# anonymousauthors001/SGS-GNN

Measured on AMD Instinct MI355X. Metric: sampled edges/sec + training steps/sec, Reddit hybrid 20% sparsity, higher is better.
Workload: dtype f32

## Files before the change

### include/sgs_hip.h

```cpp
#ifndef SGS_HIP_H_
#define SGS_HIP_H_

#include <stddef.h>
#include <stdint.h>

#ifdef __cplusplus
extern "C" {
#endif

#define SGS_ABI_VERSION 1

#define SGS_OK 0
#define SGS_EINVAL (-1)
#define SGS_EWORKSPACE (-2)
#define SGS_EHIP (-3)

typedef void* sgs_stream_t;

int sgs_abi_version(void);
const char* sgs_last_error(void);

int sgs_rng_set_epoch_buffer(const uint64_t* epoch_dev);
int sgs_exp_noise(uint64_t seed, uint64_t stream_id, int64_t E, float* noise, sgs_stream_t stream);
int sgs_dropout_keep(uint64_t seed, uint32_t site, int64_t rows, int64_t cols, float p, uint8_t* keep,
// ... 171 lines not shown
                            const float* W1, const float* b1, const float* w2, const float* b2, float p_drop,
                            uint64_t seed, uint32_t site, float* dv, float* hdz_part, float* dz, float* feat, void* ws,
                            size_t ws_bytes, sgs_stream_t stream);
int sgs_edge_score_bwd_dfeat_supported(int64_t H);
int sgs_edge_score_bwd_dfeat(const float* dv, int64_t n, int64_t H, const float* W1, float* dfeat, void* ws, size_t ws_bytes,
                             sgs_stream_t stream);

int sgs_edge_score_bwd_bits_supported(int64_t H);
int sgs_edge_score_fwd_mask(const float* codes, const float* U, int64_t N, int64_t H, const int64_t* edge_index, int64_t E,
                            int64_t edge_id_offset, const int32_t* canon, int64_t M, const int32_t* mate, const float* W1, const float* b1,
                            const float* w2, const float* b2, float p_drop, uint64_t seed, uint32_t site, float* p_out, uint32_t* maskbits,
                            void* ws, size_t ws_bytes, sgs_stream_t stream);
int sgs_edge_score_bwd_prep(const float* codes, int64_t N, int64_t H, const int64_t* edge_index, int64_t E, const int64_t* active_eid,
                            int64_t n_active, const float* grad_p, const float* p, const uint32_t* maskbits, float* dz, uint32_t* dvbits,
                            float* feat, sgs_stream_t stream);
int sgs_edge_score_dw2_from_parts(const float* W1, const float* T_raw, const float* U, const float* R_raw, const float* b1, const float* c_raw,
                                  int64_t N, int64_t H, float p_drop, float* dw2, sgs_stream_t stream);
int sgs_edge_score_probe_set(int stagger, int prio, uint32_t mode_mask);
int sgs_edge_score_probe_trace(unsigned long long* buf);
size_t sgs_edge_score_epd_workspace_bytes(int64_t H);
int sgs_edge_score_epd_fwd(const float* A, int64_t N, int64_t H, const int64_t* edge_index, int64_t E, int64_t edge_id_offset, const float* W1,
                           const float* b1, const float* w2, const float* b2, float p_hidden, uint64_t seed, uint32_t site, float p_ep,
                           uint64_t seed_x, uint32_t site_x, uint64_t seed_y, uint32_t site_y, float* p_out, void* ws, size_t ws_bytes,
                           sgs_stream_t stream);
int sgs_edge_score_epd_bwd_core(const float* A, int64_t N, int64_t H, const int64_t* edge_index, int64_t E, int64_t edge_id_offset,
                                const int64_t* active_eid, int64_t n_active, const float* grad_p, const float* W1, const float* b1, const float* w2,
                                const float* b2, float p_hidden, uint64_t seed, uint32_t site, float p_ep, uint64_t seed_x, uint32_t site_x,
                                uint64_t seed_y, uint32_t site_y, float* dv, float* hdz_part, float* dz, float* feat2, void* ws, size_t ws_bytes,
                                sgs_stream_t stream);
int sgs_edge_score_epd_reduce(const float* dfeat2, const float* A, int64_t N, int64_t H, const int32_t* in_ptr, const int32_t* in_src,
                              const int32_t* in_eid, const int32_t* out_ptr, const int32_t* out_dst, const int32_t* out_eid,
                              const int64_t* active_eid, int64_t edge_id_offset, float p_ep, uint64_t seed_x, uint32_t site_x, uint64_t seed_y,
                              uint32_t site_y, float* dA, sgs_stream_t stream);

int sgs_edge_score_bwd_prep_sd(const float* codes, int64_t N, int64_t H, const int64_t* edge_index, int64_t E, const int64_t* active_eid,
                               int64_t n_active, const float* grad_p, const float* p, const uint32_t* maskbits, float* dz, uint32_t* dvbits,
                               int32_t* sd, sgs_stream_t stream);
size_t sgs_edge_score_bwd_fused_opart_rows(int64_t n, int64_t N);
int sgs_edge_score_bwd_dfeat_fused(const uint32_t* dvbits, const float* dz, const int32_t* sd, const float* codes, int64_t n, int64_t N, int64_t H,
                                   const float* W1, const float* w2, float p_drop, float* G, float* opart, void* ws, size_t ws_bytes,
                                   sgs_stream_t stream);
int sgs_edge_score_bwd_reduce_fused(const float* G, const float* opart, const uint32_t* dvbits, const float* dz, const float* w2, float p_drop,
                                    int64_t N, int64_t H, int64_t nnz, const int32_t* in_ptr, const int32_t* in_eid, const int32_t* out_ptr,
                                    float* out_codes, float* out_U, float* out_U_raw, sgs_stream_t stream);
int sgs_edge_score_bwd_prep_sd_pack(const float* codes, int64_t N, int64_t H, const int64_t* edge_index, int64_t E, const int64_t* active_eid,
                                    int64_t n_active, const float* grad_p, const float* p, const uint32_t* maskbits, float* dz, uint32_t* dvbits,
                                    int32_t* sd, const float* W1, const float* w2, float p_drop, void* ws, size_t ws_bytes, sgs_stream_t stream);
int sgs_edge_score_bwd_dfeat_fused_packed(const uint32_t* dvbits, const float* dz, const int32_t* sd, const float* codes, int64_t n, int64_t N,
                                          int64_t H, float* G, float* opart, const void* ws, size_t ws_bytes, sgs_stream_t stream);
int sgs_edge_score_bwd_core_bits(const float* codes, const float* U, int64_t N, int64_t H, const int64_t* edge_index, int64_t E,
                                 int64_t edge_id_offset, const int64_t* active_eid, int64_t n_active, const float* grad_p, const float* W1,
                                 const float* b1, const float* w2, const float* b2, float p_drop, uint64_t seed, uint32_t site,
                                 uint32_t* dvbits, float* hdz_part, float* dz, float* feat, void* ws, size_t ws_bytes, sgs_stream_t stream);
int sgs_edge_score_bwd_dfeat_bits(const uint32_t* dvbits, const float* dz, int64_t n, int64_t H, const float* W1, const float* w2, float p_drop,
                                  float* dfeat, void* ws, size_t ws_bytes, sgs_stream_t stream);
int sgs_endpoint_reduce_pair_bits(const float* dfeat, const uint32_t* dvbits, const float* dz, const float* w2, float p_drop, const float* codes,
                                  int64_t N, int64_t H, int64_t nnz, const int32_t* in_ptr, const int32_t* in_src, const int32_t* in_eid,
                                  const int32_t* out_ptr, const int32_t* out_dst, const int32_t* out_eid, float* out_codes, float* out_U,
                                  float* out_U_raw, sgs_stream_t stream);
int sgs_gemm_tn_mask_supported(int64_t K, int64_t M, int64_t N);
int sgs_gemm_tn_mask_gather(const uint32_t* Abits, const float* dz, const float* rowscale, float scale, const float* codes, int64_t codes_rows,
                            const int32_t* sd, int64_t K, int64_t M, int64_t N, float* C, int64_t ldc, float* colsum_A, float* dz_sum, float* C_raw,
                            float* colsum_raw, void* ws, size_t ws_bytes, sgs_stream_t stream);
void sgs_gemm_tn_set_gather_variant(int shared, int slabs);
int sgs_gemm_tn_mask(const uint32_t* Abits, const float* dz, const float* rowscale, float scale, const float* B, int64_t K, int64_t M, int64_t N,
                     float* C, int64_t ldc, float* colsum_A, float* dz_sum, float* C_raw, float* colsum_raw, void* ws, size_t ws_bytes,
                     sgs_stream_t stream);

int sgs_edge_score_bf16_supported(int64_t H);
int sgs_edge_score_fwd_bf16(const float* codes, const float* U, int64_t N, int64_t H, const int64_t* edge_index, int64_t E,
                            int64_t edge_id_offset, const float* W1, const float* b1, const float* w2, const float* b2, float p_drop,
                            uint64_t seed, uint32_t site, float* p_out, void* ws, size_t ws_bytes, sgs_stream_t stream);
int sgs_edge_score_fwd_paired_bf16(const float* codes, const float* U, int64_t N, int64_t H, const int64_t* edge_index, int64_t E,
                                   int64_t edge_id_offset, const int32_t* canon, int64_t M, const int32_t* mate, const float* W1, const float* b1,
                                   const float* w2, const float* b2, float p_drop, uint64_t seed, uint32_t site, float* p_out, void* ws,
                                   size_t ws_bytes, sgs_stream_t stream);
int sgs_edge_score_fwd_mask_bf16(const float* codes, const float* U, int64_t N, int64_t H, const int64_t* edge_index, int64_t E,
                                 int64_t edge_id_offset, const int32_t* canon, int64_t M, const int32_t* mate, const float* W1, const float* b1,
                                 const float* w2, const float* b2, float p_drop, uint64_t seed, uint32_t site, float* p_out, uint32_t* maskbits,
                                 void* ws, size_t ws_bytes, sgs_stream_t stream);
int sgs_edge_score_bwd_dfeat_bits_bf16(const uint32_t* dvbits, const float* dz, int64_t n, int64_t H, const float* W1, const float* w2,
                                       float p_drop, float* dfeat, void* ws, size_t ws_bytes, sgs_stream_t stream);
int sgs_edge_score_bwd_prep_sd_pack_bf16(const float* codes, int64_t N, int64_t H, const int64_t* edge_index, int64_t E, const int64_t* active_eid,
                                         int64_t n_active, const float* grad_p, const float* p, const uint32_t* maskbits, float* dz, uint32_t* dvbits,
                                         int32_t* sd, const float* W1, const float* w2, float p_drop, void* ws, size_t ws_bytes, sgs_stream_t stream);
int sgs_edge_score_bwd_dfeat_fused_bf16(const uint32_t* dvbits, const float* dz, const int32_t* sd, const float* codes, int64_t n, int64_t N,
                                        int64_t H, const float* W1, const float* w2, float p_drop, float* G, float* opart, void* ws, size_t ws_bytes,
                                        sgs_stream_t stream);
int sgs_edge_score_bwd_dfeat_fused_packed_bf16(const uint32_t* dvbits, const float* dz, const int32_t* sd, const float* codes, int64_t n, int64_t N,
                                               int64_t H, float* G, float* opart, const void* ws, size_t ws_bytes, sgs_stream_t stream);
int sgs_gemm_tn_mask_bf16(const uint32_t* Abits, const float* dz, const float* rowscale, float scale, const float* B, int64_t K, int64_t M, int64_t N,
                          float* C, int64_t ldc, float* colsum_A, float* dz_sum, float* C_raw, float* colsum_raw, void* ws, size_t ws_bytes,
                          sgs_stream_t stream);
int sgs_gemm_tn_mask_gather_bf16(const uint32_t* Abits, const float* dz, const float* rowscale, float scale, const float* codes, int64_t codes_rows,
                                 const int32_t* sd, int64_t K, int64_t M, int64_t N, float* C, int64_t ldc, float* colsum_A, float* dz_sum, float* C_raw,
                                 float* colsum_raw, void* ws, size_t ws_bytes, sgs_stream_t stream);

int sgs_endpoint_reduce(const float* M_out, const float* M_in, const float* T, int64_t N, int64_t H, int64_t nnz,
                        const int32_t* in_ptr, const int32_t* in_src, const int32_t* in_eid, const int32_t* out_ptr,
                        const int32_t* out_dst, const int32_t* out_eid, float sign_out, float sign_in, float* out,
                        sgs_stream_t stream);
int sgs_endpoint_reduce_pair(const float* dfeat, const float* dv, const float* codes, int64_t N, int64_t H, int64_t nnz,
                             const int32_t* in_ptr, const int32_t* in_src, const int32_t* in_eid, const int32_t* out_ptr,
                             const int32_t* out_dst, const int32_t* out_eid, float* out_codes, float* out_U, sgs_stream_t stream);

int sgs_masked_correct(const float* logits, int64_t N, int64_t C, const int64_t* y, const uint8_t* train_mask,
                       int32_t* correct, sgs_stream_t stream);
int sgs_masked_correct_pair(const float* logits_a, const float* logits_b, int64_t N, int64_t C, const int64_t* y,
                            const uint8_t* train_mask, int32_t* correct4, sgs_stream_t stream);

int sgs_confusion_counts(const float* logits, int64_t N, int64_t C, const int64_t* y, const uint8_t* m0, const uint8_t* m1, const uint8_t* m2,
                         int64_t* conf, sgs_stream_t stream);
int sgs_confusion_variant(int64_t N, int64_t C);
int sgs_confusion_variant_set(int code);

size_t sgs_gate_counts_workspace_bytes(int64_t N);
int sgs_gate_counts(const float* logits_a, const float* logits_b, int64_t N, int64_t C, const int64_t* y, const uint8_t* train_mask,
                    int32_t* out5, const uint64_t* seq_dev, int32_t* dst_host_mapped, void* ws, size_t ws_bytes, sgs_stream_t stream);

int sgs_loss_tick(float* loss_sum, const float* loss, uint64_t* epoch, sgs_stream_t stream);
int sgs_publish_to_host(const int32_t* src_dev, int64_t n, const uint64_t* seq_dev, int32_t* dst_host_mapped, sgs_stream_t stream);

int sgs_masked_ce_fwd(const float* logits, int64_t N, int64_t C, const int64_t* y, const uint8_t* train_mask,
                      float* loss, float* row_lse, float* rowloss, int32_t* n_rows, sgs_stream_t stream);
int sgs_masked_ce_bwd(const float* logits, int64_t N, int64_t C, const int64_t* y, const uint8_t* train_mask,
                      const float* row_lse, const int32_t* n_rows, const float* grad_loss, float* dlogits,
                      sgs_stream_t stream);

size_t sgs_edge_reg_workspace_bytes(int64_t q);
int sgs_edge_reg_fwd(const float* w, const int64_t* sampled_edge_index, int64_t q, const float* logits, int64_t N,
                     int64_t C, const int64_t* y, const uint8_t* train_mask, float coef1, float coef2, float* out,
                     float* cos_out, void* ws, size_t ws_bytes, sgs_stream_t stream);
int sgs_edge_reg_bwd(const float* w, const int64_t* sampled_edge_index, int64_t q, int64_t q_global, const float* logits,
                     int64_t N, int64_t C, const int64_t* y, const uint8_t* train_mask, const float* out, float coef1,
                     float coef2, const float* grad_loss, float* dw, float* Gs, float* Gd, sgs_stream_t stream);

int sgs_hybrid_loss_fwd(const float* logits, int64_t N, int64_t C, const int64_t* y, const uint8_t* train_mask, const float* w,
                        const int64_t* sampled_edge_index, int64_t q, float coef1, float coef2, float* out, float* row_lse, float* rowloss,
                        int32_t* n_rows, void* ws, size_t ws_bytes, sgs_stream_t stream);
int sgs_masked_ce_bwd_acc(const float* logits, int64_t N, int64_t C, const int64_t* y, const uint8_t* train_mask, const float* row_lse,
                          const int32_t* n_rows, const float* grad_loss, float* dlogits, sgs_stream_t stream);

int sgs_masked_ce_w_fwd(const float* logits, int64_t N, int64_t C, const int64_t* y, const uint8_t* train_mask, const float* weight,
                        float label_smoothing, float* loss, float* row_lse, float* rowloss, float* den, sgs_stream_t stream);
int sgs_masked_ce_w_bwd(const float* logits, int64_t N, int64_t C, const int64_t* y, const uint8_t* train_mask, const float* weight,
                        float label_smoothing, const float* row_lse, const float* den, const float* grad_loss, float* dlogits,
                        sgs_stream_t stream);
int sgs_masked_ce_w_bwd_acc(const float* logits, int64_t N, int64_t C, const int64_t* y, const uint8_t* train_mask, const float* weight,
                            float label_smoothing, const float* row_lse, const float* den, const float* grad_loss, float* dlogits,
                            sgs_stream_t stream);
int sgs_hybrid_loss_w_fwd(const float* logits, int64_t N, int64_t C, const int64_t* y, const uint8_t* train_mask, const float* w,
                          const int64_t* sampled_edge_index, int64_t q, float coef1, float coef2, const float* weight, float label_smoothing,
                          float* out, float* row_lse, float* rowloss, float* den, void* ws, size_t ws_bytes, sgs_stream_t stream);

int sgs_edge_reg_partial(const float* w, const int64_t* sampled_edge_index, int64_t q, const float* logits, int64_t N,
                         int64_t C, const int64_t* y, const uint8_t* train_mask, float* raw, void* ws, size_t ws_bytes,
                         sgs_stream_t stream);

int sgs_gat_scores_fwd(const float* xl, int64_t N, int64_t D, const float* att_src, const float* att_dst, float* a_src, float* a_dst,
                       sgs_stream_t stream);
size_t sgs_gat_scores_bwd_workspace_bytes(int64_t N, int64_t D);
int sgs_gat_scores_bwd(const float* xl, int64_t N, int64_t D, const float* att_src, const float* att_dst, const float* g_src, const float* g_dst,
                       int accumulate, float* dxl, float* datt_src, float* datt_dst, void* ws, size_t ws_bytes, sgs_stream_t stream);
int sgs_gat_alpha_fwd(const float* a_src, const float* a_dst, int64_t N, int64_t n_edges, const int32_t* in_ptr,
                      const int32_t* in_src, const int32_t* in_eid, float negative_slope, float p_drop, uint64_t seed,
                      uint32_t site, float* soft_in, float* soft_loop, float* alpha_in, float* alpha_loop,
                      sgs_stream_t stream);
int sgs_gat_alpha_bwd(const float* a_src, const float* a_dst, int64_t N, int64_t n_edges, const int32_t* in_ptr,
                      const int32_t* in_src, const int32_t* in_eid, float negative_slope, float p_drop, uint64_t seed,
                      uint32_t site, const float* soft_in, const float* soft_loop, const float* galpha,
                      const float* gloop, float* g_edge, float* g_selfloop, float* d_a_dst, sgs_stream_t stream);
int sgs_gather_by_eid(const float* by_eid, const int32_t* eid, int64_t n, float* out_order, sgs_stream_t stream);
int sgs_scatter_by_eid(const float* in_order, const int32_t* eid, int64_t n, float* by_eid, sgs_stream_t stream);

#define SGS_HEADS_CONCAT 0
#define SGS_HEADS_MEAN 1
#define SGS_HEADS_BROADCAST 2
int sgs_gat_heads_supported(int64_t K, int64_t C);
#define SGS_GAT_OP_SCORES_FWD 0
#define SGS_GAT_OP_SCORES_BWD 1
#define SGS_GAT_OP_SPMM_CONCAT 2
#define SGS_GAT_OP_SPMM_MEAN 3
#define SGS_GAT_OP_SPMM_BROADCAST 4
#define SGS_GAT_OP_SDDMM 5
#define SGS_GAT_OP_SDDMM_BROADCAST 6
#define SGS_GAT_OP_ROW 7
int sgs_gat_heads_variant(int op, int64_t N, int64_t K, int64_t C, int aligned16);
int sgs_gat_scores_heads_fwd(const float* xl, int64_t N, int64_t K, int64_t C, const float* att_src, const float* att_dst, float* a_src,
                             float* a_dst, sgs_stream_t stream);
size_t sgs_gat_scores_heads_bwd_workspace_bytes(int64_t N, int64_t K, int64_t C);
int sgs_gat_scores_heads_bwd(const float* xl, int64_t N, int64_t K, int64_t C, const float* att_src, const float* att_dst, const float* g_src,
                             const float* g_dst, int accumulate, float* dxl, float* datt_src, float* datt_dst, void* ws, size_t ws_bytes,
                             sgs_stream_t stream);
int sgs_gat_alpha_heads_fwd(const float* a_src, const float* a_dst, int64_t N, int64_t K, int64_t n_edges, const int32_t* in_ptr,
                            const int32_t* in_src, const int32_t* in_eid, float negative_slope, float p_drop, uint64_t seed, uint32_t site,
                            float* soft, float* soft_loop, float* alpha, float* alpha_loop, sgs_stream_t stream);
int sgs_gat_alpha_heads_bwd(const float* a_src, const float* a_dst, int64_t N, int64_t K, int64_t n_edges, const int32_t* in_ptr,
                            const int32_t* in_src, const int32_t* in_eid, float negative_slope, float p_drop, uint64_t seed, uint32_t site,
                            const float* soft, const float* soft_loop, const float* galpha, const float* gloop, float* g_edge, float* g_selfloop,
                            float* d_a_dst, sgs_stream_t stream);
int sgs_gat_alpha_heads_edge_fwd(const float* a_src, const float* a_dst, const float* edge_w, const float* edge_coef, int64_t N, int64_t K,
                                 int64_t n_edges, const int32_t* in_ptr, const int32_t* in_src, const int32_t* in_eid, float negative_slope,
                                 float p_drop, uint64_t seed, uint32_t site, float* soft, float* soft_loop, float* alpha, float* alpha_loop,
                                 float* loop_w, float* loop_inv_cnt, sgs_stream_t stream);
size_t sgs_gat_alpha_heads_edge_bwd_workspace_bytes(int64_t N, int64_t K);
int sgs_gat_alpha_heads_edge_bwd(const float* a_src, const float* a_dst, const float* edge_w, const float* edge_coef, const float* loop_w,
                                 const float* loop_inv_cnt, int64_t N, int64_t K, int64_t n_edges, const int32_t* in_ptr, const int32_t* in_src,
                                 const int32_t* in_eid, float negative_slope, float p_drop, uint64_t seed, uint32_t site, const float* soft,
                                 const float* soft_loop, const float* galpha, const float* gloop, const float* dw_add, float* g_edge,
                                 float* g_selfloop, float* d_a_dst, float* d_edge_w, float* d_edge_coef, void* ws, size_t ws_bytes,
                                 sgs_stream_t stream);
int sgs_edge_sum_by_row_heads(const float* g_edge, const float* g_self, int64_t N, int64_t K, int64_t nnz, const int32_t* ptr, const int32_t* eid,
                              float* out, sgs_stream_t stream);
int sgs_spmm_csr_heads(const float* X, int64_t N, int64_t K, int64_t C, int64_t nnz, const int32_t* ptr, const int32_t* col, const int32_t* eid,
                       const float* val, const float* diag, int mode, const float* bias, int act, float p_drop, uint64_t seed, uint32_t site,
                       float* Y, sgs_stream_t stream);
int sgs_sddmm_csr_heads(const float* A, const float* B, int64_t N, int64_t K, int64_t C, int64_t nnz, const int32_t* ptr, const int32_t* col,
                        const int32_t* eid, int broadcast, float* g, float* gdiag, sgs_stream_t stream);

#define SGS_GATV2_OP_ALPHA_FWD 0
#define SGS_GATV2_OP_ALPHA_BWD 1
#define SGS_GATV2_OP_DXL 2
int sgs_gatv2_variant(int op, int64_t N, int64_t K, int64_t C, int aligned16);
int sgs_gatv2_alpha_heads_fwd(const float* xl, const float* xr, const float* att, const float* edge_w, const float* lin_edge, int64_t N,
                              int64_t K, int64_t C, int64_t n_edges, const int32_t* in_ptr, const int32_t* in_src, const int32_t* in_eid,
                              float negative_slope, float p_drop, uint64_t seed, uint32_t site, float* soft, float* soft_loop, float* alpha,
                              float* alpha_loop, float* loop_w, float* loop_inv_cnt, sgs_stream_t stream);
int sgs_gatv2_alpha_heads_fwd_multi(const float* xl, const float* xr, int64_t x_stride, const float* att, const float* edge_w,
                                    const float* lin_edge, int64_t N, int64_t K, int64_t C, int64_t D, int64_t nnz, const int32_t* in_ptr,
                                    const int32_t* in_src, const int32_t* in_eid, float negative_slope, float* alpha, float* alpha_loop,
                                    sgs_stream_t stream);
size_t sgs_gatv2_alpha_heads_bwd_workspace_bytes(int64_t N, int64_t K, int64_t C);
int sgs_gatv2_alpha_heads_bwd(const float* xl, const float* xr, const float* att, const float* edge_w, const float* lin_edge, const float* loop_w,
                              const float* loop_inv_cnt, int64_t N, int64_t K, int64_t C, int64_t n_edges, const int32_t* in_ptr,
                              const int32_t* in_src, const int32_t* in_eid, float negative_slope, float p_drop, uint64_t seed, uint32_t site,
                              const float* soft, const float* soft_loop, const float* galpha, const float* gloop, const float* dw_add,
                              float* g_logit, float* g_loop, float* d_xr, float* d_att, float* d_lin_edge, float* d_edge_w, void* ws,
                              size_t ws_bytes, sgs_stream_t stream);
int sgs_gatv2_dxl_heads(const float* xl, const float* xr, const float* att, const float* edge_w, const float* lin_edge, const float* loop_w,
                        const float* g_logit, const float* g_loop, int64_t N, int64_t K, int64_t C, int64_t nnz, const int32_t* out_ptr,
                        const int32_t* out_dst, const int32_t* out_eid, float negative_slope, int accumulate, float* d_xl,
                        sgs_stream_t stream);

int sgs_gine_variant(int64_t N, int64_t D, int64_t nnz, int align_bytes);
int sgs_gine_aggregate_fwd(const float* x, const float* edge_w, const float* a, const float* b, float diag, int64_t N, int64_t D,
                           int64_t n_edges, const int32_t* in_ptr, const int32_t* in_src, const int32_t* in_eid, float* z,
                           sgs_stream_t stream);
int sgs_gine_aggregate_fwd_multi(const float* x, int64_t x_stride, const float* edge_w, const float* a, const float* b, float diag,
                                 int64_t N, int64_t Dc, int64_t nnz, int64_t D, const int32_t* in_ptr, const int32_t* in_src,
                                 const int32_t* in_eid, float* z, sgs_stream_t stream);
size_t sgs_gine_aggregate_bwd_workspace_bytes(int64_t N, int64_t D);
int sgs_gine_aggregate_bwd(const float* x, const float* dz, const float* edge_w, const float* a, const float* b, float diag, int64_t N,
                           int64_t D, int64_t n_edges, const int32_t* out_ptr, const int32_t* out_dst, const int32_t* out_eid,
                           const float* dw_add, float* d_x, float* d_edge_w, float* d_a, float* d_b, void* ws, size_t ws_bytes,
                           sgs_stream_t stream);

int sgs_cheb_supported(int64_t K);
int sgs_cheb_norm_fwd(const float* w, int64_t n_edges, int64_t N, const int32_t* in_ptr, const int32_t* in_src, const int32_t* in_eid,
                      const int32_t* out_ptr, const int32_t* out_dst, const int32_t* out_eid, float* dis, float* l_in, float* l_out,
                      sgs_stream_t stream);
size_t sgs_cheb_norm_bwd_workspace_bytes(int64_t N);
int sgs_cheb_norm_bwd(const float* w, const float* g, const float* g2, int64_t n_edges, int64_t N, const float* dis, const int32_t* in_ptr,
                      const int32_t* in_src, const int32_t* in_eid, const int32_t* out_ptr, const int32_t* out_dst, const int32_t* out_eid,
                      const int64_t* edge_index, float* dw, void* ws, size_t ws_bytes, sgs_stream_t stream);
int sgs_cheb_spmm_variant(int64_t N, int64_t D, int64_t nnz, int64_t ldx, int aligned16);
int sgs_cheb_spmm(int64_t K, const float* X, int64_t ldx, int64_t N, int64_t D, int64_t nnz, const int32_t* ptr, const int32_t* col,
                  const float* val, float alpha, const float* add, int64_t ldadd, const float* sub, int64_t ldsub, const float* bias, int act,
                  float p_drop, uint64_t seed, uint32_t site, float* Y, int64_t ldy, float* Y2, int64_t ldy2, float scale2,
                  sgs_stream_t stream);

size_t sgs_gemm_tn_workspace_bytes(int64_t K, int64_t M, int64_t N);
int sgs_gemm_tn(const float* A, const float* B, int64_t K, int64_t M, int64_t N, float* C, void* ws, size_t ws_bytes,
                sgs_stream_t stream);
void sgs_gemm_tn_set_tall_variant(int variant);
int sgs_gemm_tn_can_colsum(int64_t K, int64_t M, int64_t N);
int sgs_gemm_tn_colsum(const float* A, const float* B, int64_t K, int64_t M, int64_t N, float* C, float* colsum_A, void* ws,
                       size_t ws_bytes, sgs_stream_t stream);
int sgs_gemm_tn_ld(const float* A, const float* B, int64_t K, int64_t M, int64_t N, float* C, int64_t ldc, float* colsum_A, void* ws,
                   size_t ws_bytes, sgs_stream_t stream);
typedef struct SgsGemmTnProblem {
    const float* A;
    const float* B;
    int64_t K, M, N;
    float* C;
    int64_t ldc;
    void* ws;
    size_t ws_bytes;
} SgsGemmTnProblem;
int sgs_gemm_tn_group_supported(int64_t K, int64_t M, int64_t N);
int sgs_gemm_tn_group(const SgsGemmTnProblem* problems, int count, sgs_stream_t stream);

int sgs_er_weight(const int64_t* edge_index, int64_t E, int64_t N, const int32_t* out_ptr, const int32_t* out_dst, int walk_lengths,
                  int walks, uint64_t seed, float* weight, sgs_stream_t stream);

int sgs_adam_max_tensors(void);
int sgs_adam_step(const int64_t* desc_host, int64_t n_tensors, float lr, float beta1, float beta2, float eps, float weight_decay,
                  int maximize, uint32_t* ticket, sgs_stream_t stream);
int sgs_adam_multi_max_tensors(void);
int sgs_adam_step_multi(const int64_t* desc_host, const float* hyper_host, int64_t n_tensors, uint32_t* ticket, float* loss_sum, const float* loss,
                        uint64_t* epoch, sgs_stream_t stream);

size_t sgs_sample_topq_multi_workspace_bytes(int64_t E, int64_t D);
int sgs_sample_topq_multi(int mode, const float* p, const float* prior, double degree_bias_coef, const float* noise, uint64_t seed,
                          uint64_t stream_id0, int64_t D, int64_t E, int64_t q, const int64_t* edge_index, uint8_t* mask, int64_t* sampled_eid,
                          int64_t* sampled_edge_index, float* stats, float* st_weights, void* ws, size_t ws_bytes, sgs_stream_t stream);
size_t sgs_sample_topq_multi_cover_workspace_bytes(int64_t E, int64_t N, int64_t D);
// ... 41 lines not shown
```

### sgs-gnn_amd/csrc/edge_score.hip

```cpp
#include <type_traits>

#include "sgs_common.h"

namespace sgs {
namespace {

constexpr int kT = 256;
constexpr int kBM = 64;
constexpr int kBK = 16;
using f32x16 = __attribute__((ext_vector_type(16))) float;

__global__ void __launch_bounds__(kT) transpose_w1a(const float* __restrict__ W1, int H, float* __restrict__ WaT) {
    __shared__ float t[32][33];
    const int bx = blockIdx.x * 32, by = blockIdx.y * 32;
    const int tx = threadIdx.x & 31, ty = threadIdx.x >> 5;
    for (int r = ty; r < 32; r += 8) {
        const int h = by + r, k = bx + tx;
        t[r][tx] = (h < H && k < H) ? W1[static_cast<int64_t>(h) * 2 * H + k] : 0.f;
    }
    __syncthreads();
    for (int r = ty; r < 32; r += 8) {
        const int k = bx + r, h = by + tx;
        if (k < H && h < H) WaT[static_cast<int64_t>(k) * H + h] = t[tx][r];
    }
}

__global__ void __launch_bounds__(kT) transpose_w1_full(const float* __restrict__ W1, int H, float* __restrict__ WT) {
    __shared__ float t[32][33];
    const int bx = blockIdx.x * 32, by = blockIdx.y * 32;
    const int tx = threadIdx.x & 31, ty = threadIdx.x >> 5;
    for (int r = ty; r < 32; r += 8) {
        const int h = by + r, k = bx + tx;
        t[r][tx] = (h < H && k < 2 * H) ? W1[static_cast<int64_t>(h) * 2 * H + k] : 0.f;
    }
    __syncthreads();
    for (int r = ty; r < 32; r += 8) {
        const int k = bx + r, h = by + tx;
        if (k < 2 * H && h < H) WT[static_cast<int64_t>(k) * H + h] = t[tx][r];
    }
}

struct ScoreArgs {
    const float* codes;
    const float* U;
    const int64_t* src;
    const int64_t* dst;
    const int64_t* active;
    int64_t n;
    const int32_t* canon;
    const int32_t* mate;
    const int64_t* dyn_n;
    int64_t row_offset;
    int H;
    const float* WaT;
    const float* b1;
    const float* w2;
    const float* b2;
    float drop_scale;
    uint32_t drop_thresh;
    uint64_t seed;
    const uint64_t* epoch;
    uint32_t site;
    int use_drop;
    float* p_out;
    const float* gp;
    float* dv;
    float* hdz;
    float* dz;
    float* feat;
    uint32_t* dvbits;
    const uint32_t* inbits;
    const float* indz;
    int epd;
    uint64_t seed_x, seed_y;
    uint32_t site_x, site_y;
    float ep_scale;
    uint32_t ep_thresh;
    const int32_t* sd;
    float* opart;
    int stagger, prio;
    unsigned long long* trace;
};

template <int NT, bool BWD, bool EXACT, bool EPD = false>
__global__ void __launch_bounds__(kT, 3) edge_score_kernel(ScoreArgs a) {
    constexpr int HP = 32 * NT;
    constexpr int NTW = NT / 2;
    extern __shared__ __attribute__((aligned(16))) char smem[];
    float* Wt_s0 = reinterpret_cast<float*>(smem);
    float* Ft_s0 = Wt_s0 + 2 * kBK * HP;
    int* s_idx = reinterpret_cast<int*>(Ft_s0 + 2 * kBK * kBM);
    int* d_idx = s_idx + kBM;
    float* zpart = reinterpret_cast<float*>(d_idx + kBM);
    const int tid = threadIdx.x, lane = tid & 63, wave = tid >> 6;
    const int eg = wave & 1, hh = wave >> 1;
    const int H = EXACT ? HP : a.H;
    const int64_t row0 = static_cast<int64_t>(blockIdx.x) * kBM;
    if (a.dyn_n) {
        const int64_t live_n = *a.dyn_n;
        if (live_n < a.n) a.n = live_n;
        if (row0 >= a.n) return;
    }

    if (tid < kBM) {
        const int64_t r = row0 + tid;
        int s = 0, d = 0;
        if (r < a.n) {
            const int64_t e = a.active ? a.active[r] : r;
            s = static_cast<int>(a.src[e]);
            d = static_cast<int>(a.dst[e]);
        }
        s_idx[tid] = s;
        d_idx[tid] = d;
    }

    f32x16 acc[NTW];
#pragma unroll
    for (int t = 0; t < NTW; ++t)
#pragma unroll
        for (int r = 0; r < 16; ++r) acc[t][r] = 0.f;

    const int kh = lane >> 5, l31 = lane & 31;
    __syncthreads();

    constexpr int kWV = (kBK * (HP / 4) + kT - 1) / kT;
    float4 wreg[kWV], xreg, yreg;
    const int fe = tid & (kBM - 1), fc = tid >> 6;
    const int my_s = s_idx[fe], my_d = d_idx[fe];
    const int KT = EPD ? 2 * H : H;
    uint32_t rkx = 0u, rky = 0u;
    if (EPD) {
        const int64_t r_ = row0 + fe;
        const int64_t e_ = r_ < a.n ? (a.active ? a.active[r_] : r_) : 0;
        rkx = dropout_row_key(fold_epoch(a.seed_x, a.epoch), a.site_x, static_cast<uint64_t>(a.row_offset + e_));
        rky = dropout_row_key(fold_epoch(a.seed_y, a.epoch), a.site_y, static_cast<uint64_t>(a.row_offset + e_));
    }
    auto ep_mask = [&](float4& v, uint32_t rk, int kk) {
        const uint32_t b0 = dropout_pair_bits(rk, static_cast<uint32_t>(kk >> 1)), b1 = dropout_pair_bits(rk, static_cast<uint32_t>((kk >> 1) + 1));
        v.x = (b0 & 0xFFFFu) >= a.ep_thresh ? v.x * a.ep_scale : 0.f;
        v.y = (b0 >> 16) >= a.ep_thresh ? v.y * a.ep_scale : 0.f;
        v.z = (b1 & 0xFFFFu) >= a.ep_thresh ? v.z * a.ep_scale : 0.f;
        v.w = (b1 >> 16) >= a.ep_thresh ? v.w * a.ep_scale : 0.f;
    };
    auto fetch = [&](int k0) {
#pragma unroll
        for (int j = 0; j < kWV; ++j) {
            const int i = j * kT + tid;
            const int k = i / (HP / 4), h4 = (i % (HP / 4)) * 4;
            wreg[j] = make_float4(0.f, 0.f, 0.f, 0.f);
            if (EXACT || (i < kBK * (HP / 4) && k0 + k < KT && h4 < H))
                wreg[j] = *reinterpret_cast<const float4*>(a.WaT + static_cast<int64_t>(k0 + k) * H + h4);
        }
        const int kf = k0 + 4 * fc;
        const int kk = (EPD && kf >= H) ? kf - H : kf;
        xreg = make_float4(0.f, 0.f, 0.f, 0.f);
// ... 1367 lines not shown
#pragma unroll
    for (int i = 0; i < 4 * NT; ++i) {
        if (8 * i < Hrt) {
            const int t = i >> 2, g4 = i & 3;
            const int hb = 8 * i + 4 * kh;
            const float4 ww = *reinterpret_cast<const float4*>(&bw[1][hb]);
            const float w4[4] = {ww.x, ww.y, ww.z, ww.w};
            float dv4[4], hs[4];
#pragma unroll
            for (int j = 0; j < 4; ++j) {
                const float hd = acc[t][4 * g4 + j];
                dv4[j] = dzv * w4[j] * (hd > 0.f ? dscale : 0.f);
                hs[j] = dzv * hd;
                mbits[t] |= (hd > 0.f ? 1u : 0u) << (8 * g4 + 4 * kh + j);
            }
            if (live && a.dv) *reinterpret_cast<float4*>(a.dv + r * H + hb) = make_float4(dv4[0], dv4[1], dv4[2], dv4[3]);
#pragma unroll
            for (int j = 0; j < 4; ++j) hs[j] = half_wave_sum_hi(hs[j]);
            if (l31 == 31) *reinterpret_cast<float4*>(hsum + wave * H + hb) = make_float4(hs[0], hs[1], hs[2], hs[3]);
        }
    }
    if (a.dvbits) {
#pragma unroll
        for (int t = 0; t < NT; ++t) mbits[t] |= __shfl_xor(mbits[t], 32, 64);
        if (live && kh == 0) {
            uint4* bo = reinterpret_cast<uint4*>(a.dvbits + r * NT);
#pragma unroll
            for (int t = 0; t < NT; t += 4) bo[t >> 2] = make_uint4(mbits[t], mbits[t + 1], mbits[t + 2], mbits[t + 3]);
        }
    }
    __syncthreads();
    for (int idx = tid; idx < (NW / 2) * H; idx += TH) {
        const int m = idx / H, h = idx - m * H;
        const int64_t prow = static_cast<int64_t>(blockIdx.x) * (NW / 2) + m;
        if (prow * 64 < a.n) a.hdz[prow * H + h] = hsum[(2 * m) * H + h] + hsum[(2 * m + 1) * H + h];
    }
}

template <int NT, int THREADS>
__global__ void __launch_bounds__(THREADS, THREADS / 256) edge_score_wres_kernel(ScoreArgs a, const float* __restrict__ Wp,
                                                                                  const float* __restrict__ Ceo,
                                                                                  unsigned int* __restrict__ tile_ctr,
                                                                                  float* __restrict__ zpart) {
    constexpr int H = 32 * NT;
    constexpr int NTW = NT / 2;
    constexpr int NJ4 = H / 8;
    extern __shared__ __attribute__((aligned(16))) char smem[];
    float4* Ws = reinterpret_cast<float4*>(smem);
    const int tid = threadIdx.x, lane = tid & 63;
    const int hh = blockIdx.x & 1;
    const int kh = lane >> 5, l31 = lane & 31;
    {
        const float4* src = reinterpret_cast<const float4*>(Wp) + static_cast<int64_t>(hh) * NTW * NJ4 * 64;
        for (int i = tid; i < NTW * NJ4 * 64; i += THREADS) Ws[i] = src[i];
    }
    __syncthreads();
    const int64_t n_tiles = (a.n + 31) >> 5;
    const int Hrt = a.H;
    for (;;) {
        unsigned int t32 = 0;
        if (lane == 0) t32 = atomicAdd(&tile_ctr[hh], 1u);
        t32 = __builtin_amdgcn_readfirstlane(t32);
        if (static_cast<int64_t>(t32) >= n_tiles) break;
        const int64_t r = static_cast<int64_t>(t32) * 32 + l31;
        const bool live = r < a.n;
        int s = 0, d = 0;
        int64_t eg_id = 0;
        if (live) {
            eg_id = a.active ? a.active[r] : r;
            s = static_cast<int>(a.src[eg_id]);
            d = static_cast<int>(a.dst[eg_id]);
        }
        const float4* xp = reinterpret_cast<const float4*>(Ceo + static_cast<int64_t>(s) * H + kh * (H / 2));
        const float4* yp = reinterpret_cast<const float4*>(Ceo + static_cast<int64_t>(d) * H + kh * (H / 2));
        f32x16 acc[NTW];
#pragma unroll
        for (int t = 0; t < NTW; ++t)
#pragma unroll
            for (int q = 0; q < 16; ++q) acc[t][q] = 0.f;
        float4 A0[NTW], A1[NTW], x0, y0, x1, y1;
        auto load = [&](int j4, float4 (&A)[NTW], float4& x, float4& y) {
#pragma unroll
            for (int t = 0; t < NTW; ++t) A[t] = Ws[(t * NJ4 + j4) * 64 + lane];
            x = xp[j4];
            y = yp[j4];
        };
        auto mma = [&](const float4 (&A)[NTW], const float4& x, const float4& y) {
            const float b[4] = {x.x * y.x, x.y * y.y, x.z * y.z, x.w * y.w};
#pragma unroll
            for (int jj = 0; jj < 4; ++jj) {
#pragma unroll
                for (int t = 0; t < NTW; ++t) {
                    const float av = jj == 0 ? A[t].x : jj == 1 ? A[t].y : jj == 2 ? A[t].z : A[t].w;
                    acc[t] = __builtin_amdgcn_mfma_f32_32x32x2f32(av, b[jj], acc[t], 0, 0, 0);
                }
            }
        };
        load(0, A0, x0, y0);
#pragma unroll 1
        for (int j4 = 0; j4 < NJ4; j4 += 2) {
            load(j4 + 1, A1, x1, y1);
            mma(A0, x0, y0);
            if (j4 + 2 < NJ4) load(j4 + 2, A0, x0, y0);
            mma(A1, x1, y1);
        }
        const uint32_t rkey = dropout_row_key(fold_epoch(a.seed, a.epoch), a.site, static_cast<uint64_t>(a.row_offset + eg_id));
        const float* Us = a.U + static_cast<int64_t>(s) * H;
        const float* Ud = a.U + static_cast<int64_t>(d) * H;
        float z = 0.f;
#pragma unroll
        for (int t = 0; t < NTW; ++t) {
#pragma unroll
            for (int g = 0; g < 4; ++g) {
                const int hb = hh * (H / 2) + 32 * t + 8 * g + 4 * kh;
                if (hb < Hrt) {
                    const float4 us = *reinterpret_cast<const float4*>(Us + hb);
                    const float4 ud = *reinterpret_cast<const float4*>(Ud + hb);
                    const float4 bb = *reinterpret_cast<const float4*>(a.b1 + hb);
                    const float4 ww = *reinterpret_cast<const float4*>(a.w2 + hb);
                    const float u4[4] = {us.x - ud.x, us.y - ud.y, us.z - ud.z, us.w - ud.w};
                    const float b4[4] = {bb.x, bb.y, bb.z, bb.w};
                    const float w4[4] = {ww.x, ww.y, ww.z, ww.w};
                    uint32_t bits[2] = {0u, 0u};
                    if (a.use_drop) {
                        bits[0] = dropout_pair_bits(rkey, static_cast<uint32_t>(hb >> 1));
                        bits[1] = dropout_pair_bits(rkey, static_cast<uint32_t>((hb >> 1) + 1));
                    }
#pragma unroll
                    for (int j = 0; j < 4; ++j) {
                        const float v = (acc[t][4 * g + j] + u4[j]) + b4[j];
                        float m = v > 0.f ? 1.f : 0.f;
                        if (a.use_drop) {
                            const uint32_t draw = (j & 1) ? (bits[j >> 1] >> 16) : (bits[j >> 1] & 0xFFFFu);
                            m = draw >= a.drop_thresh ? m * a.drop_scale : 0.f;
                        }
                        z = fmaf(w4[j], v * m, z);
                    }
                }
            }
        }
        z += __shfl_xor(z, 32, 64);
        if (live && kh == 0) zpart[static_cast<int64_t>(hh) * a.n + r] = z;
    }
}

__global__ void __launch_bounds__(kT) edge_score_finish(const float* __restrict__ zpart, int64_t n, const float* __restrict__ b2,
                                                       float* __restrict__ p_out) {
    const int64_t r = static_cast<int64_t>(blockIdx.x) * kT + threadIdx.x;
    if (r >= n) return;
    const float z = (zpart[r] + zpart[n + r]) + b2[0];
    p_out[r] = 1.0f / (1.0f + expf(-z));
}

template <int VEC, bool HAS_T>
__global__ void __launch_bounds__(kT) endpoint_reduce(const float* __restrict__ Mo, const float* __restrict__ Mi,
                                                     const float* __restrict__ T, int64_t N, int64_t H,
                                                     const int* __restrict__ in_ptr, const int* __restrict__ in_src,
                                                     const int* __restrict__ in_eid, const int* __restrict__ out_ptr,
                                                     const int* __restrict__ out_dst, const int* __restrict__ out_eid,
                                                     float sgn_out, float sgn_in, float* __restrict__ out) {
    const int lane = threadIdx.x & 63;
    const int64_t v = (static_cast<int64_t>(blockIdx.x) * kT + threadIdx.x) >> 6;
    if (v >= N) return;
    for (int64_t c0 = static_cast<int64_t>(lane) * VEC; c0 < H; c0 += 64 * VEC) {
        float acc[VEC];
#pragma unroll
        for (int j = 0; j < VEC; ++j) acc[j] = 0.f;
        for (int dir = 0; dir < 2; ++dir) {
            const int* ptr = dir == 0 ? out_ptr : in_ptr;
            const int* col = dir == 0 ? out_dst : in_src;
            const int* eid = dir == 0 ? out_eid : in_eid;
            const float sg = dir == 0 ? sgn_out : sgn_in;
            const float* M = dir == 0 ? Mo : Mi;
            const int b = ptr[v], e = ptr[v + 1];
            for (int k = b; k < e; ++k) {
                float m[VEC], t[VEC];
                if (VEC == 4) {
                    *reinterpret_cast<float4*>(m) = *reinterpret_cast<const float4*>(M + static_cast<int64_t>(eid[k]) * H + c0);
                    if (HAS_T) *reinterpret_cast<float4*>(t) = *reinterpret_cast<const float4*>(T + static_cast<int64_t>(col[k]) * H + c0);
                } else {
                    m[0] = M[static_cast<int64_t>(eid[k]) * H + c0];
                    if (HAS_T) t[0] = T[static_cast<int64_t>(col[k]) * H + c0];
                }
#pragma unroll
                for (int j = 0; j < VEC; ++j) acc[j] = fmaf(sg * m[j], HAS_T ? t[j] : 1.0f, acc[j]);
            }
        }
        if (VEC == 4) *reinterpret_cast<float4*>(out + v * H + c0) = *reinterpret_cast<float4*>(acc);
        else out[v * H + c0] = acc[0];
    }
}

template <int VEC, bool HAS_T, int NW>
__global__ void __launch_bounds__(64 * NW) endpoint_reduce_rowblock(const float* __restrict__ Mo, const float* __restrict__ Mi,
                                                              const float* __restrict__ T, int64_t N, int64_t H,
                                                              const int* __restrict__ in_ptr, const int* __restrict__ in_src,
                                                              const int* __restrict__ in_eid, const int* __restrict__ out_ptr,
                                                              const int* __restrict__ out_dst, const int* __restrict__ out_eid,
                                                              float sgn_out, float sgn_in, float* __restrict__ out) {
    using V = typename std::conditional<VEC == 4, float4, float>::type;
    __shared__ float part[NW][64 * VEC];
    const int lane = threadIdx.x & 63, wave = threadIdx.x >> 6;
    const int64_t v = blockIdx.x;
    const int ob = out_ptr[v], no = out_ptr[v + 1] - ob;
    const int ib = in_ptr[v], ni = in_ptr[v + 1] - ib;
    const int total = no + ni;
    for (int64_t cbase = 0; cbase < H; cbase += 64 * VEC) {
        const int64_t c0 = cbase + static_cast<int64_t>(lane) * VEC;
        float acc[VEC];
#pragma unroll
        for (int j = 0; j < VEC; ++j) acc[j] = 0.f;
        if (c0 < H) {
            for (int k0 = wave; k0 < total; k0 += 4 * NW) {
                float m[4][VEC], t[4][VEC], sg[4];
                int er[4], cr[4];
                const float* Mp[4];
#pragma unroll
                for (int u = 0; u < 4; ++u) {
                    const int k = k0 + NW * u;
                    const int kc = k < total ? k : total - 1;
                    const bool isout = kc < no;
                    const int idx = isout ? ob + kc : ib + (kc - no);
                    er[u] = (isout ? out_eid : in_eid)[idx];
                    if (HAS_T) cr[u] = (isout ? out_dst : in_src)[idx];
                    Mp[u] = isout ? Mo : Mi;
                    sg[u] = k < total ? (isout ? sgn_out : sgn_in) : 0.f;
                }
#pragma unroll
                for (int u = 0; u < 4; ++u) {
                    *reinterpret_cast<V*>(m[u]) = *reinterpret_cast<const V*>(Mp[u] + static_cast<int64_t>(er[u]) * H + c0);
                    if (HAS_T) *reinterpret_cast<V*>(t[u]) = *reinterpret_cast<const V*>(T + static_cast<int64_t>(cr[u]) * H + c0);
                    else {
#pragma unroll
                        for (int j = 0; j < VEC; ++j) t[u][j] = 1.f;
                    }
                }
#pragma unroll
                for (int u = 0; u < 4; ++u)
#pragma unroll
                    for (int j = 0; j < VEC; ++j) acc[j] = fmaf(sg[u] * m[u][j], t[u][j], acc[j]);
            }
        }
#pragma unroll
        for (int j = 0; j < VEC; ++j) part[wave][lane * VEC + j] = acc[j];
        __syncthreads();
        const int tt = threadIdx.x;
        if (tt < 64 * VEC && cbase + tt < H) {
            float sum = 0.f;
#pragma unroll
            for (int g = 0; g < NW; g += 4) sum += (part[g][tt] + part[g + 1][tt]) + (part[g + 2][tt] + part[g + 3][tt]);
            out[v * H + cbase + tt] = sum;
        }
        __syncthreads();
    }
}

__global__ void __launch_bounds__(kT) scorer_bwd_prep(const float* __restrict__ codes, int64_t H, const int64_t* __restrict__ src,
                                                     const int64_t* __restrict__ dst, const int64_t* __restrict__ active, int64_t n,
                                                     const float* __restrict__ gp, const float* __restrict__ p,
                                                     const uint32_t* __restrict__ maskbits, float* __restrict__ dz,
                                                     uint32_t* __restrict__ bits, float* __restrict__ feat, int32_t* __restrict__ sd) {
    constexpr int R = 4;
    const int lane = threadIdx.x & 63;
    const int64_t r0 = ((static_cast<int64_t>(blockIdx.x) * kT + threadIdx.x) >> 6) * R;
    if (r0 >= n) return;
    const int wpr = static_cast<int>(H >> 5);
    int64_t e[R], s[R], d[R];
#pragma unroll
    for (int u = 0; u < R; ++u) {
        const int64_t r = r0 + u < n ? r0 + u : n - 1;
        e[u] = active ? active[r] : r;
    }
#pragma unroll
    for (int u = 0; u < R; ++u) { s[u] = src[e[u]]; d[u] = dst[e[u]]; }
#pragma unroll
    for (int u = 0; u < R; ++u) {
        if (r0 + u >= n) break;
        if (lane < wpr) bits[(r0 + u) * wpr + lane] = maskbits[e[u] * wpr + lane];
        if (lane == 63) { const float pe = p[e[u]]; dz[r0 + u] = gp[r0 + u] * pe * (1.0f - pe); }
        if (sd && lane == 62) { sd[2 * (r0 + u)] = static_cast<int32_t>(s[u]); sd[2 * (r0 + u) + 1] = static_cast<int32_t>(d[u]); }
    }
    if (!feat) return;
    for (int64_t c0 = static_cast<int64_t>(lane) * 4; c0 < H; c0 += 256) {
        float4 a[R], b[R];
#pragma unroll
        for (int u = 0; u < R; ++u) {
            a[u] = *reinterpret_cast<const float4*>(codes + s[u] * H + c0);
            b[u] = *reinterpret_cast<const float4*>(codes + d[u] * H + c0);
        }
#pragma unroll
        for (int u = 0; u < R; ++u)
            if (r0 + u < n)
                *reinterpret_cast<float4*>(feat + (r0 + u) * H + c0) = make_float4(a[u].x * b[u].x, a[u].y * b[u].y, a[u].z * b[u].z, a[u].w * b[u].w);
    }
}

template <int P = 3>
__global__ void __launch_bounds__(kT) scorer_bwd_prep_sd_pack(const int64_t* __restrict__ src, const int64_t* __restrict__ dst,
                                                             const int64_t* __restrict__ active, int64_t n, int wpr,
                                                             const float* __restrict__ gp, const float* __restrict__ p,
                                                             const uint32_t* __restrict__ maskbits, float* __restrict__ dz,
                                                             uint32_t* __restrict__ bits, int2* __restrict__ sd, int64_t n_prep_blocks,
                                                             const float* __restrict__ W1, int H, uint4* __restrict__ Wp16,
                                                             const float* __restrict__ w2, float scale) {
    if (static_cast<int64_t>(blockIdx.x) >= n_prep_blocks) {
        pack_w1a_bf16x3_one<true, P>((static_cast<int64_t>(blockIdx.x) - n_prep_blocks) * kT + threadIdx.x, W1, H, Wp16, w2, scale);
        return;
    }
    const int64_t r = static_cast<int64_t>(blockIdx.x) * kT + threadIdx.x;
    if (r >= n) return;
    const int64_t e = active ? active[r] : r;
    const int64_t s = src[e], d = dst[e];
    const float pe = p[e], g = gp[r];
    if ((wpr & 3) == 0) {
        const uint4* mi = reinterpret_cast<const uint4*>(maskbits + e * wpr);
        uint4* mo = reinterpret_cast<uint4*>(bits + r * wpr);
        for (int k = 0; k < (wpr >> 2); ++k) mo[k] = mi[k];
    } else {
        for (int k = 0; k < wpr; ++k) bits[r * wpr + k] = maskbits[e * wpr + k];
    }
    dz[r] = g * pe * (1.0f - pe);
    sd[r] = make_int2(static_cast<int32_t>(s), static_cast<int32_t>(d));
}

__global__ void __launch_bounds__(kT) scorer_dw2_from_parts(const float* __restrict__ W1, const float* __restrict__ Traw, const float* __restrict__ U,
                                                           const float* __restrict__ Rraw, const float* __restrict__ b1,
                                                           const float* __restrict__ craw, int64_t N, int H, float scale,
                                                           float* __restrict__ dw2) {
    __shared__ float red[kT / 64];
    const int h = blockIdx.x;
    float a = 0.f, b = 0.f;
    for (int k = threadIdx.x; k < H; k += kT) a = fmaf(W1[static_cast<int64_t>(h) * 2 * H + k], Traw[static_cast<int64_t>(h) * H + k], a);
    for (int64_t v = threadIdx.x; v < N; v += kT) b = fmaf(U[v * H + h], Rraw[v * H + h], b);
    const float ra = block_sum(a, red);
    const float rb = block_sum(b, red);
    if (threadIdx.x == 0) dw2[h] = scale * ((ra + rb) + b1[h] * craw[h]);
}

constexpr int kEpU = 4;
template <int NW, bool BITS = false>
__global__ void __launch_bounds__(64 * NW) endpoint_reduce_pair_rowblock(const float* __restrict__ dfeat, const float* __restrict__ dv,
                                                                        const float* __restrict__ codes, int64_t N, int64_t H,
                                                                        const int* __restrict__ in_ptr, const int* __restrict__ in_src,
                                                                        const int* __restrict__ in_eid, const int* __restrict__ out_ptr,
                                                                        const int* __restrict__ out_dst, const int* __restrict__ out_eid,
                                                                        float* __restrict__ out_codes, float* __restrict__ out_U,
                                                                        const uint32_t* __restrict__ bits = nullptr,
                                                                        const float* __restrict__ dz = nullptr,
                                                                        const float* __restrict__ w2 = nullptr, float scale = 1.f,
                                                                        float* __restrict__ out_Uraw = nullptr) {
    __shared__ float part[2][NW][256];
    const int lane = threadIdx.x & 63, wave = threadIdx.x >> 6;
    const int64_t v = blockIdx.x;
    const int ob = out_ptr[v], no = out_ptr[v + 1] - ob;
    const int ib = in_ptr[v], ni = in_ptr[v + 1] - ib;
    const int total = no + ni;
    for (int64_t cbase = 0; cbase < H; cbase += 256) {
        const int64_t c0 = cbase + static_cast<int64_t>(lane) * 4;
        float a1[4] = {0.f, 0.f, 0.f, 0.f}, a2[4] = {0.f, 0.f, 0.f, 0.f};
        if (c0 < H) {
            for (int k0 = wave; k0 < total; k0 += kEpU * NW) {
                int er[kEpU], cr[kEpU];
                float sg[kEpU], ok[kEpU];
#pragma unroll
                for (int u = 0; u < kEpU; ++u) {
                    const int k = k0 + NW * u;
                    const int kc = k < total ? k : total - 1;
                    const bool isout = kc < no;
                    const int idx = isout ? ob + kc : ib + (kc - no);
                    er[u] = (isout ? out_eid : in_eid)[idx];
                    cr[u] = (isout ? out_dst : in_src)[idx];
                    ok[u] = k < total ? 1.f : 0.f;
                    sg[u] = k < total ? (isout ? 1.f : -1.f) : 0.f;
                }
                float m1[kEpU][4], m2[kEpU][4], t[kEpU][4];
                uint32_t wd[kEpU];
                float dzr[kEpU];
#pragma unroll
                for (int u = 0; u < kEpU; ++u) {
                    *reinterpret_cast<float4*>(m1[u]) = *reinterpret_cast<const float4*>(dfeat + static_cast<int64_t>(er[u]) * H + c0);
                    *reinterpret_cast<float4*>(t[u]) = *reinterpret_cast<const float4*>(codes + static_cast<int64_t>(cr[u]) * H + c0);
                    if constexpr (BITS) {
                        wd[u] = bits[static_cast<int64_t>(er[u]) * (H >> 5) + (c0 >> 5)];
                        dzr[u] = dz[er[u]];
                    } else {
                        *reinterpret_cast<float4*>(m2[u]) = *reinterpret_cast<const float4*>(dv + static_cast<int64_t>(er[u]) * H + c0);
                    }
                }
#pragma unroll
                for (int u = 0; u < kEpU; ++u) {
                    if constexpr (BITS) {
                        const uint32_t w = wd[u] >> (c0 & 31);
#pragma unroll
                        for (int j = 0; j < 4; ++j) m2[u][j] = (w >> j) & 1u ? dzr[u] : 0.f;
                    }
#pragma unroll
                    for (int j = 0; j < 4; ++j) {
                        a1[j] = fmaf(ok[u] * m1[u][j], t[u][j], a1[j]);
                        a2[j] = fmaf(sg[u], m2[u][j], a2[j]);
                    }
                }
            }
        }
#pragma unroll
        for (int j = 0; j < 4; ++j) { part[0][wave][lane * 4 + j] = a1[j]; part[1][wave][lane * 4 + j] = a2[j]; }
        __syncthreads();
        for (int tt = threadIdx.x; tt < 512; tt += 64 * NW) {
            const int which = tt >> 8, c = tt & 255;
// ... 528 lines not shown
    SGS_REQUIRE(n_active >= 0 && (active_eid || n_active == E), SGS_EINVAL,
                "sgs_edge_score_bwd_core: n_active must equal E when active_eid is NULL");
    if (n_active == 0) return SGS_OK;
    SGS_REQUIRE(codes && U && edge_index && grad_p && W1 && b1 && w2 && b2 && (dv || dvbits) && hdz_part && dz && feat, SGS_EINVAL,
                "sgs_edge_score_bwd_core: null pointer");
    SGS_REQUIRE(ws && ws_bytes >= sgs_edge_score_workspace_bytes(N, H, 0), SGS_EWORKSPACE, "sgs_edge_score_bwd_core: workspace too small");
    Carver cv(ws);
    float* WaT = cv.take<float>(static_cast<size_t>(H) * H);
    float* Ceo = cv.take<float>(static_cast<size_t>(N) * H);
    if (H > 256) {
        SGS_REQUIRE(dv && !dvbits && N > 0, SGS_EINVAL, "sgs_edge_score_bwd_core: H=%lld needs the dense dv form", (long long)H);
        hipLaunchKernelGGL(transpose_w1a, dim3(cdiv(H, 32), cdiv(H, 32)), dim3(kT), 0, stream, W1, static_cast<int>(H), WaT);
        ScoreArgs a{};
        a.codes = codes; a.U = U; a.src = edge_index; a.dst = edge_index + E; a.active = active_eid; a.n = n_active;
        a.row_offset = edge_id_offset;
        a.H = static_cast<int>(H); a.WaT = WaT; a.b1 = b1; a.w2 = w2; a.b2 = b2;
        a.drop_scale = 1.0f / (1.0f - p_drop); a.drop_thresh = dropout_thresh(p_drop); a.seed = seed; a.epoch = epoch_ptr(); a.site = site;
        a.use_drop = p_drop > 0.f; a.gp = grad_p; a.dv = dv; a.hdz = hdz_part; a.dz = dz; a.feat = feat;
        return launch_score_wide<true, false>(a, stream);
    }
    const int bwd_variant = dvbits ? 4 : (g_bwd_variant >= 0 ? g_bwd_variant : ((H % 128 == 0 && cdiv(n_active, 128) >= 512) ? 4 : 0));
    if (bwd_variant == 4 && H % 128 == 0 && N > 0) {
        cv.take<float>(0);
        cv.take<unsigned int>(64);
        uint4* Wp16 = cv.take<uint4>(static_cast<size_t>(H) * H * 6 / 16);
        hipLaunchKernelGGL(pack_w1a_bf16x3<false>, dim3(static_cast<unsigned>(cdiv((H / 16) * (H / 32) * 64, kT))), dim3(kT), 0, stream, W1,
                           static_cast<int>(H), Wp16);
        ScoreArgs b{};
        b.codes = codes; b.U = U; b.src = edge_index; b.dst = edge_index + E; b.active = active_eid; b.n = n_active;
        b.row_offset = edge_id_offset;
        b.H = static_cast<int>(H); b.WaT = nullptr; b.b1 = b1; b.w2 = w2; b.b2 = b2;
        b.drop_scale = 1.0f / (1.0f - p_drop); b.drop_thresh = dropout_thresh(p_drop); b.seed = seed; b.epoch = epoch_ptr(); b.site = site;
        b.use_drop = p_drop > 0.f; b.gp = grad_p; b.dv = dv; b.dvbits = dvbits; b.hdz = hdz_part; b.dz = dz; b.feat = feat;
        const dim3 grid(static_cast<unsigned>(cdiv(n_active, 128))), blk(256);
        bf16x6_launch_knobs(b, 1, H);
        if (H == 256) hipLaunchKernelGGL((edge_score_bf16x6_kernel<8, 4, 1>), grid, blk, 0, stream, b, Wp16);
        else          hipLaunchKernelGGL((edge_score_bf16x6_kernel<4, 4, 1>), grid, blk, 0, stream, b, Wp16);
        SGS_LAUNCH_OK();
        return SGS_OK;
    }
    const bool stream64 = H % 64 == 0 && bwd_variant == 3;
    if (stream64) {
        const int n_w = static_cast<int>(cdiv(H * H, kT));
        hipLaunchKernelGGL(pack_stream_operands, dim3(static_cast<unsigned>(n_w + cdiv(N * H, kT))), dim3(kT), 0, stream, W1,
                           static_cast<int>(H), WaT, n_w, codes, N, Ceo);
    } else {
        hipLaunchKernelGGL(transpose_w1a, dim3(cdiv(H, 32), cdiv(H, 32)), dim3(kT), 0, stream, W1, static_cast<int>(H), WaT);
    }
    ScoreArgs a{};
    a.codes = codes; a.U = U; a.src = edge_index; a.dst = edge_index + E; a.active = active_eid; a.n = n_active;
    a.row_offset = edge_id_offset;
    a.H = static_cast<int>(H); a.WaT = WaT; a.b1 = b1; a.w2 = w2; a.b2 = b2;
    a.drop_scale = 1.0f / (1.0f - p_drop); a.drop_thresh = dropout_thresh(p_drop); a.seed = seed; a.epoch = epoch_ptr(); a.site = site;
    a.use_drop = p_drop > 0.f; a.gp = grad_p; a.dv = dv; a.hdz = hdz_part; a.dz = dz; a.feat = feat;
    if (stream64) {
        const dim3 grid(static_cast<unsigned>(cdiv(n_active, kBM2))), blk(kT);
        if (H == 256)      hipLaunchKernelGGL((edge_score_stream64_kernel<8, true>), grid, blk, 0, stream, a, WaT, Ceo);
        else if (H == 128) hipLaunchKernelGGL((edge_score_stream64_kernel<4, true>), grid, blk, 0, stream, a, WaT, Ceo);
        else               hipLaunchKernelGGL((edge_score_stream64_kernel<2, true>), grid, blk, 0, stream, a, WaT, Ceo);
        SGS_LAUNCH_OK();
        return SGS_OK;
    }
    return launch_score<true>(a, stream);
}

int sgs_edge_score_bwd_dfeat_supported(int64_t H) { return (H == 128 || H == 256) ? 1 : 0; }

int sgs_edge_score_bwd_dfeat(const float* dv, int64_t n, int64_t H, const float* W1, float* dfeat, void* ws, size_t ws_bytes,
                             sgs_stream_t stream_) {
    hipStream_t stream = static_cast<hipStream_t>(stream_);
    SGS_REQUIRE(n >= 0 && H > 0, SGS_EINVAL, "sgs_edge_score_bwd_dfeat: bad sizes");
    SGS_REQUIRE(sgs_edge_score_bwd_dfeat_supported(H), SGS_EINVAL, "sgs_edge_score_bwd_dfeat: H=%lld unsupported (128 or 256)", (long long)H);
    if (n == 0) return SGS_OK;
    SGS_REQUIRE(dv && W1 && dfeat, SGS_EINVAL, "sgs_edge_score_bwd_dfeat: null pointer");
    SGS_REQUIRE(ws && ws_bytes >= sgs_edge_score_workspace_bytes(0, H, 0), SGS_EWORKSPACE, "sgs_edge_score_bwd_dfeat: workspace too small");
    Carver cv(ws);
    cv.take<float>(static_cast<size_t>(H) * H);
    cv.take<float>(0);
    cv.take<float>(0);
    cv.take<unsigned int>(64);
    uint4* Wp16 = cv.take<uint4>(static_cast<size_t>(H) * H * 6 / 16);
    hipLaunchKernelGGL(pack_w1a_bf16x3<true>, dim3(static_cast<unsigned>(cdiv((H / 16) * (H / 32) * 64, kT))), dim3(kT), 0, stream, W1,
                       static_cast<int>(H), Wp16);
    ScoreArgs a{};
    a.codes = dv; a.n = n; a.H = static_cast<int>(H); a.feat = dfeat;
    const dim3 grid(static_cast<unsigned>(cdiv(n, 128))), blk(256);
    bf16x6_launch_knobs(a, 2, H);
    if (H == 256) hipLaunchKernelGGL((edge_score_bf16x6_kernel<8, 4, 2>), grid, blk, 0, stream, a, Wp16);
    else          hipLaunchKernelGGL((edge_score_bf16x6_kernel<4, 4, 2>), grid, blk, 0, stream, a, Wp16);
    SGS_LAUNCH_OK();
    return SGS_OK;
}

int sgs_edge_score_bwd_dfeat_bits(const uint32_t* dvbits, const float* dz, int64_t n, int64_t H, const float* W1, const float* w2, float p_drop,
                                  float* dfeat, void* ws, size_t ws_bytes, sgs_stream_t stream_) {
    hipStream_t stream = static_cast<hipStream_t>(stream_);
    SGS_REQUIRE(n >= 0 && H > 0 && p_drop >= 0.f && p_drop < 1.f, SGS_EINVAL, "sgs_edge_score_bwd_dfeat_bits: bad arguments");
    SGS_REQUIRE(sgs_edge_score_bwd_bits_supported(H), SGS_EINVAL, "sgs_edge_score_bwd_dfeat_bits: H=%lld unsupported (128 or 256)", (long long)H);
    if (n == 0) return SGS_OK;
    SGS_REQUIRE(dvbits && dz && W1 && w2 && dfeat, SGS_EINVAL, "sgs_edge_score_bwd_dfeat_bits: null pointer");
    SGS_REQUIRE(ws && ws_bytes >= sgs_edge_score_workspace_bytes(0, H, 0), SGS_EWORKSPACE, "sgs_edge_score_bwd_dfeat_bits: workspace too small");
    Carver cv(ws);
    cv.take<float>(static_cast<size_t>(H) * H);
    cv.take<float>(0);
    cv.take<float>(0);
    cv.take<unsigned int>(64);
    uint4* Wp16 = cv.take<uint4>(static_cast<size_t>(H) * H * 6 / 16);
    hipLaunchKernelGGL(pack_w1a_bf16x3<true>, dim3(static_cast<unsigned>(cdiv((H / 16) * (H / 32) * 64, kT))), dim3(kT), 0, stream, W1,
                       static_cast<int>(H), Wp16, w2, 1.0f / (1.0f - p_drop));
    ScoreArgs a{};
    a.inbits = dvbits; a.indz = dz; a.n = n; a.H = static_cast<int>(H); a.feat = dfeat;
    const dim3 grid(static_cast<unsigned>(cdiv(n, 128))), blk(256);
    bf16x6_launch_knobs(a, 4, H);
    if (H == 256) hipLaunchKernelGGL((edge_score_bf16x6_kernel<8, 4, 4>), grid, blk, 0, stream, a, Wp16);
    else          hipLaunchKernelGGL((edge_score_bf16x6_kernel<4, 4, 4>), grid, blk, 0, stream, a, Wp16);
    SGS_LAUNCH_OK();
    return SGS_OK;
}

static uint4* fused_wp16(void* ws, int64_t H);

int sgs_edge_score_bwd_dfeat_bits_bf16(const uint32_t* dvbits, const float* dz, int64_t n, int64_t H, const float* W1, const float* w2,
                                       float p_drop, float* dfeat, void* ws, size_t ws_bytes, sgs_stream_t stream_) {
    hipStream_t stream = static_cast<hipStream_t>(stream_);
    SGS_REQUIRE(n >= 0 && H > 0 && p_drop >= 0.f && p_drop < 1.f, SGS_EINVAL, "sgs_edge_score_bwd_dfeat_bits_bf16: bad arguments");
    SGS_REQUIRE(sgs_edge_score_bf16_supported(H), SGS_EINVAL, "sgs_edge_score_bwd_dfeat_bits_bf16: H=%lld unsupported (128 or 256)", (long long)H);
    if (n == 0) return SGS_OK;
    SGS_REQUIRE(dvbits && dz && W1 && w2 && dfeat, SGS_EINVAL, "sgs_edge_score_bwd_dfeat_bits_bf16: null pointer");
    SGS_REQUIRE(ws && ws_bytes >= sgs_edge_score_workspace_bytes(0, H, 0), SGS_EWORKSPACE, "sgs_edge_score_bwd_dfeat_bits_bf16: workspace too small");
    uint4* Wp16 = fused_wp16(ws, H);
    hipLaunchKernelGGL((pack_w1a_bf16x3<true, 1>), dim3(static_cast<unsigned>(cdiv(pack_w1a_threads(H), kT))), dim3(kT), 0, stream, W1,
                       static_cast<int>(H), Wp16, w2, 1.0f / (1.0f - p_drop));
    ScoreArgs a{};
    a.inbits = dvbits; a.indz = dz; a.n = n; a.H = static_cast<int>(H); a.feat = dfeat;
    const dim3 grid(static_cast<unsigned>(cdiv(n, 128))), blk(256);
    bf16x6_launch_knobs(a, 4, H, 1);
    if (H == 256) hipLaunchKernelGGL((edge_score_bf16x6_kernel<8, 4, 4, 1>), grid, blk, 0, stream, a, Wp16);
    else          hipLaunchKernelGGL((edge_score_bf16x6_kernel<4, 4, 4, 1>), grid, blk, 0, stream, a, Wp16);
    SGS_LAUNCH_OK();
    return SGS_OK;
}

int sgs_endpoint_reduce(const float* M_out, const float* M_in, const float* T, int64_t N, int64_t H, int64_t nnz,
                        const int32_t* in_ptr, const int32_t* in_src,
                        const int32_t* in_eid, const int32_t* out_ptr, const int32_t* out_dst, const int32_t* out_eid,
                        float sign_out, float sign_in, float* out, sgs_stream_t stream_) {
    hipStream_t stream = static_cast<hipStream_t>(stream_);
    SGS_REQUIRE(N >= 0 && H >= 0, SGS_EINVAL, "sgs_endpoint_reduce: bad sizes");
    if (N == 0 || H == 0) return SGS_OK;
    SGS_REQUIRE(M_out && M_in && in_ptr && out_ptr && out, SGS_EINVAL, "sgs_endpoint_reduce: null pointer");
    const bool v4 = H % 4 == 0 && (reinterpret_cast<uintptr_t>(M_out) & 15) == 0 && (reinterpret_cast<uintptr_t>(M_in) & 15) == 0 &&
                    (reinterpret_cast<uintptr_t>(out) & 15) == 0 &&
                    (!T || (reinterpret_cast<uintptr_t>(T) & 15) == 0);
    const dim3 blk(kT);
    if (nnz >= 8 * N) {
        const dim3 grid(static_cast<unsigned>(N));
        const bool wide = nnz >= 64 * N;
#define SGS_EPR(VEC_, HT_)                                                                                                   \
        do {                                                                                                                    \
            if (wide) hipLaunchKernelGGL((endpoint_reduce_rowblock<VEC_, HT_, 16>), grid, dim3(1024), 0, stream, M_out, M_in, T, N, H, in_ptr, \
                                         in_src, in_eid, out_ptr, out_dst, out_eid, sign_out, sign_in, out);                  \
            else      hipLaunchKernelGGL((endpoint_reduce_rowblock<VEC_, HT_, 4>), grid, blk, 0, stream, M_out, M_in, T, N, H, in_ptr,        \
                                         in_src, in_eid, out_ptr, out_dst, out_eid, sign_out, sign_in, out);                  \
        } while (0)
        if (v4) { if (T) SGS_EPR(4, true); else SGS_EPR(4, false); }
        else    { if (T) SGS_EPR(1, true); else SGS_EPR(1, false); }
#undef SGS_EPR
        SGS_LAUNCH_OK();
        return SGS_OK;
    }
    const dim3 grid(static_cast<unsigned>(cdiv(N * 64, kT)));
    if (v4) {
        if (T) hipLaunchKernelGGL((endpoint_reduce<4, true>), grid, blk, 0, stream, M_out, M_in, T, N, H, in_ptr, in_src, in_eid, out_ptr, out_dst, out_eid, sign_out, sign_in, out);
        else   hipLaunchKernelGGL((endpoint_reduce<4, false>), grid, blk, 0, stream, M_out, M_in, T, N, H, in_ptr, in_src, in_eid, out_ptr, out_dst, out_eid, sign_out, sign_in, out);
    } else {
        if (T) hipLaunchKernelGGL((endpoint_reduce<1, true>), grid, blk, 0, stream, M_out, M_in, T, N, H, in_ptr, in_src, in_eid, out_ptr, out_dst, out_eid, sign_out, sign_in, out);
        else   hipLaunchKernelGGL((endpoint_reduce<1, false>), grid, blk, 0, stream, M_out, M_in, T, N, H, in_ptr, in_src, in_eid, out_ptr, out_dst, out_eid, sign_out, sign_in, out);
    }
    SGS_LAUNCH_OK();
    return SGS_OK;
}

int sgs_endpoint_reduce_pair(const float* dfeat, const float* dv, const float* codes, int64_t N, int64_t H, int64_t nnz, const int32_t* in_ptr,
                             const int32_t* in_src, const int32_t* in_eid, const int32_t* out_ptr, const int32_t* out_dst,
                             const int32_t* out_eid, float* out_codes, float* out_U, sgs_stream_t stream_) {
    hipStream_t stream = static_cast<hipStream_t>(stream_);
    SGS_REQUIRE(N >= 0 && H >= 0 && H % 4 == 0 && N < (int64_t(1) << 31), SGS_EINVAL, "sgs_endpoint_reduce_pair: needs H %% 4 == 0");
    if (N == 0 || H == 0) return SGS_OK;
    SGS_REQUIRE(dfeat && dv && codes && in_ptr && out_ptr && out_codes && out_U, SGS_EINVAL, "sgs_endpoint_reduce_pair: null pointer");
    const dim3 grid(static_cast<unsigned>(N));
    if (nnz >= 64 * N)
        hipLaunchKernelGGL((endpoint_reduce_pair_rowblock<16>), grid, dim3(1024), 0, stream, dfeat, dv, codes, N, H, in_ptr, in_src, in_eid, out_ptr,
                           out_dst, out_eid, out_codes, out_U);
    else
        hipLaunchKernelGGL((endpoint_reduce_pair_rowblock<4>), grid, dim3(256), 0, stream, dfeat, dv, codes, N, H, in_ptr, in_src, in_eid, out_ptr,
                           out_dst, out_eid, out_codes, out_U);
    SGS_LAUNCH_OK();
    return SGS_OK;
}

static int bwd_prep_impl(const float* codes, int64_t N, int64_t H, const int64_t* edge_index, int64_t E, const int64_t* active_eid,
                         int64_t n_active, const float* grad_p, const float* p, const uint32_t* maskbits, float* dz, uint32_t* dvbits,
                         float* feat, int32_t* sd, hipStream_t stream) {
    SGS_REQUIRE(N > 0 && H > 0 && H % 32 == 0 && E >= 0 && n_active >= 0 && (active_eid || n_active == E), SGS_EINVAL,
                "sgs_edge_score_bwd_prep: bad arguments (H %% 32 == 0; n_active == E when active_eid is NULL)");
    if (n_active == 0) return SGS_OK;
    SGS_REQUIRE(codes && edge_index && grad_p && p && maskbits && dz && dvbits && (feat || sd), SGS_EINVAL, "sgs_edge_score_bwd_prep: null pointer");
    hipLaunchKernelGGL(scorer_bwd_prep, dim3(static_cast<unsigned>(cdiv(cdiv(n_active, 4) * 64, kT))), dim3(kT), 0, stream, codes, H, edge_index,
                       edge_index + E, active_eid, n_active, grad_p, p, maskbits, dz, dvbits, feat, sd);
    SGS_LAUNCH_OK();
    return SGS_OK;
}

int sgs_edge_score_bwd_prep(const float* codes, int64_t N, int64_t H, const int64_t* edge_index, int64_t E, const int64_t* active_eid,
                            int64_t n_active, const float* grad_p, const float* p, const uint32_t* maskbits, float* dz, uint32_t* dvbits,
                            float* feat, sgs_stream_t stream_) {
    SGS_REQUIRE(feat || n_active == 0, SGS_EINVAL, "sgs_edge_score_bwd_prep: null pointer");
    return bwd_prep_impl(codes, N, H, edge_index, E, active_eid, n_active, grad_p, p, maskbits, dz, dvbits, feat, nullptr,
                         static_cast<hipStream_t>(stream_));
}

static uint4* fused_wp16(void* ws, int64_t H) {
    Carver cv(ws);
    cv.take<float>(static_cast<size_t>(H) * H);
    cv.take<float>(0);
    cv.take<float>(0);
    cv.take<unsigned int>(64);
    return cv.take<uint4>(static_cast<size_t>(H) * H * 6 / 16);
}

static int bwd_prep_sd_impl(const float* codes, int64_t N, int64_t H, const int64_t* edge_index, int64_t E, const int64_t* active_eid,
                            int64_t n_active, const float* grad_p, const float* p, const uint32_t* maskbits, float* dz, uint32_t* dvbits,
                            int32_t* sd, const float* W1, const float* w2, float p_drop, uint4* Wp16, hipStream_t stream, int P = 3) {
    SGS_REQUIRE(N > 0 && H > 0 && H % 32 == 0 && E >= 0 && n_active >= 0 && (active_eid || n_active == E), SGS_EINVAL,
                "sgs_edge_score_bwd_prep_sd: bad arguments (H %% 32 == 0; n_active == E when active_eid is NULL)");
    if (n_active == 0) return SGS_OK;
    SGS_REQUIRE(codes && edge_index && grad_p && p && maskbits && dz && dvbits && sd, SGS_EINVAL, "sgs_edge_score_bwd_prep_sd: null pointer");
    const int64_t nb = cdiv(n_active, kT), npack = Wp16 ? cdiv(pack_w1a_threads(H), kT) : 0;
    if (P == 1)
        hipLaunchKernelGGL(scorer_bwd_prep_sd_pack<1>, dim3(static_cast<unsigned>(nb + npack)), dim3(kT), 0, stream, edge_index, edge_index + E,
                           active_eid, n_active, static_cast<int>(H >> 5), grad_p, p, maskbits, dz, dvbits, reinterpret_cast<int2*>(sd), nb, W1,
                           static_cast<int>(H), Wp16, w2, 1.0f / (1.0f - p_drop));
    else
        hipLaunchKernelGGL(scorer_bwd_prep_sd_pack<3>, dim3(static_cast<unsigned>(nb + npack)), dim3(kT), 0, stream, edge_index, edge_index + E,
                           active_eid, n_active, static_cast<int>(H >> 5), grad_p, p, maskbits, dz, dvbits, reinterpret_cast<int2*>(sd), nb, W1,
                           static_cast<int>(H), Wp16, w2, 1.0f / (1.0f - p_drop));
    SGS_LAUNCH_OK();
    return SGS_OK;
}

int sgs_edge_score_bwd_prep_sd(const float* codes, int64_t N, int64_t H, const int64_t* edge_index, int64_t E, const int64_t* active_eid,
                               int64_t n_active, const float* grad_p, const float* p, const uint32_t* maskbits, float* dz, uint32_t* dvbits,
                               int32_t* sd, sgs_stream_t stream_) {
    return bwd_prep_sd_impl(codes, N, H, edge_index, E, active_eid, n_active, grad_p, p, maskbits, dz, dvbits, sd, nullptr, nullptr, 0.f,
                            nullptr, static_cast<hipStream_t>(stream_));
}

int sgs_edge_score_bwd_prep_sd_pack(const float* codes, int64_t N, int64_t H, const int64_t* edge_index, int64_t E, const int64_t* active_eid,
                                    int64_t n_active, const float* grad_p, const float* p, const uint32_t* maskbits, float* dz, uint32_t* dvbits,
                                    int32_t* sd, const float* W1, const float* w2, float p_drop, void* ws, size_t ws_bytes, sgs_stream_t stream_) {
    SGS_REQUIRE(p_drop >= 0.f && p_drop < 1.f, SGS_EINVAL, "sgs_edge_score_bwd_prep_sd_pack: bad arguments");
    SGS_REQUIRE(sgs_edge_score_bwd_bits_supported(H), SGS_EINVAL, "sgs_edge_score_bwd_prep_sd_pack: H=%lld unsupported (128 or 256)", (long long)H);
    if (n_active == 0) return SGS_OK;
    SGS_REQUIRE(W1 && w2, SGS_EINVAL, "sgs_edge_score_bwd_prep_sd_pack: null pointer");
    SGS_REQUIRE(ws && ws_bytes >= sgs_edge_score_workspace_bytes(0, H, 0), SGS_EWORKSPACE, "sgs_edge_score_bwd_prep_sd_pack: workspace too small");
    return bwd_prep_sd_impl(codes, N, H, edge_index, E, active_eid, n_active, grad_p, p, maskbits, dz, dvbits, sd, W1, w2, p_drop,
                            fused_wp16(ws, H), static_cast<hipStream_t>(stream_));
}

int sgs_edge_score_bwd_prep_sd_pack_bf16(const float* codes, int64_t N, int64_t H, const int64_t* edge_index, int64_t E, const int64_t* active_eid,
                                         int64_t n_active, const float* grad_p, const float* p, const uint32_t* maskbits, float* dz, uint32_t* dvbits,
                                         int32_t* sd, const float* W1, const float* w2, float p_drop, void* ws, size_t ws_bytes, sgs_stream_t stream_) {
    SGS_REQUIRE(p_drop >= 0.f && p_drop < 1.f, SGS_EINVAL, "sgs_edge_score_bwd_prep_sd_pack_bf16: bad arguments");
    SGS_REQUIRE(sgs_edge_score_bf16_supported(H), SGS_EINVAL, "sgs_edge_score_bwd_prep_sd_pack_bf16: H=%lld unsupported (128 or 256)", (long long)H);
    if (n_active == 0) return SGS_OK;
    SGS_REQUIRE(W1 && w2, SGS_EINVAL, "sgs_edge_score_bwd_prep_sd_pack_bf16: null pointer");
    SGS_REQUIRE(ws && ws_bytes >= sgs_edge_score_workspace_bytes(0, H, 0), SGS_EWORKSPACE, "sgs_edge_score_bwd_prep_sd_pack_bf16: workspace too small");
    return bwd_prep_sd_impl(codes, N, H, edge_index, E, active_eid, n_active, grad_p, p, maskbits, dz, dvbits, sd, W1, w2, p_drop,
                            fused_wp16(ws, H), static_cast<hipStream_t>(stream_), 1);
}

size_t sgs_edge_score_bwd_fused_opart_rows(int64_t n, int64_t N) { return static_cast<size_t>(cdiv(n < 0 ? 0 : n, 32) + (N < 0 ? 0 : N)); }

static int bwd_dfeat_fused_launch(const uint32_t* dvbits, const float* dz, const int32_t* sd, const float* codes, int64_t n, int64_t H,
                                  const uint4* Wp16, float* G, float* opart, hipStream_t stream, int P = 3) {
    ScoreArgs a{};
    a.inbits = dvbits; a.indz = dz; a.n = n; a.H = static_cast<int>(H); a.feat = G; a.codes = codes; a.sd = sd; a.opart = opart;
    const dim3 grid(static_cast<unsigned>(cdiv(n, 128))), blk(256);
    bf16x6_launch_knobs(a, 5, H, P);
    if (P == 1) {
        if (H == 256) hipLaunchKernelGGL((edge_score_bf16x6_kernel<8, 4, 5, 1>), grid, blk, 0, stream, a, Wp16);
        else          hipLaunchKernelGGL((edge_score_bf16x6_kernel<4, 4, 5, 1>), grid, blk, 0, stream, a, Wp16);
        SGS_LAUNCH_OK();
        return SGS_OK;
    }
    if (H == 256) hipLaunchKernelGGL((edge_score_bf16x6_kernel<8, 4, 5>), grid, blk, 0, stream, a, Wp16);
    else          hipLaunchKernelGGL((edge_score_bf16x6_kernel<4, 4, 5>), grid, blk, 0, stream, a, Wp16);
    SGS_LAUNCH_OK();
    return SGS_OK;
}

int sgs_edge_score_bwd_dfeat_fused(const uint32_t* dvbits, const float* dz, const int32_t* sd, const float* codes, int64_t n, int64_t N, int64_t H,
                                   const float* W1, const float* w2, float p_drop, float* G, float* opart, void* ws, size_t ws_bytes,
                                   sgs_stream_t stream_) {
    hipStream_t stream = static_cast<hipStream_t>(stream_);
    SGS_REQUIRE(n >= 0 && N > 0 && H > 0 && p_drop >= 0.f && p_drop < 1.f, SGS_EINVAL, "sgs_edge_score_bwd_dfeat_fused: bad arguments");
    SGS_REQUIRE(sgs_edge_score_bwd_bits_supported(H), SGS_EINVAL, "sgs_edge_score_bwd_dfeat_fused: H=%lld unsupported (128 or 256)", (long long)H);
    if (n == 0) return SGS_OK;
    SGS_REQUIRE(dvbits && dz && sd && codes && W1 && w2 && G && opart, SGS_EINVAL, "sgs_edge_score_bwd_dfeat_fused: null pointer");
    SGS_REQUIRE(ws && ws_bytes >= sgs_edge_score_workspace_bytes(0, H, 0), SGS_EWORKSPACE, "sgs_edge_score_bwd_dfeat_fused: workspace too small");
    uint4* Wp16 = fused_wp16(ws, H);
    hipLaunchKernelGGL(pack_w1a_bf16x3<true>, dim3(static_cast<unsigned>(cdiv(pack_w1a_threads(H), kT))), dim3(kT), 0, stream, W1,
                       static_cast<int>(H), Wp16, w2, 1.0f / (1.0f - p_drop));
    return bwd_dfeat_fused_launch(dvbits, dz, sd, codes, n, H, Wp16, G, opart, stream);
}

int sgs_edge_score_bwd_dfeat_fused_packed(const uint32_t* dvbits, const float* dz, const int32_t* sd, const float* codes, int64_t n, int64_t N,
                                          int64_t H, float* G, float* opart, const void* ws, size_t ws_bytes, sgs_stream_t stream_) {
    SGS_REQUIRE(n >= 0 && N > 0 && H > 0, SGS_EINVAL, "sgs_edge_score_bwd_dfeat_fused_packed: bad arguments");
    SGS_REQUIRE(sgs_edge_score_bwd_bits_supported(H), SGS_EINVAL, "sgs_edge_score_bwd_dfeat_fused_packed: H=%lld unsupported (128 or 256)",
                (long long)H);
    if (n == 0) return SGS_OK;
    SGS_REQUIRE(dvbits && dz && sd && codes && G && opart, SGS_EINVAL, "sgs_edge_score_bwd_dfeat_fused_packed: null pointer");
    SGS_REQUIRE(ws && ws_bytes >= sgs_edge_score_workspace_bytes(0, H, 0), SGS_EWORKSPACE, "sgs_edge_score_bwd_dfeat_fused_packed: workspace too small");
    return bwd_dfeat_fused_launch(dvbits, dz, sd, codes, n, H, fused_wp16(const_cast<void*>(ws), H), G, opart, static_cast<hipStream_t>(stream_));
}

int sgs_edge_score_bwd_dfeat_fused_bf16(const uint32_t* dvbits, const float* dz, const int32_t* sd, const float* codes, int64_t n, int64_t N,
                                        int64_t H, const float* W1, const float* w2, float p_drop, float* G, float* opart, void* ws, size_t ws_bytes,
                                        sgs_stream_t stream_) {
    hipStream_t stream = static_cast<hipStream_t>(stream_);
// ... 158 lines not shown
```

### sgs-gnn_amd/csrc/losses.hip

```cpp
#include <algorithm>
#include <atomic>

#include "sgs_common.h"

namespace sgs {
namespace {

constexpr int kT = 256;

__device__ __forceinline__ void lane_argmax(const float* __restrict__ row, int64_t C, int lane, float& best, int& bi) {
    if (lane >= C) return;
    best = row[lane];
    bi = lane;
    for (int64_t c = lane + 64; c < C; c += 64) {
        const float v = row[c];
        if (v > best) { best = v; bi = static_cast<int>(c); }
    }
}

__global__ void __launch_bounds__(kT) masked_correct(const float* __restrict__ logits, int64_t N, int64_t C,
                                                    const int64_t* __restrict__ y, const uint8_t* __restrict__ mask,
                                                    int* __restrict__ correct) {
    const int lane = threadIdx.x & 63;
    const int64_t i = (static_cast<int64_t>(blockIdx.x) * kT + threadIdx.x) >> 6;
    if (i >= N || !mask[i]) return;
    float best = -INFINITY;
    int bi = 0x7fffffff;
    lane_argmax(logits + i * C, C, lane, best, bi);
#pragma unroll
    for (int o = 32; o > 0; o >>= 1) {
        const float ov = __shfl_xor(best, o, 64);
        const int oi = __shfl_xor(bi, o, 64);
        if (oi != 0x7fffffff && (bi == 0x7fffffff || ov > best || (ov == best && oi < bi))) { best = ov; bi = oi; }
    }
    if (lane == 0) {
        atomicAdd(&correct[1], 1);
        if (static_cast<int64_t>(bi) == y[i]) atomicAdd(&correct[0], 1);
    }
}

__global__ void __launch_bounds__(1024) masked_correct_pair(const float* __restrict__ logits_a, const float* __restrict__ logits_b, int64_t N,
                                                           int64_t C, const int64_t* __restrict__ y, const uint8_t* __restrict__ mask,
                                                           int* __restrict__ correct) {
    __shared__ int red[2 * 16];
    const int lane = threadIdx.x & 63, wid = threadIdx.x >> 6;
    const int64_t i = static_cast<int64_t>(blockIdx.x) * 16 + wid;
    const float* __restrict__ logits = blockIdx.y ? logits_b : logits_a;
    int ok = 0, row = 0;
    if (i < N && mask[i]) {
        float best = -INFINITY;
        int bi = 0x7fffffff;
        lane_argmax(logits + i * C, C, lane, best, bi);
#pragma unroll
        for (int o = 32; o > 0; o >>= 1) {
            const float ov = __shfl_xor(best, o, 64);
            const int oi = __shfl_xor(bi, o, 64);
            if (oi != 0x7fffffff && (bi == 0x7fffffff || ov > best || (ov == best && oi < bi))) { best = ov; bi = oi; }
        }
        row = 1;
        ok = (static_cast<int64_t>(bi) == y[i]) ? 1 : 0;
    }
    if (lane == 0) { red[2 * wid] = ok; red[2 * wid + 1] = row; }
    __syncthreads();
    if (threadIdx.x == 0) {
        int a_ = 0, b_ = 0;
        for (int w = 0; w < 16; ++w) { a_ += red[2 * w]; b_ += red[2 * w + 1]; }
        int* out = correct + (blockIdx.y ? 2 : 0);
        if (b_) atomicAdd(&out[1], b_);
        if (a_) atomicAdd(&out[0], a_);
    }
}

__global__ void __launch_bounds__(1024) gate_counts_partial(const float* __restrict__ logits_a, const float* __restrict__ logits_b, int64_t N,
                                                           int64_t C, const int64_t* __restrict__ y, const uint8_t* __restrict__ mask,
                                                           int2* __restrict__ part) {
    __shared__ int red[2 * 16];
    const int lane = threadIdx.x & 63, wid = threadIdx.x >> 6;
    const int64_t i = static_cast<int64_t>(blockIdx.x) * 16 + wid;
    const float* __restrict__ logits = blockIdx.y ? logits_b : logits_a;
    int ok = 0, row = 0;
    if (i < N && mask[i]) {
        float best = -INFINITY;
        int bi = 0x7fffffff;
        lane_argmax(logits + i * C, C, lane, best, bi);
#pragma unroll
        for (int o = 32; o > 0; o >>= 1) {
            const float ov = __shfl_xor(best, o, 64);
            const int oi = __shfl_xor(bi, o, 64);
            if (oi != 0x7fffffff && (bi == 0x7fffffff || ov > best || (ov == best && oi < bi))) { best = ov; bi = oi; }
        }
        row = 1;
        ok = (static_cast<int64_t>(bi) == y[i]) ? 1 : 0;
    }
    if (lane == 0) { red[2 * wid] = ok; red[2 * wid + 1] = row; }
    __syncthreads();
    if (threadIdx.x == 0) {
        int a_ = 0, b_ = 0;
        for (int w = 0; w < 16; ++w) { a_ += red[2 * w]; b_ += red[2 * w + 1]; }
        part[static_cast<int64_t>(blockIdx.y) * gridDim.x + blockIdx.x] = make_int2(a_, b_);
    }
}
__global__ void __launch_bounds__(64) gate_counts_finish(const int2* __restrict__ part, int nblk, int* __restrict__ out,
                                                        const uint64_t* __restrict__ seq, int32_t* __restrict__ dst) {
    int a0 = 0, r0 = 0, a1 = 0, r1 = 0;
    for (int b = threadIdx.x; b < nblk; b += 64) {
        const int2 pa = part[b], pb = part[nblk + b];
        a0 += pa.x; r0 += pa.y; a1 += pb.x; r1 += pb.y;
    }
    a0 = wave_sum_int_all(a0); r0 = wave_sum_int_all(r0); a1 = wave_sum_int_all(a1); r1 = wave_sum_int_all(r1);
    if (threadIdx.x == 0) {
        out[0] = a0; out[1] = r0; out[2] = a1; out[3] = r1; out[4] = 0;
        if (dst) {
            __hip_atomic_store(dst + 0, a0, __ATOMIC_RELAXED, __HIP_MEMORY_SCOPE_SYSTEM);
            __hip_atomic_store(dst + 1, r0, __ATOMIC_RELAXED, __HIP_MEMORY_SCOPE_SYSTEM);
            __hip_atomic_store(dst + 2, a1, __ATOMIC_RELAXED, __HIP_MEMORY_SCOPE_SYSTEM);
            __hip_atomic_store(dst + 3, r1, __ATOMIC_RELAXED, __HIP_MEMORY_SCOPE_SYSTEM);
            __atomic_thread_fence(__ATOMIC_RELEASE);
            __hip_atomic_store(dst + 4, static_cast<int32_t>(seq ? seq[0] : 1), __ATOMIC_RELEASE, __HIP_MEMORY_SCOPE_SYSTEM);
        }
    }
}

__global__ void loss_tick(float* __restrict__ sum, const float* __restrict__ loss, uint64_t* __restrict__ epoch) {
    if (threadIdx.x == 0) {
        if (sum && loss) sum[0] += loss[0];
        if (epoch) epoch[0] += 1;
    }
}

__global__ void publish_words(const int32_t* __restrict__ src, int n, const uint64_t* __restrict__ seq, int32_t* dst) {
    if (threadIdx.x < n) __hip_atomic_store(dst + threadIdx.x, src[threadIdx.x], __ATOMIC_RELAXED, __HIP_MEMORY_SCOPE_SYSTEM);
    __syncthreads();
    if (threadIdx.x == 0) {
        __atomic_thread_fence(__ATOMIC_RELEASE);
        __hip_atomic_store(dst + n, static_cast<int32_t>(seq ? seq[0] : 1), __ATOMIC_RELEASE, __HIP_MEMORY_SCOPE_SYSTEM);
    }
}

__global__ void __launch_bounds__(kT) ce_rows(const float* __restrict__ logits, int64_t N, int64_t C, const int64_t* __restrict__ y,
                                             const uint8_t* __restrict__ mask, float* __restrict__ row_lse,
                                             float* __restrict__ rowloss) {
    const int lane = threadIdx.x & 63;
    const int64_t i = (static_cast<int64_t>(blockIdx.x) * kT + threadIdx.x) >> 6;
    if (i >= N) return;
    if (!mask[i]) {
        if (lane == 0) { rowloss[i] = 0.f; row_lse[i] = 0.f; }
        return;
    }
    float mx = -INFINITY;
    for (int64_t c = lane; c < C; c += 64) mx = fmaxf(mx, logits[i * C + c]);
    mx = wave_max_all(mx);
    float s = 0.f;
    for (int64_t c = lane; c < C; c += 64) s += expf(logits[i * C + c] - mx);
    s = wave_sum_all(s);
    const float lse = mx + logf(s);
    if (lane == 0) {
        row_lse[i] = lse;
        rowloss[i] = lse - logits[i * C + y[i]];
    }
}

__global__ void __launch_bounds__(1024) ce_final(const float* __restrict__ rowloss, const uint8_t* __restrict__ mask, int64_t N,
                                                float* __restrict__ loss, int* __restrict__ n_rows) {
    __shared__ float red[16];
    __shared__ int redi[16];
    float acc = 0.f;
    int cnt = 0;
    for (int64_t i = threadIdx.x; i < N; i += 1024) { acc += rowloss[i]; cnt += mask[i] ? 1 : 0; }
    const float r = block_sum(acc, red);
    cnt = wave_sum_int_all(cnt);
    if ((threadIdx.x & 63) == 0) redi[threadIdx.x >> 6] = cnt;
    __syncthreads();
    if (threadIdx.x == 0) {
        int n = 0;
        for (int w = 0; w < 16; ++w) n += redi[w];
        n_rows[0] = n;
        loss[0] = r / static_cast<float>(n);
    }
}

__global__ void __launch_bounds__(kT) ce_bwd(const float* __restrict__ logits, int64_t N, int64_t C, const int64_t* __restrict__ y,
                                            const uint8_t* __restrict__ mask, const float* __restrict__ row_lse,
                                            const int* __restrict__ n_rows, const float* __restrict__ grad_loss,
                                            float* __restrict__ dlogits) {
    const int64_t idx = static_cast<int64_t>(blockIdx.x) * kT + threadIdx.x;
    if (idx >= N * C) return;
    const int64_t i = idx / C, c = idx - i * C;
    float g = 0.f;
    if (mask[i]) {
        const float sm = expf(logits[idx] - row_lse[i]);
        g = (sm - (y[i] == c ? 1.f : 0.f)) * (grad_loss[0] / static_cast<float>(n_rows[0]));
    }
    dlogits[idx] = g;
}

struct EdgeTerms {
    float dot, nx, ny;
};
__device__ __forceinline__ EdgeTerms edge_dot(const float* __restrict__ x, const float* __restrict__ y, int64_t C) {
    EdgeTerms t{0.f, 0.f, 0.f};
    for (int64_t c = 0; c < C; ++c) {
        const float a = x[c], b = y[c];
        t.dot = fmaf(a, b, t.dot); t.nx = fmaf(a, a, t.nx); t.ny = fmaf(b, b, t.ny);
    }
    return t;
}
__device__ __forceinline__ float cos_from(const EdgeTerms& t) { return t.dot / sqrtf(fmaxf(t.nx * t.ny, 1e-16f)); }

constexpr int kRegRounds = 4;
constexpr int kRegEdges = kRegRounds * (kT / 16);
__global__ void __launch_bounds__(kT) reg_fwd_partial(const float* __restrict__ w, const int64_t* __restrict__ sei, int64_t q,
                                                     const float* __restrict__ logits, int64_t C, const int64_t* __restrict__ y,
                                                     const uint8_t* __restrict__ tm, float* __restrict__ cos_out,
                                                     float* __restrict__ part) {
    __shared__ float red[kT / 64];
    const int sub = threadIdx.x & 15, grp = threadIdx.x >> 4;
    float bce = 0.f, sq = 0.f, nv = 0.f, nl = 0.f;
#pragma unroll
    for (int r = 0; r < kRegRounds; ++r) {
        const int64_t j = static_cast<int64_t>(blockIdx.x) * kRegEdges + r * (kT / 16) + grp;
        const bool live = j < q;
        const int64_t jj = live ? j : 0;
        const int64_t s = sei[jj], d = sei[q + jj];
        const float* x = logits + s * C;
        const float* yv = logits + d * C;
        float dot = 0.f, nx = 0.f, ny = 0.f;
        for (int64_t c = sub; c < C; c += 16) {
            const float a = x[c], b = yv[c];
            dot = fmaf(a, b, dot); nx = fmaf(a, a, nx); ny = fmaf(b, b, ny);
        }
        dot = row16_sum_all_dpp(dot); nx = row16_sum_all_dpp(nx); ny = row16_sum_all_dpp(ny);
        if (live && sub == 0) {
            const float wj = w[j];
            const float cs = cos_from(EdgeTerms{dot, nx, ny});
            if (cos_out) cos_out[j] = cs;
            const float df = wj - cs;
            sq += df * df;
            if (tm[s] && tm[d]) {
                nv += 1.f;
                const bool same = y[s] == y[d];
                nl += same ? 1.f : 0.f;
                bce += same ? -fmaxf(logf(wj), -100.f) : -fmaxf(logf(1.f - wj), -100.f);
            }
        }
    }
    const float r0 = block_sum(bce, red);
    const float r1 = block_sum(sq, red);
    const float r2 = block_sum(nv, red);
    const float r3 = block_sum(nl, red);
    if (threadIdx.x == 0) {
        part[4 * blockIdx.x + 0] = r0; part[4 * blockIdx.x + 1] = r1;
        part[4 * blockIdx.x + 2] = r2; part[4 * blockIdx.x + 3] = r3;
    }
}

__global__ void __launch_bounds__(kT) reg_fwd_final(const float* __restrict__ part, int64_t nblk, int64_t q, float coef1, float coef2,
                                                   float* __restrict__ out) {
    __shared__ float red[kT / 64];
    float a0 = 0.f, a1 = 0.f, a2 = 0.f, a3 = 0.f;
    for (int64_t b = threadIdx.x; b < nblk; b += kT) {
        a0 += part[4 * b]; a1 += part[4 * b + 1]; a2 += part[4 * b + 2]; a3 += part[4 * b + 3];
    }
    const float r0 = block_sum(a0, red), r1 = block_sum(a1, red), r2 = block_sum(a2, red), r3 = block_sum(a3, red);
    if (threadIdx.x == 0) {
        const float reg1 = (r3 > 1.f) ? r0 / r2 : 0.f;
        const float reg2 = r1 / static_cast<float>(q);
        out[0] = reg1; out[1] = reg2; out[2] = r2; out[3] = r3;
        out[4] = coef1 * reg1 + coef2 * reg2;
    }
}

__global__ void __launch_bounds__(kT) hybrid_loss_final(const float* __restrict__ part, int64_t nblk, int64_t q, float coef1, float coef2,
                                                       const float* __restrict__ rowloss, const uint8_t* __restrict__ mask, int64_t N,
                                                       float* __restrict__ out, int* __restrict__ n_rows) {
    __shared__ float red[kT / 64];
    float a0 = 0.f, a1 = 0.f, a2 = 0.f, a3 = 0.f, ce = 0.f, cnt = 0.f;
    for (int64_t b = threadIdx.x; b < nblk; b += kT) {
        a0 += part[4 * b]; a1 += part[4 * b + 1]; a2 += part[4 * b + 2]; a3 += part[4 * b + 3];
    }
    for (int64_t i = threadIdx.x; i < N; i += kT) { ce += rowloss[i]; cnt += mask[i] ? 1.f : 0.f; }
    const float r0 = block_sum(a0, red), r1 = block_sum(a1, red), r2 = block_sum(a2, red), r3 = block_sum(a3, red);
    const float rc = block_sum(ce, red), rn = block_sum(cnt, red);
    if (threadIdx.x == 0) {
        const float reg1 = (r3 > 1.f) ? r0 / r2 : 0.f;
        const float reg2 = r1 / static_cast<float>(q);
        out[0] = reg1; out[1] = reg2; out[2] = r2; out[3] = r3;
        out[4] = coef1 * reg1 + coef2 * reg2;
        out[5] = rc / rn;
        out[6] = out[5] + out[4];
        n_rows[0] = static_cast<int>(rn);
    }
}

__global__ void __launch_bounds__(kT) ce_bwd_acc(const float* __restrict__ logits, int64_t N, int64_t C, const int64_t* __restrict__ y,
                                                const uint8_t* __restrict__ mask, const float* __restrict__ row_lse,
                                                const int* __restrict__ n_rows, const float* __restrict__ grad_loss,
                                                float* __restrict__ dlogits) {
    const int64_t idx = static_cast<int64_t>(blockIdx.x) * kT + threadIdx.x;
    if (idx >= N * C) return;
    const int64_t i = idx / C, c = idx - i * C;
    if (!mask[i]) return;
    const float sm = expf(logits[idx] - row_lse[i]);
    dlogits[idx] += (sm - (y[i] == c ? 1.f : 0.f)) * (grad_loss[0] / static_cast<float>(n_rows[0]));
}

__device__ __forceinline__ float class_weight(const float* __restrict__ weight, int64_t yi, int64_t C) {
    if (yi < 0 || yi >= C) return 0.f;
    return weight ? weight[yi] : 1.f;
}

__global__ void __launch_bounds__(kT) ce_rows_w(const float* __restrict__ logits, int64_t N, int64_t C, const int64_t* __restrict__ y,
                                               const uint8_t* __restrict__ mask, const float* __restrict__ weight, float eps,
                                               float* __restrict__ row_lse, float* __restrict__ rowloss) {
    const int lane = threadIdx.x & 63;
    const int64_t i = (static_cast<int64_t>(blockIdx.x) * kT + threadIdx.x) >> 6;
    if (i >= N) return;
    if (!mask[i]) {
        if (lane == 0) { rowloss[i] = 0.f; row_lse[i] = 0.f; }
        return;
    }
    float mx = -INFINITY;
    for (int64_t c = lane; c < C; c += 64) mx = fmaxf(mx, logits[i * C + c]);
    mx = wave_max_all(mx);
    float s = 0.f;
    for (int64_t c = lane; c < C; c += 64) s += expf(logits[i * C + c] - mx);
    s = wave_sum_all(s);
    const float lse = mx + logf(s);
    float sm = 0.f;
    if (eps != 0.f) {
        for (int64_t c = lane; c < C; c += 64) sm += (weight ? weight[c] : 1.f) * (lse - logits[i * C + c]);
        sm = wave_sum_all(sm);
    }
    if (lane == 0) {
        const int64_t yi = y[i];
        const float wy = class_weight(weight, yi, C);
        const float hard = (yi >= 0 && yi < C) ? wy * (lse - logits[i * C + yi]) : 0.f;
        row_lse[i] = lse;
        rowloss[i] = (eps != 0.f) ? (1.f - eps) * hard + (eps / static_cast<float>(C)) * sm : hard;
    }
}

__global__ void __launch_bounds__(1024) ce_final_w(const float* __restrict__ rowloss, const uint8_t* __restrict__ mask,
                                                  const int64_t* __restrict__ y, const float* __restrict__ weight, int64_t N, int64_t C,
                                                  float* __restrict__ loss, float* __restrict__ den) {
    __shared__ float red[16];
    float acc = 0.f, dn = 0.f;
    for (int64_t i = threadIdx.x; i < N; i += 1024) {
        acc += rowloss[i];
        if (mask[i]) dn += class_weight(weight, y[i], C);
    }
    const float r = block_sum(acc, red);
    const float d = block_sum(dn, red);
    if (threadIdx.x == 0) {
        den[0] = d;
        loss[0] = (d == 0.f) ? NAN : r / d;
    }
}

__device__ __forceinline__ float block_weight_sum(const float* __restrict__ weight, int64_t C, float* red) {
    float v = 0.f;
    for (int64_t c = threadIdx.x; c < C; c += kT) v += weight[c];
    v = wave_sum_all(v);
    if ((threadIdx.x & 63) == 0) red[threadIdx.x >> 6] = v;
    __syncthreads();
    float r = 0.f;
#pragma unroll
    for (int k = 0; k < kT / 64; ++k) r += red[k];
    return r;
}

__device__ __forceinline__ float ce_w_grad(float x, float lse, bool is_label, float wy, float wc, float W, float eps, float invC, float sc) {
    const float sm = expf(x - lse);
    const float hard = wy * (sm - (is_label ? 1.f : 0.f));
    if (eps == 0.f) return hard * sc;
    return ((1.f - eps) * hard + (eps * invC) * (W * sm - wc)) * sc;
}

template <bool kAcc>
__global__ void __launch_bounds__(kT) ce_bwd_w(const float* __restrict__ logits, int64_t N, int64_t C, const int64_t* __restrict__ y,
                                              const uint8_t* __restrict__ mask, const float* __restrict__ weight, float eps,
                                              const float* __restrict__ row_lse, const float* __restrict__ den,
                                              const float* __restrict__ grad_loss, float* __restrict__ dlogits) {
    __shared__ float red[kT / 64];
    float W = static_cast<float>(C);
    if (eps != 0.f && weight) W = block_weight_sum(weight, C, red);
    const int64_t idx = static_cast<int64_t>(blockIdx.x) * kT + threadIdx.x;
    if (idx >= N * C) return;
    const int64_t i = idx / C, c = idx - i * C;
    if (!mask[i]) {
        if (!kAcc) dlogits[idx] = 0.f;
        return;
    }
    const float d = den[0];
    const float sc = (d == 0.f) ? NAN : grad_loss[0] / d;
    const int64_t yi = y[i];
    const float g = ce_w_grad(logits[idx], row_lse[i], yi == c, class_weight(weight, yi, C), weight ? weight[c] : 1.f, W, eps,
                              1.f / static_cast<float>(C), sc);
    if (kAcc) dlogits[idx] += g;
    else dlogits[idx] = g;
}

__global__ void __launch_bounds__(kT) hybrid_loss_final_w(const float* __restrict__ part, int64_t nblk, int64_t q, float coef1, float coef2,
                                                         const float* __restrict__ rowloss, const uint8_t* __restrict__ mask,
                                                         const int64_t* __restrict__ y, const float* __restrict__ weight, int64_t N, int64_t C,
                                                         float* __restrict__ out, float* __restrict__ den) {
    __shared__ float red[kT / 64];
    float a0 = 0.f, a1 = 0.f, a2 = 0.f, a3 = 0.f, ce = 0.f, dn = 0.f;
    for (int64_t b = threadIdx.x; b < nblk; b += kT) {
        a0 += part[4 * b]; a1 += part[4 * b + 1]; a2 += part[4 * b + 2]; a3 += part[4 * b + 3];
    }
    for (int64_t i = threadIdx.x; i < N; i += kT) {
        ce += rowloss[i];
        if (mask[i]) dn += class_weight(weight, y[i], C);
    }
    const float r0 = block_sum(a0, red), r1 = block_sum(a1, red), r2 = block_sum(a2, red), r3 = block_sum(a3, red);
    const float rc = block_sum(ce, red), rd = block_sum(dn, red);
    if (threadIdx.x == 0) {
        const float reg1 = (r3 > 1.f) ? r0 / r2 : 0.f;
        const float reg2 = r1 / static_cast<float>(q);
        out[0] = reg1; out[1] = reg2; out[2] = r2; out[3] = r3;
        out[4] = coef1 * reg1 + coef2 * reg2;
        out[5] = (rd == 0.f) ? NAN : rc / rd;
        out[6] = out[5] + out[4];
        den[0] = rd;
    }
}

__global__ void __launch_bounds__(kT) reg_raw_final(const float* __restrict__ part, int64_t nblk, float* __restrict__ raw) {
    __shared__ float red[kT / 64];
    float a0 = 0.f, a1 = 0.f, a2 = 0.f, a3 = 0.f;
    for (int64_t b = threadIdx.x; b < nblk; b += kT) {
        a0 += part[4 * b]; a1 += part[4 * b + 1]; a2 += part[4 * b + 2]; a3 += part[4 * b + 3];
    }
    const float r0 = block_sum(a0, red), r1 = block_sum(a1, red), r2 = block_sum(a2, red), r3 = block_sum(a3, red);
    if (threadIdx.x == 0) { raw[0] = r0; raw[1] = r1; raw[2] = r2; raw[3] = r3; }
}

__global__ void __launch_bounds__(kT) reg_bwd_edges(const float* __restrict__ w, const int64_t* __restrict__ sei, int64_t q,
                                                   const float* __restrict__ logits, int64_t C, const int64_t* __restrict__ y,
                                                   const uint8_t* __restrict__ tm, const float* __restrict__ out, float coef1,
                                                   float coef2, float q_norm, const float* __restrict__ grad_loss,
                                                   float* __restrict__ dw, float* __restrict__ Gs, float* __restrict__ Gd) {
    const int sub = threadIdx.x & 15;
    const int64_t j = static_cast<int64_t>(blockIdx.x) * (kT / 16) + (threadIdx.x >> 4);
    const bool live = j < q;
    const int64_t jj = live ? j : 0;
    const float gl = grad_loss[0];
    const int64_t s = sei[jj], d = sei[q + jj];
    const float* x = logits + s * C;
    const float* yv = logits + d * C;
    float dot = 0.f, nx = 0.f, ny = 0.f;
    for (int64_t c = sub; c < C; c += 16) {
        const float a = x[c], b = yv[c];
        dot = fmaf(a, b, dot); nx = fmaf(a, a, nx); ny = fmaf(b, b, ny);
    }
    dot = row16_sum_all_dpp(dot); nx = row16_sum_all_dpp(nx); ny = row16_sum_all_dpp(ny);
    if (!live) return;
    const float den2 = fmaxf(nx * ny, 1e-16f);
    const float inv = 1.0f / sqrtf(den2);
    const float cs = dot * inv;
    const float wj = w[j];
    const float r = 2.0f * (wj - cs) / q_norm * coef2 * gl;
    if (sub == 0) {
        float g = r;
        if (coef1 != 0.f && out[3] > 1.f && tm[s] && tm[d]) {
            const float tgt = (y[s] == y[d]) ? 1.f : 0.f;
            g += coef1 * gl * (wj - tgt) / fmaxf((1.f - wj) * wj, 1e-12f) / out[2];
        }
        dw[j] = g;
    }
    const bool clamped = nx * ny < 1e-16f;
    const float cx = clamped ? 0.f : cs / nx, cy = clamped ? 0.f : cs / ny;
    for (int64_t c = sub; c < C; c += 16) {
        const float a = x[c], b = yv[c];
        Gs[j * C + c] = -r * (b * inv - cx * a);
        Gd[j * C + c] = -r * (a * inv - cy * b);
    }
}


__global__ void __launch_bounds__(kT) ensemble_mean_correct(const float* __restrict__ logits, int64_t xs, int Dc, int64_t N, int64_t C,
                                                           float* __restrict__ acc, int first, int last, int D_total, float inv,
                                                           const int64_t* __restrict__ y, const uint8_t* __restrict__ m0,
                                                           const uint8_t* __restrict__ m1, const uint8_t* __restrict__ m2,
                                                           unsigned long long* __restrict__ counts) {
    const int lane = threadIdx.x & 63;
    const int64_t i = (static_cast<int64_t>(blockIdx.x) * kT + threadIdx.x) >> 6;
    if (i >= N) return;
    float best = -INFINITY;
    int bi = 0x7fffffff;
    for (int64_t c = lane; c < C; c += 64) {
        float v = first ? logits[i * C + c] : acc[i * C + c];
        for (int d = first ? 1 : 0; d < Dc; ++d) v = __fadd_rn(v, logits[static_cast<int64_t>(d) * xs + i * C + c]);
        if (last && D_total > 1) v = __fmul_rn(v, inv);
        acc[i * C + c] = v;
        if (v > best || (v == best && static_cast<int>(c) < bi) || bi == 0x7fffffff) { best = v; bi = static_cast<int>(c); }
    }
    if (!last) return;
#pragma unroll
    for (int o = 32; o > 0; o >>= 1) {
        const float ov = __shfl_xor(best, o, 64);
        const int oi = __shfl_xor(bi, o, 64);
        if (oi != 0x7fffffff && (bi == 0x7fffffff || ov > best || (ov == best && oi < bi))) { best = ov; bi = oi; }
    }
    if (lane == 0) {
        const bool ok = static_cast<int64_t>(bi) == y[i];
        const uint8_t* ms[3] = {m0, m1, m2};
#pragma unroll
        for (int s = 0; s < 3; ++s)
            if (ms[s][i]) {
                atomicAdd(&counts[2 * s + 1], 1ull);
                if (ok) atomicAdd(&counts[2 * s], 1ull);
            }
    }
}

__device__ __forceinline__ int wave_row_argmax(const float* __restrict__ row, int64_t C, int lane) {
    float best = -INFINITY;
    int bi = 0x7fffffff;
    lane_argmax(row, C, lane, best, bi);
#pragma unroll
    for (int o = 32; o > 0; o >>= 1) {
        const float ov = __shfl_xor(best, o, 64);
        const int oi = __shfl_xor(bi, o, 64);
        if (oi != 0x7fffffff && (bi == 0x7fffffff || ov > best || (ov == best && oi < bi))) { best = ov; bi = oi; }
    }
    return bi;
}

__global__ void __launch_bounds__(kT) confusion_direct(const float* __restrict__ logits, int64_t N, int64_t C, const int64_t* __restrict__ y,
                                                      const uint8_t* __restrict__ m0, const uint8_t* __restrict__ m1,
                                                      const uint8_t* __restrict__ m2, unsigned long long* __restrict__ conf) {
    const int lane = threadIdx.x & 63;
    const int64_t i = (static_cast<int64_t>(blockIdx.x) * kT + threadIdx.x) >> 6;
    if (i >= N) return;
    const bool in0 = m0[i] != 0, in1 = m1[i] != 0, in2 = m2[i] != 0;
    if (!(in0 || in1 || in2)) return;
    const int bi = wave_row_argmax(logits + i * C, C, lane);
    if (lane != 0) return;
    const int64_t t = y[i];
    if (t < 0 || t >= C) return;
    const int64_t cell = t * C + bi;
    if (in0) atomicAdd(&conf[cell], 1ull);
    if (in1) atomicAdd(&conf[C * C + cell], 1ull);
    if (in2) atomicAdd(&conf[2 * C * C + cell], 1ull);
}

constexpr int kConfT = 1024;
__global__ void __launch_bounds__(kConfT) confusion_private(const float* __restrict__ logits, int64_t N, int64_t C, const int64_t* __restrict__ y,
                                                           const uint8_t* __restrict__ m0, const uint8_t* __restrict__ m1,
                                                           const uint8_t* __restrict__ m2, unsigned long long* __restrict__ conf) {
    extern __shared__ int hist[];
    const int cells = 3 * static_cast<int>(C * C);
    for (int k = threadIdx.x; k < cells; k += kConfT) hist[k] = 0;
    __syncthreads();
    const int lane = threadIdx.x & 63, wid = threadIdx.x >> 6;
    const int cc = static_cast<int>(C * C);
    for (int64_t i = static_cast<int64_t>(blockIdx.x) * (kConfT / 64) + wid; i < N; i += static_cast<int64_t>(gridDim.x) * (kConfT / 64)) {
        const bool in0 = m0[i] != 0, in1 = m1[i] != 0, in2 = m2[i] != 0;
        if (!(in0 || in1 || in2)) continue;
        const int bi = wave_row_argmax(logits + i * C, C, lane);
        if (lane != 0) continue;
        const int64_t t = y[i];
        if (t < 0 || t >= C) continue;
        const int cell = static_cast<int>(t * C) + bi;
        if (in0) atomicAdd(&hist[cell], 1);
        if (in1) atomicAdd(&hist[cc + cell], 1);
        if (in2) atomicAdd(&hist[2 * cc + cell], 1);
    }
    __syncthreads();
    for (int k = threadIdx.x; k < cells; k += kConfT) {
        const int v = hist[k];
        if (v) atomicAdd(&conf[k], static_cast<unsigned long long>(v));
    }
}

constexpr int64_t kConfPrivMaxC = 73;
constexpr int64_t kConfAutoMaxC = 12;
constexpr int64_t kConfAutoMinRows = 4096;
std::atomic<int> g_conf_variant{0};

}
}

using namespace sgs;

extern "C" {

int sgs_masked_correct(const float* logits, int64_t N, int64_t C, const int64_t* y, const uint8_t* train_mask,
                       int32_t* correct, sgs_stream_t stream_) {
    hipStream_t stream = static_cast<hipStream_t>(stream_);
    SGS_REQUIRE(N >= 0 && C > 0 && correct, SGS_EINVAL, "sgs_masked_correct: bad arguments");
    if (int rc = zero_async(correct, 8, stream)) return rc;
    if (N == 0) return SGS_OK;
    SGS_REQUIRE(logits && y && train_mask, SGS_EINVAL, "sgs_masked_correct: null pointer");
    hipLaunchKernelGGL(masked_correct, dim3(cdiv(N * 64, kT)), dim3(kT), 0, stream, logits, N, C, y, train_mask, correct);
    SGS_LAUNCH_OK();
    return SGS_OK;
}

int sgs_masked_correct_pair(const float* logits_a, const float* logits_b, int64_t N, int64_t C, const int64_t* y,
                            const uint8_t* train_mask, int32_t* correct4, sgs_stream_t stream_) {
    hipStream_t stream = static_cast<hipStream_t>(stream_);
    SGS_REQUIRE(N >= 0 && C > 0 && correct4, SGS_EINVAL, "sgs_masked_correct_pair: bad arguments");
    if (N == 0) return SGS_OK;
    SGS_REQUIRE(logits_a && logits_b && y && train_mask, SGS_EINVAL, "sgs_masked_correct_pair: null pointer");
    hipLaunchKernelGGL(masked_correct_pair, dim3(static_cast<unsigned>(cdiv(N, 16)), 2), dim3(1024), 0, stream, logits_a, logits_b, N, C, y, train_mask,
                       correct4);
    SGS_LAUNCH_OK();
    return SGS_OK;
}

size_t sgs_gate_counts_workspace_bytes(int64_t N) { return carve_bytes(static_cast<size_t>(2 * (cdiv(N < 0 ? 0 : N, 16) + 1)), 8) + 256; }

int sgs_gate_counts(const float* logits_a, const float* logits_b, int64_t N, int64_t C, const int64_t* y, const uint8_t* train_mask,
                    int32_t* out5, const uint64_t* seq_dev, int32_t* dst_host_mapped, void* ws, size_t ws_bytes, sgs_stream_t stream_) {
    hipStream_t stream = static_cast<hipStream_t>(stream_);
    SGS_REQUIRE(N >= 0 && N < (int64_t(1) << 30) && C > 0 && out5, SGS_EINVAL, "sgs_gate_counts: bad arguments");
    SGS_REQUIRE(N == 0 || (logits_a && logits_b && y && train_mask), SGS_EINVAL, "sgs_gate_counts: null pointer");
    SGS_REQUIRE(ws && ws_bytes >= sgs_gate_counts_workspace_bytes(N), SGS_EWORKSPACE, "sgs_gate_counts: workspace too small");
    Carver cv(ws);
    const int nblk = static_cast<int>(cdiv(N, 16));
    int2* part = reinterpret_cast<int2*>(cv.take<int64_t>(static_cast<size_t>(2 * (nblk + 1))));
    if (nblk > 0)
        hipLaunchKernelGGL(gate_counts_partial, dim3(static_cast<unsigned>(nblk), 2), dim3(1024), 0, stream, logits_a, logits_b, N, C, y, train_mask,
                           part);
    hipLaunchKernelGGL(gate_counts_finish, dim3(1), dim3(64), 0, stream, static_cast<const int2*>(part), nblk, out5, seq_dev, dst_host_mapped);
    SGS_LAUNCH_OK();
    return SGS_OK;
}

// ... 30 lines not shown
    SGS_REQUIRE(N > 0 && C > 0 && logits && y && train_mask && row_lse && n_rows && grad_loss && dlogits, SGS_EINVAL,
                "sgs_masked_ce_bwd: bad arguments");
    hipLaunchKernelGGL(ce_bwd, dim3(cdiv(N * C, kT)), dim3(kT), 0, stream, logits, N, C, y, train_mask, row_lse, n_rows, grad_loss,
                       dlogits);
    SGS_LAUNCH_OK();
    return SGS_OK;
}

size_t sgs_edge_reg_workspace_bytes(int64_t q) { return carve_bytes(4 * (cdiv(q < 0 ? 0 : q, kRegEdges) + 1), 4) + 256; }

int sgs_edge_reg_fwd(const float* w, const int64_t* sampled_edge_index, int64_t q, const float* logits, int64_t N, int64_t C,
                     const int64_t* y, const uint8_t* train_mask, float coef1, float coef2, float* out, float* cos_out,
                     void* ws, size_t ws_bytes, sgs_stream_t stream_) {
    hipStream_t stream = static_cast<hipStream_t>(stream_);
    SGS_REQUIRE(q > 0 && N > 0 && C > 0 && w && sampled_edge_index && logits && y && train_mask && out, SGS_EINVAL,
                "sgs_edge_reg_fwd: bad arguments");
    SGS_REQUIRE(ws && ws_bytes >= sgs_edge_reg_workspace_bytes(q), SGS_EWORKSPACE, "sgs_edge_reg_fwd: workspace too small");
    Carver cv(ws);
    const int64_t nblk = cdiv(q, kRegEdges);
    float* part = cv.take<float>(4 * (nblk + 1));
    hipLaunchKernelGGL(reg_fwd_partial, dim3(nblk), dim3(kT), 0, stream, w, sampled_edge_index, q, logits, C, y, train_mask, cos_out,
                       part);
    hipLaunchKernelGGL(reg_fwd_final, dim3(1), dim3(kT), 0, stream, part, nblk, q, coef1, coef2, out);
    SGS_LAUNCH_OK();
    return SGS_OK;
}

int sgs_hybrid_loss_fwd(const float* logits, int64_t N, int64_t C, const int64_t* y, const uint8_t* train_mask, const float* w,
                        const int64_t* sampled_edge_index, int64_t q, float coef1, float coef2, float* out, float* row_lse, float* rowloss,
                        int32_t* n_rows, void* ws, size_t ws_bytes, sgs_stream_t stream_) {
    hipStream_t stream = static_cast<hipStream_t>(stream_);
    SGS_REQUIRE(q > 0 && N > 0 && N < (int64_t(1) << 24) && C > 0 && logits && y && train_mask && w && sampled_edge_index && out && row_lse &&
                    rowloss && n_rows,
                SGS_EINVAL, "sgs_hybrid_loss_fwd: bad arguments");
    SGS_REQUIRE(ws && ws_bytes >= sgs_edge_reg_workspace_bytes(q), SGS_EWORKSPACE, "sgs_hybrid_loss_fwd: workspace too small");
    Carver cv(ws);
    const int64_t nblk = cdiv(q, kRegEdges);
    float* part = cv.take<float>(4 * (nblk + 1));
    hipLaunchKernelGGL(ce_rows, dim3(cdiv(N * 64, kT)), dim3(kT), 0, stream, logits, N, C, y, train_mask, row_lse, rowloss);
    hipLaunchKernelGGL(reg_fwd_partial, dim3(nblk), dim3(kT), 0, stream, w, sampled_edge_index, q, logits, C, y, train_mask,
                       static_cast<float*>(nullptr), part);
    hipLaunchKernelGGL(hybrid_loss_final, dim3(1), dim3(kT), 0, stream, part, nblk, q, coef1, coef2, rowloss, train_mask, N, out, n_rows);
    SGS_LAUNCH_OK();
    return SGS_OK;
}

int sgs_masked_ce_bwd_acc(const float* logits, int64_t N, int64_t C, const int64_t* y, const uint8_t* train_mask, const float* row_lse,
                          const int32_t* n_rows, const float* grad_loss, float* dlogits, sgs_stream_t stream_) {
    hipStream_t stream = static_cast<hipStream_t>(stream_);
    SGS_REQUIRE(N > 0 && C > 0 && logits && y && train_mask && row_lse && n_rows && grad_loss && dlogits, SGS_EINVAL,
                "sgs_masked_ce_bwd_acc: bad arguments");
    hipLaunchKernelGGL(ce_bwd_acc, dim3(cdiv(N * C, kT)), dim3(kT), 0, stream, logits, N, C, y, train_mask, row_lse, n_rows, grad_loss,
                       dlogits);
    SGS_LAUNCH_OK();
    return SGS_OK;
}

int sgs_masked_ce_w_fwd(const float* logits, int64_t N, int64_t C, const int64_t* y, const uint8_t* train_mask, const float* weight,
                        float label_smoothing, float* loss, float* row_lse, float* rowloss, float* den, sgs_stream_t stream_) {
    hipStream_t stream = static_cast<hipStream_t>(stream_);
    SGS_REQUIRE(N > 0 && N < (int64_t(1) << 24) && C > 0 && logits && y && train_mask && loss && row_lse && rowloss, SGS_EINVAL,
                "sgs_masked_ce_w_fwd: bad arguments");
    SGS_REQUIRE(label_smoothing >= 0.f && label_smoothing <= 1.f, SGS_EINVAL, "sgs_masked_ce_w_fwd: label_smoothing outside [0, 1]");
    SGS_REQUIRE(den, SGS_EINVAL, "sgs_masked_ce_w_fwd: den is NULL");
    hipLaunchKernelGGL(ce_rows_w, dim3(cdiv(N * 64, kT)), dim3(kT), 0, stream, logits, N, C, y, train_mask, weight, label_smoothing, row_lse,
                       rowloss);
    hipLaunchKernelGGL(ce_final_w, dim3(1), dim3(1024), 0, stream, rowloss, train_mask, y, weight, N, C, loss, den);
    SGS_LAUNCH_OK();
    return SGS_OK;
}

int sgs_masked_ce_w_bwd(const float* logits, int64_t N, int64_t C, const int64_t* y, const uint8_t* train_mask, const float* weight,
                        float label_smoothing, const float* row_lse, const float* den, const float* grad_loss, float* dlogits,
                        sgs_stream_t stream_) {
    hipStream_t stream = static_cast<hipStream_t>(stream_);
    SGS_REQUIRE(N > 0 && C > 0 && logits && y && train_mask && row_lse && grad_loss && dlogits, SGS_EINVAL, "sgs_masked_ce_w_bwd: bad arguments");
    SGS_REQUIRE(label_smoothing >= 0.f && label_smoothing <= 1.f, SGS_EINVAL, "sgs_masked_ce_w_bwd: label_smoothing outside [0, 1]");
    SGS_REQUIRE(den, SGS_EINVAL, "sgs_masked_ce_w_bwd: den is NULL");
    hipLaunchKernelGGL(ce_bwd_w<false>, dim3(cdiv(N * C, kT)), dim3(kT), 0, stream, logits, N, C, y, train_mask, weight, label_smoothing,
                       row_lse, den, grad_loss, dlogits);
    SGS_LAUNCH_OK();
    return SGS_OK;
}

int sgs_masked_ce_w_bwd_acc(const float* logits, int64_t N, int64_t C, const int64_t* y, const uint8_t* train_mask, const float* weight,
                            float label_smoothing, const float* row_lse, const float* den, const float* grad_loss, float* dlogits,
                            sgs_stream_t stream_) {
    hipStream_t stream = static_cast<hipStream_t>(stream_);
    SGS_REQUIRE(N > 0 && C > 0 && logits && y && train_mask && row_lse && grad_loss && dlogits, SGS_EINVAL,
                "sgs_masked_ce_w_bwd_acc: bad arguments");
    SGS_REQUIRE(label_smoothing >= 0.f && label_smoothing <= 1.f, SGS_EINVAL, "sgs_masked_ce_w_bwd_acc: label_smoothing outside [0, 1]");
    SGS_REQUIRE(den, SGS_EINVAL, "sgs_masked_ce_w_bwd_acc: den is NULL");
    hipLaunchKernelGGL(ce_bwd_w<true>, dim3(cdiv(N * C, kT)), dim3(kT), 0, stream, logits, N, C, y, train_mask, weight, label_smoothing,
                       row_lse, den, grad_loss, dlogits);
    SGS_LAUNCH_OK();
    return SGS_OK;
}

int sgs_hybrid_loss_w_fwd(const float* logits, int64_t N, int64_t C, const int64_t* y, const uint8_t* train_mask, const float* w,
                          const int64_t* sampled_edge_index, int64_t q, float coef1, float coef2, const float* weight, float label_smoothing,
                          float* out, float* row_lse, float* rowloss, float* den, void* ws, size_t ws_bytes, sgs_stream_t stream_) {
    hipStream_t stream = static_cast<hipStream_t>(stream_);
    SGS_REQUIRE(q > 0 && N > 0 && N < (int64_t(1) << 24) && C > 0 && logits && y && train_mask && w && sampled_edge_index && out && row_lse &&
                    rowloss,
                SGS_EINVAL, "sgs_hybrid_loss_w_fwd: bad arguments");
    SGS_REQUIRE(label_smoothing >= 0.f && label_smoothing <= 1.f, SGS_EINVAL, "sgs_hybrid_loss_w_fwd: label_smoothing outside [0, 1]");
    SGS_REQUIRE(den, SGS_EINVAL, "sgs_hybrid_loss_w_fwd: den is NULL");
    SGS_REQUIRE(ws && ws_bytes >= sgs_edge_reg_workspace_bytes(q), SGS_EWORKSPACE, "sgs_hybrid_loss_w_fwd: workspace too small");
    Carver cv(ws);
    const int64_t nblk = cdiv(q, kRegEdges);
    float* part = cv.take<float>(4 * (nblk + 1));
    hipLaunchKernelGGL(ce_rows_w, dim3(cdiv(N * 64, kT)), dim3(kT), 0, stream, logits, N, C, y, train_mask, weight, label_smoothing, row_lse,
                       rowloss);
    hipLaunchKernelGGL(reg_fwd_partial, dim3(nblk), dim3(kT), 0, stream, w, sampled_edge_index, q, logits, C, y, train_mask,
                       static_cast<float*>(nullptr), part);
    hipLaunchKernelGGL(hybrid_loss_final_w, dim3(1), dim3(kT), 0, stream, part, nblk, q, coef1, coef2, rowloss, train_mask, y, weight, N, C, out,
                       den);
    SGS_LAUNCH_OK();
    return SGS_OK;
}

int sgs_edge_reg_partial(const float* w, const int64_t* sampled_edge_index, int64_t q, const float* logits, int64_t N, int64_t C,
                         const int64_t* y, const uint8_t* train_mask, float* raw, void* ws, size_t ws_bytes, sgs_stream_t stream_) {
    hipStream_t stream = static_cast<hipStream_t>(stream_);
    SGS_REQUIRE(q >= 0 && N > 0 && C > 0 && raw, SGS_EINVAL, "sgs_edge_reg_partial: bad arguments");
    SGS_REQUIRE(ws && ws_bytes >= sgs_edge_reg_workspace_bytes(q), SGS_EWORKSPACE, "sgs_edge_reg_partial: workspace too small");
    Carver cv(ws);
    const int64_t nblk = cdiv(q, kRegEdges);
    float* part = cv.take<float>(4 * (nblk + 1));
    if (q > 0) {
        SGS_REQUIRE(w && sampled_edge_index && logits && y && train_mask, SGS_EINVAL, "sgs_edge_reg_partial: null pointer");
        hipLaunchKernelGGL(reg_fwd_partial, dim3(nblk), dim3(kT), 0, stream, w, sampled_edge_index, q, logits, C, y, train_mask,
                           static_cast<float*>(nullptr), part);
    }
    hipLaunchKernelGGL(reg_raw_final, dim3(1), dim3(kT), 0, stream, part, nblk, raw);
    SGS_LAUNCH_OK();
    return SGS_OK;
}

int sgs_edge_reg_bwd(const float* w, const int64_t* sampled_edge_index, int64_t q, int64_t q_global, const float* logits, int64_t N,
                     int64_t C, const int64_t* y, const uint8_t* train_mask, const float* out, float coef1, float coef2,
                     const float* grad_loss, float* dw, float* Gs, float* Gd, sgs_stream_t stream_) {
    hipStream_t stream = static_cast<hipStream_t>(stream_);
    SGS_REQUIRE(q >= 0 && q_global >= q && N > 0 && C > 0, SGS_EINVAL, "sgs_edge_reg_bwd: bad arguments");
    if (q == 0) return SGS_OK;
    SGS_REQUIRE(w && sampled_edge_index && logits && y && train_mask && out && grad_loss && dw && Gs && Gd, SGS_EINVAL,
                "sgs_edge_reg_bwd: null pointer");
    hipLaunchKernelGGL(reg_bwd_edges, dim3(cdiv(q, kT / 16)), dim3(kT), 0, stream, w, sampled_edge_index, q, logits, C, y, train_mask, out,
                       coef1, coef2, static_cast<float>(q_global), grad_loss, dw, Gs, Gd);
    SGS_LAUNCH_OK();
    return SGS_OK;
}

int sgs_ensemble_mean_correct(const float* logits, int64_t x_stride, int64_t Dc, int64_t N, int64_t C, float* acc, int first, int last,
                              int64_t D_total, const int64_t* y, const uint8_t* mask0, const uint8_t* mask1, const uint8_t* mask2, int64_t* counts,
                              sgs_stream_t stream_) {
    hipStream_t stream = static_cast<hipStream_t>(stream_);
    SGS_REQUIRE(Dc >= 1 && N >= 0 && C > 0 && D_total >= Dc && x_stride >= 0 && (Dc == 1 || x_stride == 0 || x_stride >= N * C), SGS_EINVAL,
                "sgs_ensemble_mean_correct: bad sizes");
    if (N == 0) return SGS_OK;
    SGS_REQUIRE(logits && acc && (!last || (y && mask0 && mask1 && mask2 && counts)), SGS_EINVAL, "sgs_ensemble_mean_correct: null pointer");
    const float inv = 1.0f / static_cast<float>(D_total);
    hipLaunchKernelGGL(ensemble_mean_correct, dim3(cdiv(N * 64, kT)), dim3(kT), 0, stream, logits, x_stride, static_cast<int>(Dc), N, C, acc,
                       first, last, static_cast<int>(D_total), inv, y, mask0, mask1, mask2, reinterpret_cast<unsigned long long*>(counts));
    SGS_LAUNCH_OK();
    return SGS_OK;
}

int sgs_confusion_variant_set(int code) {
    SGS_REQUIRE(code >= 0 && code <= 2, SGS_EINVAL, "sgs_confusion_variant_set: code %d, need 0 (automatic), 1 (direct) or 2 (privatised)", code);
    g_conf_variant.store(code);
    return SGS_OK;
}

int sgs_confusion_variant(int64_t N, int64_t C) {
    if (N < 0 || C < 1) return -1;
    if (N == 0) return 0;
    const bool priv_ok = C <= kConfPrivMaxC && N < (int64_t(1) << 31);
    switch (g_conf_variant.load()) {
        case 1: return 1;
        case 2: return priv_ok ? 2 : -1;
        default: return priv_ok && C <= kConfAutoMaxC && N >= kConfAutoMinRows ? 2 : 1;
    }
}

int sgs_confusion_counts(const float* logits, int64_t N, int64_t C, const int64_t* y, const uint8_t* m0, const uint8_t* m1, const uint8_t* m2,
                         int64_t* conf, sgs_stream_t stream_) {
    hipStream_t stream = static_cast<hipStream_t>(stream_);
    SGS_REQUIRE(N >= 0 && N < (int64_t(1) << 32) && C >= 1 && C < (int64_t(1) << 24) && conf, SGS_EINVAL, "sgs_confusion_counts: bad arguments");
    if (N == 0) return SGS_OK;
    SGS_REQUIRE(logits && y && m0 && m1 && m2, SGS_EINVAL, "sgs_confusion_counts: null pointer");
    const int var = sgs_confusion_variant(N, C);
    SGS_REQUIRE(var > 0, SGS_EINVAL, "sgs_confusion_counts: the privatised form (forced by sgs_confusion_variant_set(2)) needs C <= 73 and N < 2^31");
    unsigned long long* out = reinterpret_cast<unsigned long long*>(conf);
    if (var == 1) {
        hipLaunchKernelGGL(confusion_direct, dim3(cdiv(N * 64, kT)), dim3(kT), 0, stream, logits, N, C, y, m0, m1, m2, out);
    } else {
        static const int cus = [] {
            int dev = 0, n = 0;
            if (hipGetDevice(&dev) != hipSuccess || hipDeviceGetAttribute(&n, hipDeviceAttributeMultiprocessorCount, dev) != hipSuccess || n < 1) n = 256;
            return n;
        }();
        const int64_t grid = std::min<int64_t>(cdiv(N, kConfT / 64), cus);
        hipLaunchKernelGGL(confusion_private, dim3(static_cast<unsigned>(grid)), dim3(kConfT), static_cast<size_t>(12 * C * C), stream, logits, N, C, y,
                           m0, m1, m2, out);
    }
    SGS_LAUNCH_OK();
    return SGS_OK;
}

}
```

### sgs-gnn_amd/ops.py

```python
from __future__ import annotations

import ctypes
import os

import numpy as np
import torch

from . import _lib

SAMPLE_LEARNED, SAMPLE_PRIOR = 0, 1
ACT_NONE, ACT_RELU, ACT_RELU_DROPOUT = 0, 1, 2

_workspaces = {}
_retired_workspaces = []
_pin_workspaces = False


def _need_gpu(*tensors):
    for t in tensors:
        if t is not None and not t.is_cuda:
            raise RuntimeError("sgs_gnn_amd: the SGS hot path runs only on a HIP device (got a CPU tensor); "
                               "there is no CPU fallback")


# ... 1115 lines not shown
    _lib.check(L.sgs_loss_tick(_ptr(loss_sum, torch.float32), _ptr(loss.detach().reshape(1), torch.float32), epoch.data_ptr(), _stream()),
               "sgs_loss_tick")


def publish_to_host(src, n, seq, dst_pinned) -> None:
    L = _lib.lib()
    _need_gpu(src, seq)
    if dst_pinned.is_cuda or not dst_pinned.is_pinned() or dst_pinned.dtype != torch.int32 or dst_pinned.numel() < n + 1:
        raise RuntimeError("publish_to_host: destination must be a pinned host int32 tensor with n + 1 entries")
    _lib.check(L.sgs_publish_to_host(_ptr(src, torch.int32), n, None if seq is None else seq.data_ptr(), dst_pinned.data_ptr(), _stream()),
               "sgs_publish_to_host")


class _MaskedCE(torch.autograd.Function):
    @staticmethod
    def forward(ctx, logits, y, mask_u8):
        L = _lib.lib()
        N, C = logits.shape
        dev = logits.device
        loss = torch.empty(1, dtype=torch.float32, device=dev)
        row_lse = torch.empty(N, dtype=torch.float32, device=dev)
        rowloss = torch.empty(N, dtype=torch.float32, device=dev)
        n_rows = torch.empty(1, dtype=torch.int32, device=dev)
        _lib.check(L.sgs_masked_ce_fwd(_ptr(logits), N, C, _ptr(y), _ptr(mask_u8), _ptr(loss), _ptr(row_lse), _ptr(rowloss),
                                       _ptr(n_rows), _stream()), "sgs_masked_ce_fwd")
        ctx.save_for_backward(logits, y, mask_u8, row_lse, n_rows)
        return loss.reshape(())

    @staticmethod
    def backward(ctx, g):
        L = _lib.lib()
        logits, y, mask_u8, row_lse, n_rows = ctx.saved_tensors
        N, C = logits.shape
        g = g.reshape(1).contiguous().float()
        d = torch.empty_like(logits)
        _lib.check(L.sgs_masked_ce_bwd(_ptr(logits), N, C, _ptr(y), _ptr(mask_u8), _ptr(row_lse), _ptr(n_rows), _ptr(g), _ptr(d),
                                       _stream()), "sgs_masked_ce_bwd")
        return d, None, None


def check_ce_spec(logits, weight, label_smoothing):
    eps = float(label_smoothing)
    if not 0.0 <= eps <= 1.0:
        raise ValueError(f"sgs_gnn_amd: label_smoothing must lie in [0, 1], got {label_smoothing!r}")
    if weight is None:
        return None, eps
    if not torch.is_tensor(weight):
        raise ValueError(f"sgs_gnn_amd: class weight must be a tensor, got {type(weight).__name__}")
    C = logits.shape[-1]
    if weight.dtype != torch.float32:
        raise ValueError(f"sgs_gnn_amd: class weight must be float32, got dtype {weight.dtype}")
    if weight.dim() != 1 or weight.numel() != C:
        raise ValueError(f"sgs_gnn_amd: class weight must have length C = {C}, got shape {tuple(weight.shape)}")
    if weight.device != logits.device:
        raise ValueError(f"sgs_gnn_amd: class weight is on device {weight.device}, the logits on {logits.device}")
    if not weight.is_contiguous():
        raise ValueError("sgs_gnn_amd: class weight must be contiguous")
    return weight.detach(), eps


class _MaskedCEW(torch.autograd.Function):

    @staticmethod
    def forward(ctx, logits, y, mask_u8, weight, eps):
        L = _lib.lib()
        N, C = logits.shape
        dev = logits.device
        loss = torch.empty(1, dtype=torch.float32, device=dev)
        row_lse = torch.empty(N, dtype=torch.float32, device=dev)
        rowloss = torch.empty(N, dtype=torch.float32, device=dev)
        den = torch.empty(1, dtype=torch.float32, device=dev)
        _lib.check(L.sgs_masked_ce_w_fwd(_ptr(logits), N, C, _ptr(y), _ptr(mask_u8), _ptr(weight), eps, _ptr(loss), _ptr(row_lse), _ptr(rowloss),
                                         _ptr(den), _stream()), "sgs_masked_ce_w_fwd")
        ctx.save_for_backward(logits, y, mask_u8, weight, row_lse, den)
        ctx.eps = eps
        return loss.reshape(())

    @staticmethod
    def backward(ctx, g):
        L = _lib.lib()
        logits, y, mask_u8, weight, row_lse, den = ctx.saved_tensors
        N, C = logits.shape
        g = g.reshape(1).contiguous().float()
        d = torch.empty_like(logits)
        _lib.check(L.sgs_masked_ce_w_bwd(_ptr(logits), N, C, _ptr(y), _ptr(mask_u8), _ptr(weight), ctx.eps, _ptr(row_lse), _ptr(den), _ptr(g),
                                         _ptr(d), _stream()), "sgs_masked_ce_w_bwd")
        return d, None, None, None, None


def masked_cross_entropy(logits, y, train_mask, *, weight=None, label_smoothing=0.0):
    if weight is None and label_smoothing == 0.0:
        _need_gpu(logits, y, train_mask)
        return _MaskedCE.apply(logits.contiguous(), y.contiguous(), _u8(train_mask))
    weight, eps = check_ce_spec(logits, weight, label_smoothing)
    _need_gpu(logits, y, train_mask)
    return _MaskedCEW.apply(logits.contiguous(), y.contiguous(), _u8(train_mask), weight, eps)


class _EdgeReg(torch.autograd.Function):
    @staticmethod
    def forward(ctx, w, logits, sei, y, mask_u8, graph, coef1, coef2, box):
        L = _lib.lib()
        q = w.numel()
        N, C = logits.shape
        dev = w.device
        out = torch.empty(5, dtype=torch.float32, device=dev)
        ws = workspace(L.sgs_edge_reg_workspace_bytes(q), dev)
        _lib.check(L.sgs_edge_reg_fwd(_ptr(w), _ptr(sei), q, _ptr(logits), N, C, _ptr(y), _ptr(mask_u8), float(coef1), float(coef2),
                                      _ptr(out), None, ws.data_ptr(), ws.numel(), _stream()), "sgs_edge_reg_fwd")
        ctx.save_for_backward(w, logits, sei, y, mask_u8, out)
        ctx.graph, ctx.coef1, ctx.coef2 = graph, float(coef1), float(coef2)
        box.append(out)
        return out[4]

    @staticmethod
    def backward(ctx, g):
        L = _lib.lib()
        w, logits, sei, y, mask_u8, out = ctx.saved_tensors
        q = w.numel()
        N, C = logits.shape
        dev = w.device
        g = g.reshape(1).contiguous().float()
        dw = torch.empty(q, dtype=torch.float32, device=dev)
        Gs = torch.empty(q, C, dtype=torch.float32, device=dev)
        Gd = torch.empty(q, C, dtype=torch.float32, device=dev)
        _lib.check(L.sgs_edge_reg_bwd(_ptr(w), _ptr(sei), q, q, _ptr(logits), N, C, _ptr(y), _ptr(mask_u8), _ptr(out), ctx.coef1,
                                      ctx.coef2, _ptr(g), _ptr(dw), _ptr(Gs), _ptr(Gd), _stream()), "sgs_edge_reg_bwd")
        dlogits = _endpoint_reduce(Gs, Gd, None, ctx.graph, 1.0, 1.0, C) if ctx.coef2 != 0.0 else None
        return dw, dlogits, None, None, None, None, None, None, None


def edge_regularizers(w, logits, sampled_edge_index, y, train_mask, coef1, coef2):
    _need_gpu(w, logits, sampled_edge_index, y, train_mask)
    graph = get_graph(sampled_edge_index, logits.shape[0])
    box = []
    total = _EdgeReg.apply(w.contiguous(), logits.contiguous(), sampled_edge_index.contiguous(), y.contiguous(),
                           _u8(train_mask), graph, float(coef1), float(coef2), box)
    return total, box[0]


class _HybridLoss(torch.autograd.Function):

    @staticmethod
    def forward(ctx, logits, y, mask_u8, w, sei, graph, coef1, coef2, box, weight=None, eps=0.0):
        L = _lib.lib()
        q = w.numel()
        N, C = logits.shape
        dev = w.device
        out = torch.empty(7, dtype=torch.float32, device=dev)
        row_lse = torch.empty(N, dtype=torch.float32, device=dev)
        rowloss = torch.empty(N, dtype=torch.float32, device=dev)
        ws = workspace(L.sgs_edge_reg_workspace_bytes(q), dev)
        ctx.plain = weight is None and eps == 0.0
        if ctx.plain:
            n_rows = torch.empty(1, dtype=torch.int32, device=dev)
            _lib.check(L.sgs_hybrid_loss_fwd(_ptr(logits), N, C, _ptr(y), _ptr(mask_u8), _ptr(w), _ptr(sei), q, float(coef1), float(coef2), _ptr(out),
                                             _ptr(row_lse), _ptr(rowloss), _ptr(n_rows), ws.data_ptr(), ws.numel(), _stream()), "sgs_hybrid_loss_fwd")
        else:
            n_rows = torch.empty(1, dtype=torch.float32, device=dev)
            _lib.check(L.sgs_hybrid_loss_w_fwd(_ptr(logits), N, C, _ptr(y), _ptr(mask_u8), _ptr(w), _ptr(sei), q, float(coef1), float(coef2),
                                               _ptr(weight), eps, _ptr(out), _ptr(row_lse), _ptr(rowloss), _ptr(n_rows), ws.data_ptr(), ws.numel(),
                                               _stream()), "sgs_hybrid_loss_w_fwd")
        ctx.save_for_backward(logits, y, mask_u8, w, sei, out, row_lse, n_rows, weight)
        ctx.eps = eps
        ctx.graph, ctx.coef1, ctx.coef2 = graph, float(coef1), float(coef2)
        ctx.nm_ref = getattr(w, "_sgs_norm", None)
        box.append(out)
        return out[6]

    @staticmethod
    def backward(ctx, g):
        L = _lib.lib()
        logits, y, mask_u8, w, sei, out, row_lse, n_rows, weight = ctx.saved_tensors
        q = w.numel()
        N, C = logits.shape
        dev = w.device
        g = g.reshape(1).contiguous().float()
        dw = torch.empty(q, dtype=torch.float32, device=dev)
        Gs = torch.empty(q, C, dtype=torch.float32, device=dev)
        Gd = torch.empty(q, C, dtype=torch.float32, device=dev)
        _lib.check(L.sgs_edge_reg_bwd(_ptr(w), _ptr(sei), q, q, _ptr(logits), N, C, _ptr(y), _ptr(mask_u8), _ptr(out), ctx.coef1,
                                      ctx.coef2, _ptr(g), _ptr(dw), _ptr(Gs), _ptr(Gd), _stream()), "sgs_edge_reg_bwd")
        dlogits = _endpoint_reduce(Gs, Gd, None, ctx.graph, 1.0, 1.0, C) if ctx.coef2 != 0.0 else torch.empty_like(logits)
        if not ctx.plain:
            fn, what = (L.sgs_masked_ce_w_bwd_acc, "sgs_masked_ce_w_bwd_acc") if ctx.coef2 != 0.0 else (L.sgs_masked_ce_w_bwd, "sgs_masked_ce_w_bwd")
            _lib.check(fn(_ptr(logits), N, C, _ptr(y), _ptr(mask_u8), _ptr(weight), ctx.eps, _ptr(row_lse), _ptr(n_rows), _ptr(g), _ptr(dlogits),
                          _stream()), what)
        elif ctx.coef2 != 0.0:
            _lib.check(L.sgs_masked_ce_bwd_acc(_ptr(logits), N, C, _ptr(y), _ptr(mask_u8), _ptr(row_lse), _ptr(n_rows), _ptr(g), _ptr(dlogits),
                                               _stream()), "sgs_masked_ce_bwd_acc")
        else:
            _lib.check(L.sgs_masked_ce_bwd(_ptr(logits), N, C, _ptr(y), _ptr(mask_u8), _ptr(row_lse), _ptr(n_rows), _ptr(g), _ptr(dlogits),
                                           _stream()), "sgs_masked_ce_bwd")
        nm = ctx.nm_ref() if ctx.nm_ref is not None else None
        if nm is not None and getattr(nm, "_park_ok", False) and dw.numel() == nm.graph.n_edges:
            import weakref
            nm._dw_first = weakref.ref(dw)
        return dlogits, None, None, dw, None, None, None, None, None, None, None


def hybrid_loss(logits, y, train_mask, w, sampled_edge_index, coef1, coef2, *, weight=None, label_smoothing=0.0):
    eps = 0.0
    if weight is not None or label_smoothing != 0.0:
        weight, eps = check_ce_spec(logits, weight, label_smoothing)
    _need_gpu(w, logits, sampled_edge_index, y, train_mask)
    graph = get_graph(sampled_edge_index, logits.shape[0])
    box = []
    total = _HybridLoss.apply(logits.contiguous(), y.contiguous(), _u8(train_mask), w.contiguous(), sampled_edge_index.contiguous(), graph,
                              float(coef1), float(coef2), box, weight, eps)
    return total, box[0]


class _GATAggregate(torch.autograd.Function):

    @staticmethod
    def forward(ctx, xl, a_s, a_d, bias, graph, slope, p_att, seed_att, site_att, act, p_act, seed_act, site_act):
        L = _lib.lib()
        N, D = xl.shape
        n = graph.n_edges
        dev = xl.device
        f32 = dict(dtype=torch.float32, device=dev)
        soft_in, alpha_in = torch.empty(max(n, 1), **f32), torch.empty(max(n, 1), **f32)
        soft_loop, alpha_loop = torch.empty(N, **f32), torch.empty(N, **f32)
        _lib.check(L.sgs_gat_alpha_fwd(_ptr(a_s), _ptr(a_d), N, n, _ptr(graph.in_ptr), _ptr(graph.in_src), _ptr(graph.in_eid),
                                       float(slope), float(p_att), seed_att, site_att, _ptr(soft_in), _ptr(soft_loop),
                                       _ptr(alpha_in), _ptr(alpha_loop), _stream()), "sgs_gat_alpha_fwd")
        Y = _spmm(xl, graph.in_ptr, graph.in_src, alpha_in, alpha_loop, bias, act, p_act, seed_act, site_act, N, D, n)
        ctx.save_for_backward(xl, a_s, a_d, soft_in, soft_loop, alpha_in, alpha_loop, Y if act != ACT_NONE else None)
        ctx.graph, ctx.slope, ctx.p_att, ctx.seed_att, ctx.site_att = graph, float(slope), float(p_att), seed_att, site_att
        ctx.act, ctx.p_act, ctx.has_bias = act, float(p_act), bias is not None
        return Y

    @staticmethod
    def backward(ctx, dY):
        L = _lib.lib()
        xl, a_s, a_d, soft_in, soft_loop, alpha_in, alpha_loop, Y = ctx.saved_tensors
        gr = ctx.graph
        N, D = xl.shape
        n = gr.n_edges
        dev = xl.device
        f32 = dict(dtype=torch.float32, device=dev)
        dY = dY.contiguous()
        dbias = None
        if ctx.act != ACT_NONE and ctx.has_bias:
            dZ, dbias = _act_bwd_colsum(dY, Y, ctx.act, ctx.p_act)
        elif ctx.act != ACT_NONE:
            dZ = torch.empty_like(dY)
            _lib.check(L.sgs_act_bwd(_ptr(dY), _ptr(Y), dY.numel(), ctx.act, ctx.p_act, _ptr(dZ), _stream()), "sgs_act_bwd")
        else:
            dZ = dY
            dbias = _colsum(dZ) if ctx.has_bias else None
        by_eid = torch.empty(max(n, 1), **f32)
        alpha_out = torch.empty(max(n, 1), **f32)
        _lib.check(L.sgs_scatter_by_eid(_ptr(alpha_in), _ptr(gr.in_eid), n, _ptr(by_eid), _stream()), "sgs_scatter_by_eid")
        _lib.check(L.sgs_gather_by_eid(_ptr(by_eid), _ptr(gr.out_eid), n, _ptr(alpha_out), _stream()), "sgs_gather_by_eid")
        dxl = _spmm(dZ, gr.out_ptr, gr.out_dst, alpha_out, alpha_loop, None, ACT_NONE, 0.0, 0, 0, N, D, n)
        galpha, gloop = torch.empty(max(n, 1), **f32), torch.empty(N, **f32)
        _lib.check(L.sgs_sddmm_csr(_ptr(dZ), _ptr(xl), N, D, n, _ptr(gr.in_ptr), _ptr(gr.in_src), _ptr(gr.in_eid), _ptr(galpha),
                                   _ptr(gloop), _stream()), "sgs_sddmm_csr")
        g_edge, g_self, d_ad = torch.empty(max(n, 1), **f32), torch.empty(N, **f32), torch.empty(N, **f32)
        _lib.check(L.sgs_gat_alpha_bwd(_ptr(a_s), _ptr(a_d), N, n, _ptr(gr.in_ptr), _ptr(gr.in_src), _ptr(gr.in_eid), ctx.slope,
                                       ctx.p_att, ctx.seed_att, ctx.site_att, _ptr(soft_in), _ptr(soft_loop), _ptr(galpha),
                                       _ptr(gloop), _ptr(g_edge), _ptr(g_self), _ptr(d_ad), _stream()), "sgs_gat_alpha_bwd")
        g_out = torch.empty(max(n, 1), **f32)
        _lib.check(L.sgs_gather_by_eid(_ptr(g_edge), _ptr(gr.out_eid), n, _ptr(g_out), _stream()), "sgs_gather_by_eid")
        ones = torch.ones(N, 1, **f32)
        d_as = _spmm(ones, gr.out_ptr, gr.out_dst, g_out, g_self, None, ACT_NONE, 0.0, 0, 0, N, 1, n).reshape(N)
        return dxl, d_as, d_ad, dbias, None, None, None, None, None, None, None, None, None


class _GATScores(torch.autograd.Function):

    @staticmethod
    def forward(ctx, xl, att_s, att_d):
        L = _lib.lib()
        N, D = xl.shape
        a_s, a_d = torch.empty(N, dtype=torch.float32, device=xl.device), torch.empty(N, dtype=torch.float32, device=xl.device)
        _lib.check(L.sgs_gat_scores_fwd(_ptr(xl, torch.float32), N, D, _ptr(att_s), _ptr(att_d), _ptr(a_s), _ptr(a_d), _stream()), "sgs_gat_scores_fwd")
        ctx.save_for_backward(xl, att_s, att_d)
        return a_s, a_d

    @staticmethod
    def backward(ctx, g_s, g_d):
        L = _lib.lib()
        xl, att_s, att_d = ctx.saved_tensors
        N, D = xl.shape
        dev = xl.device
        g_s = torch.zeros(N, dtype=torch.float32, device=dev) if g_s is None else g_s.contiguous()
        g_d = torch.zeros(N, dtype=torch.float32, device=dev) if g_d is None else g_d.contiguous()
        dxl = torch.empty_like(xl)
        das, dad = torch.empty(D, dtype=torch.float32, device=dev), torch.empty(D, dtype=torch.float32, device=dev)
        ws = workspace(L.sgs_gat_scores_bwd_workspace_bytes(N, D), dev)
        _lib.check(L.sgs_gat_scores_bwd(_ptr(xl), N, D, _ptr(att_s), _ptr(att_d), _ptr(g_s), _ptr(g_d), 0, _ptr(dxl), _ptr(das), _ptr(dad), ws.data_ptr(),
                                        ws.numel(), _stream()), "sgs_gat_scores_bwd")
        return dxl, das, dad


HEADS_CONCAT, HEADS_MEAN, HEADS_BROADCAST = 0, 1, 2


def gat_heads_supported(heads: int, channels: int) -> bool:
    return bool(_lib.lib().sgs_gat_heads_supported(int(heads), int(channels)))


def _spmm_heads(X, ptr, col, eid, val, diag, mode, bias, act, p, seed, site, N, K, C, nnz):
    L = _lib.lib()
    Y = torch.empty(N, C if mode == HEADS_MEAN else K * C, dtype=torch.float32, device=X.device)
    _lib.check(L.sgs_spmm_csr_heads(_ptr(X, torch.float32), N, K, C, nnz, _ptr(ptr), _ptr(col), _ptr(eid), _ptr(val), _ptr(diag), mode, _ptr(bias),
                                    act, float(p), seed, site, _ptr(Y), _stream()), "sgs_spmm_csr_heads")
    return Y


class _GATAggregateHeads(torch.autograd.Function):

    @staticmethod
    def forward(ctx, xl, a_s, a_d, bias, graph, K, concat, slope, p_att, seed_att, site_att, act, p_act, seed_act, site_act):
        L = _lib.lib()
        N, D = xl.shape
        C = D // K
        n = graph.n_edges
        f32 = dict(dtype=torch.float32, device=xl.device)
        soft, alpha = torch.empty(max(n, 1), K, **f32), torch.empty(max(n, 1), K, **f32)
        soft_loop, alpha_loop = torch.empty(N, K, **f32), torch.empty(N, K, **f32)
        _lib.check(L.sgs_gat_alpha_heads_fwd(_ptr(a_s), _ptr(a_d), N, K, n, _ptr(graph.in_ptr), _ptr(graph.in_src), _ptr(graph.in_eid),
                                             float(slope), float(p_att), seed_att, site_att, _ptr(soft), _ptr(soft_loop), _ptr(alpha),
                                             _ptr(alpha_loop), _stream()), "sgs_gat_alpha_heads_fwd")
        Y = _spmm_heads(xl, graph.in_ptr, graph.in_src, graph.in_eid, alpha, alpha_loop, HEADS_CONCAT if concat else HEADS_MEAN, bias, act,
                        p_act, seed_act, site_act, N, K, C, n)
        ctx.save_for_backward(xl, a_s, a_d, soft, soft_loop, alpha, alpha_loop, Y if act != ACT_NONE else None)
        ctx.graph, ctx.slope, ctx.p_att, ctx.seed_att, ctx.site_att = graph, float(slope), float(p_att), seed_att, site_att
        ctx.act, ctx.p_act, ctx.has_bias, ctx.K, ctx.concat = act, float(p_act), bias is not None, K, bool(concat)
        return Y

    @staticmethod
    def backward(ctx, dY):
        L = _lib.lib()
        xl, a_s, a_d, soft, soft_loop, alpha, alpha_loop, Y = ctx.saved_tensors
        gr, K = ctx.graph, ctx.K
        N, D = xl.shape
        C = D // K
        n = gr.n_edges
        f32 = dict(dtype=torch.float32, device=xl.device)
        dY = dY.contiguous()
        dbias = None
        if ctx.act != ACT_NONE and ctx.has_bias:
            dZ, dbias = _act_bwd_colsum(dY, Y, ctx.act, ctx.p_act)
# ... 1353 lines not shown
```

Baseline: 107.8 million.

## Fuse hybrid loss edge-regularizer backward with endpoint reduction and CE backward

```diff
diff --git a/include/sgs_hip.h b/include/sgs_hip.h
--- a/include/sgs_hip.h
+++ b/include/sgs_hip.h
@@ -347,6 +347,16 @@
 int sgs_hybrid_loss_w_fwd(const float* logits, int64_t N, int64_t C, const int64_t* y, const uint8_t* train_mask, const float* w,
                           const int64_t* sampled_edge_index, int64_t q, float coef1, float coef2, const float* weight, float label_smoothing,
                           float* out, float* row_lse, float* rowloss, float* den, void* ws, size_t ws_bytes, sgs_stream_t stream);
+
+int sgs_hybrid_loss_fused_fwd(const float* logits, int64_t N, int64_t C, const int64_t* y, const uint8_t* train_mask, const float* w,
+                              const int64_t* sampled_edge_index, int64_t q, float coef1, float coef2, int weighted, const float* weight,
+                              float label_smoothing, float* out, float* row_lse, float* rowloss, void* norm, float* stash, void* ws,
+                              size_t ws_bytes, sgs_stream_t stream);
+int sgs_hybrid_loss_fused_bwd(const float* logits, int64_t N, int64_t C, const int64_t* y, const uint8_t* train_mask, const float* w, int64_t q,
+                              const float* stash, const float* out, float coef1, int weighted, const float* weight, float label_smoothing,
+                              const float* row_lse, const void* norm, const float* grad_loss, const int32_t* in_ptr, const int32_t* in_src,
+                              const int32_t* in_eid, const int32_t* out_ptr, const int32_t* out_dst, const int32_t* out_eid, float* dw,
+                              float* dlogits, sgs_stream_t stream);
 
 int sgs_edge_reg_partial(const float* w, const int64_t* sampled_edge_index, int64_t q, const float* logits, int64_t N,
                          int64_t C, const int64_t* y, const uint8_t* train_mask, float* raw, void* ws, size_t ws_bytes,
diff --git a/sgs-gnn_amd/csrc/edge_score.hip b/sgs-gnn_amd/csrc/edge_score.hip
--- a/sgs-gnn_amd/csrc/edge_score.hip
+++ b/sgs-gnn_amd/csrc/edge_score.hip
@@ -1,6 +1,7 @@
 #include <type_traits>
 
 #include "sgs_common.h"
+#include "endpoint_reduce.h"
 
 namespace sgs {
 namespace {
@@ -1674,108 +1675,6 @@
     p_out[r] = 1.0f / (1.0f + expf(-z));
 }
 
-template <int VEC, bool HAS_T>
-__global__ void __launch_bounds__(kT) endpoint_reduce(const float* __restrict__ Mo, const float* __restrict__ Mi,
-                                                     const float* __restrict__ T, int64_t N, int64_t H,
-                                                     const int* __restrict__ in_ptr, const int* __restrict__ in_src,
-                                                     const int* __restrict__ in_eid, const int* __restrict__ out_ptr,
-                                                     const int* __restrict__ out_dst, const int* __restrict__ out_eid,
-                                                     float sgn_out, float sgn_in, float* __restrict__ out) {
-    const int lane = threadIdx.x & 63;
-    const int64_t v = (static_cast<int64_t>(blockIdx.x) * kT + threadIdx.x) >> 6;
-    if (v >= N) return;
-    for (int64_t c0 = static_cast<int64_t>(lane) * VEC; c0 < H; c0 += 64 * VEC) {
-        float acc[VEC];
-#pragma unroll
-        for (int j = 0; j < VEC; ++j) acc[j] = 0.f;
-        for (int dir = 0; dir < 2; ++dir) {
-            const int* ptr = dir == 0 ? out_ptr : in_ptr;
-            const int* col = dir == 0 ? out_dst : in_src;
-            const int* eid = dir == 0 ? out_eid : in_eid;
-            const float sg = dir == 0 ? sgn_out : sgn_in;
-            const float* M = dir == 0 ? Mo : Mi;
-            const int b = ptr[v], e = ptr[v + 1];
-            for (int k = b; k < e; ++k) {
-                float m[VEC], t[VEC];
-                if (VEC == 4) {
-                    *reinterpret_cast<float4*>(m) = *reinterpret_cast<const float4*>(M + static_cast<int64_t>(eid[k]) * H + c0);
-                    if (HAS_T) *reinterpret_cast<float4*>(t) = *reinterpret_cast<const float4*>(T + static_cast<int64_t>(col[k]) * H + c0);
-                } else {
-                    m[0] = M[static_cast<int64_t>(eid[k]) * H + c0];
-                    if (HAS_T) t[0] = T[static_cast<int64_t>(col[k]) * H + c0];
-                }
-#pragma unroll
-                for (int j = 0; j < VEC; ++j) acc[j] = fmaf(sg * m[j], HAS_T ? t[j] : 1.0f, acc[j]);
-            }
-        }
-        if (VEC == 4) *reinterpret_cast<float4*>(out + v * H + c0) = *reinterpret_cast<float4*>(acc);
-        else out[v * H + c0] = acc[0];
-    }
-}
-
-template <int VEC, bool HAS_T, int NW>
-__global__ void __launch_bounds__(64 * NW) endpoint_reduce_rowblock(const float* __restrict__ Mo, const float* __restrict__ Mi,
-                                                              const float* __restrict__ T, int64_t N, int64_t H,
-                                                              const int* __restrict__ in_ptr, const int* __restrict__ in_src,
-                                                              const int* __restrict__ in_eid, const int* __restrict__ out_ptr,
-                                                              const int* __restrict__ out_dst, const int* __restrict__ out_eid,
-                                                              float sgn_out, float sgn_in, float* __restrict__ out) {
-    using V = typename std::conditional<VEC == 4, float4, float>::type;
-    __shared__ float part[NW][64 * VEC];
-    const int lane = threadIdx.x & 63, wave = threadIdx.x >> 6;
-    const int64_t v = blockIdx.x;
-    const int ob = out_ptr[v], no = out_ptr[v + 1] - ob;
-    const int ib = in_ptr[v], ni = in_ptr[v + 1] - ib;
-    const int total = no + ni;
-    for (int64_t cbase = 0; cbase < H; cbase += 64 * VEC) {
-        const int64_t c0 = cbase + static_cast<int64_t>(lane) * VEC;
-        float acc[VEC];
-#pragma unroll
-        for (int j = 0; j < VEC; ++j) acc[j] = 0.f;
-        if (c0 < H) {
-            for (int k0 = wave; k0 < total; k0 += 4 * NW) {
-                float m[4][VEC], t[4][VEC], sg[4];
-                int er[4], cr[4];
-                const float* Mp[4];
-#pragma unroll
-                for (int u = 0; u < 4; ++u) {
-                    const int k = k0 + NW * u;
-                    const int kc = k < total ? k : total - 1;
-                    const bool isout = kc < no;
-                    const int idx = isout ? ob + kc : ib + (kc - no);
-                    er[u] = (isout ? out_eid : in_eid)[idx];
-                    if (HAS_T) cr[u] = (isout ? out_dst : in_src)[idx];
-                    Mp[u] = isout ? Mo : Mi;
-                    sg[u] = k < total ? (isout ? sgn_out : sgn_in) : 0.f;
-                }
-#pragma unroll
-                for (int u = 0; u < 4; ++u) {
-                    *reinterpret_cast<V*>(m[u]) = *reinterpret_cast<const V*>(Mp[u] + static_cast<int64_t>(er[u]) * H + c0);
-                    if (HAS_T) *reinterpret_cast<V*>(t[u]) = *reinterpret_cast<const V*>(T + static_cast<int64_t>(cr[u]) * H + c0);
-                    else {
-#pragma unroll
-                        for (int j = 0; j < VEC; ++j) t[u][j] = 1.f;
-                    }
-                }
-#pragma unroll
-                for (int u = 0; u < 4; ++u)
-#pragma unroll
-                    for (int j = 0; j < VEC; ++j) acc[j] = fmaf(sg[u] * m[u][j], t[u][j], acc[j]);
-            }
-        }
-#pragma unroll
-        for (int j = 0; j < VEC; ++j) part[wave][lane * VEC + j] = acc[j];
-        __syncthreads();
-        const int tt = threadIdx.x;
-        if (tt < 64 * VEC && cbase + tt < H) {
-            float sum = 0.f;
-#pragma unroll
-            for (int g = 0; g < NW; g += 4) sum += (part[g][tt] + part[g + 1][tt]) + (part[g + 2][tt] + part[g + 3][tt]);
-            out[v * H + cbase + tt] = sum;
-        }
-        __syncthreads();
-    }
-}
 
 __global__ void __launch_bounds__(kT) scorer_bwd_prep(const float* __restrict__ codes, int64_t H, const int64_t* __restrict__ src,
                                                      const int64_t* __restrict__ dst, const int64_t* __restrict__ active, int64_t n,
@@ -2610,31 +2509,20 @@
     const bool v4 = H % 4 == 0 && (reinterpret_cast<uintptr_t>(M_out) & 15) == 0 && (reinterpret_cast<uintptr_t>(M_in) & 15) == 0 &&
                     (reinterpret_cast<uintptr_t>(out) & 15) == 0 &&
                     (!T || (reinterpret_cast<uintptr_t>(T) & 15) == 0);
-    const dim3 blk(kT);
-    if (nnz >= 8 * N) {
-        const dim3 grid(static_cast<unsigned>(N));
-        const bool wide = nnz >= 64 * N;
-#define SGS_EPR(VEC_, HT_)                                                                                                   \
-        do {                                                                                                                    \
-            if (wide) hipLaunchKernelGGL((endpoint_reduce_rowblock<VEC_, HT_, 16>), grid, dim3(1024), 0, stream, M_out, M_in, T, N, H, in_ptr, \
-                                         in_src, in_eid, out_ptr, out_dst, out_eid, sign_out, sign_in, out);                  \
-            else      hipLaunchKernelGGL((endpoint_reduce_rowblock<VEC_, HT_, 4>), grid, blk, 0, stream, M_out, M_in, T, N, H, in_ptr,        \
-                                         in_src, in_eid, out_ptr, out_dst, out_eid, sign_out, sign_in, out);                  \
-        } while (0)
-        if (v4) { if (T) SGS_EPR(4, true); else SGS_EPR(4, false); }
-        else    { if (T) SGS_EPR(1, true); else SGS_EPR(1, false); }
+    const int nw = ep_traversal(nnz, N);
+#define SGS_EPR(VEC_, HT_)                                                                                                                        \
+    do {                                                                                                                                          \
+        const EpLoadRows<VEC_, HT_> rows{M_out, M_in, T};                                                                                         \
+        if (nw == 16)     hipLaunchKernelGGL((endpoint_reduce_rowblock<VEC_, 16, EpLoadRows<VEC_, HT_>>), dim3(static_cast<unsigned>(N)), dim3(1024), 0, stream, \
+                                             rows, N, H, in_ptr, in_src, in_eid, out_ptr, out_dst, out_eid, sign_out, sign_in, out);              \
+        else if (nw == 4) hipLaunchKernelGGL((endpoint_reduce_rowblock<VEC_, 4, EpLoadRows<VEC_, HT_>>), dim3(static_cast<unsigned>(N)), dim3(256), 0, stream,   \
+                                             rows, N, H, in_ptr, in_src, in_eid, out_ptr, out_dst, out_eid, sign_out, sign_in, out);              \
+        else              hipLaunchKernelGGL((endpoint_reduce<VEC_, EpLoadRows<VEC_, HT_>>), dim3(static_cast<unsigned>(cdiv(N * 64, kEpT))), dim3(kEpT), 0,     \
+                                             stream, rows, N, H, in_ptr, in_src, in_eid, out_ptr, out_dst, out_eid, sign_out, sign_in, out);      \
+    } while (0)
+    if (v4) { if (T) SGS_EPR(4, true); else SGS_EPR(4, false); }
+    else    { if (T) SGS_EPR(1, true); else SGS_EPR(1, false); }
 #undef SGS_EPR
-        SGS_LAUNCH_OK();
-        return SGS_OK;
-    }
-    const dim3 grid(static_cast<unsigned>(cdiv(N * 64, kT)));
-    if (v4) {
-        if (T) hipLaunchKernelGGL((endpoint_reduce<4, true>), grid, blk, 0, stream, M_out, M_in, T, N, H, in_ptr, in_src, in_eid, out_ptr, out_dst, out_eid, sign_out, sign_in, out);
-        else   hipLaunchKernelGGL((endpoint_reduce<4, false>), grid, blk, 0, stream, M_out, M_in, T, N, H, in_ptr, in_src, in_eid, out_ptr, out_dst, out_eid, sign_out, sign_in, out);
-    } else {
-        if (T) hipLaunchKernelGGL((endpoint_reduce<1, true>), grid, blk, 0, stream, M_out, M_in, T, N, H, in_ptr, in_src, in_eid, out_ptr, out_dst, out_eid, sign_out, sign_in, out);
-        else   hipLaunchKernelGGL((endpoint_reduce<1, false>), grid, blk, 0, stream, M_out, M_in, T, N, H, in_ptr, in_src, in_eid, out_ptr, out_dst, out_eid, sign_out, sign_in, out);
-    }
     SGS_LAUNCH_OK();
     return SGS_OK;
 }
diff --git a/sgs-gnn_amd/csrc/endpoint_reduce.h b/sgs-gnn_amd/csrc/endpoint_reduce.h
--- /dev/null
+++ b/sgs-gnn_amd/csrc/endpoint_reduce.h
@@ -0,0 +1,158 @@
+#pragma once
+#include <type_traits>
+
+#include "sgs_common.h"
+
+namespace sgs {
+namespace {
+
+constexpr int kEpT = 256;
+
+inline int ep_traversal(int64_t nnz, int64_t N) { return nnz >= 64 * N ? 16 : (nnz >= 8 * N ? 4 : 0); }
+
+template <int VEC, bool HAS_T>
+struct EpLoadRows {
+    static constexpr bool kCol = HAS_T, kVisit = false;
+    using V = typename std::conditional<VEC == 4, float4, float>::type;
+    const float* __restrict__ Mo;
+    const float* __restrict__ Mi;
+    const float* __restrict__ T;
+    struct Blk {};
+    struct Own {};
+    struct Pre {};
+    struct Raw { float m[VEC], t[VEC]; };
+    __device__ __forceinline__ Blk block_init() const { return Blk{}; }
+    __device__ __forceinline__ Own own(int64_t, int64_t, int64_t) const { return Own{}; }
+    __device__ __forceinline__ Pre preload(int, int) const { return Pre{}; }
+    __device__ __forceinline__ Raw load(const Pre&, int, bool isout, int e, int col, int64_t H, int64_t c0) const {
+        Raw r;
+        *reinterpret_cast<V*>(r.m) = *reinterpret_cast<const V*>((isout ? Mo : Mi) + static_cast<int64_t>(e) * H + c0);
+        if (HAS_T) *reinterpret_cast<V*>(r.t) = *reinterpret_cast<const V*>(T + static_cast<int64_t>(col) * H + c0);
+        else {
+#pragma unroll
+            for (int j = 0; j < VEC; ++j) r.t[j] = 1.f;
+        }
+        return r;
+    }
+    __device__ __forceinline__ void term(const Blk&, const Raw& r, const Own&, bool, float (&m)[VEC], float (&t)[VEC]) const {
+#pragma unroll
+        for (int j = 0; j < VEC; ++j) { m[j] = r.m[j]; t[j] = r.t[j]; }
+    }
+    __device__ __forceinline__ void visit(const Blk&, int64_t, int, int) const {}
+    __device__ __forceinline__ float finish(const Blk&, int64_t, int64_t, float sum) const { return sum; }
+};
+
+template <int VEC, class P>
+__global__ void __launch_bounds__(kEpT) endpoint_reduce(const P p, int64_t N, int64_t H, const int* __restrict__ in_ptr,
+                                                       const int* __restrict__ in_src, const int* __restrict__ in_eid,
+                                                       const int* __restrict__ out_ptr, const int* __restrict__ out_dst,
+                                                       const int* __restrict__ out_eid, float sgn_out, float sgn_in, float* __restrict__ out) {
+    const typename P::Blk blk = p.block_init();
+    const int lane = threadIdx.x & 63;
+    const int64_t v = (static_cast<int64_t>(blockIdx.x) * kEpT + threadIdx.x) >> 6;
+    if (v >= N) return;
+    if (P::kVisit)
+        for (int k = out_ptr[v] + lane; k < out_ptr[v + 1]; k += 64) p.visit(blk, v, out_eid[k], out_dst[k]);
+    for (int64_t cbase = 0; cbase < H; cbase += 64 * VEC) {
+        const int64_t c0 = cbase + static_cast<int64_t>(lane) * VEC;
+        const int64_t cl = c0 < H ? c0 : cbase;
+        float acc[VEC];
+#pragma unroll
+        for (int j = 0; j < VEC; ++j) acc[j] = 0.f;
+        const typename P::Own own = p.own(v, H, cl);
+        for (int dir = 0; dir < 2; ++dir) {
+            const int* ptr = dir == 0 ? out_ptr : in_ptr;
+            const int* col = dir == 0 ? out_dst : in_src;
+            const int* eid = dir == 0 ? out_eid : in_eid;
+            const float sg = dir == 0 ? sgn_out : sgn_in;
+            const int b = ptr[v], e = ptr[v + 1];
+            for (int k = b; k < e; ++k) {
+                const int ek = eid[k], ck = P::kCol ? col[k] : 0;
+                const typename P::Pre pre = p.preload(ek, lane);
+                const typename P::Raw raw = p.load(pre, 0, dir == 0, ek, ck, H, cl);
+                float m[VEC], t[VEC];
+                p.term(blk, raw, own, dir == 0, m, t);
+#pragma unroll
+                for (int j = 0; j < VEC; ++j) acc[j] = fmaf(sg * m[j], t[j], acc[j]);
+            }
+        }
+        if (c0 < H) {
+#pragma unroll
+            for (int j = 0; j < VEC; ++j) acc[j] = p.finish(blk, v, c0 + j, acc[j]);
+            if (VEC == 4) *reinterpret_cast<float4*>(out + v * H + c0) = *reinterpret_cast<float4*>(acc);
+            else out[v * H + c0] = acc[0];
+        }
+    }
+}
+
+template <int VEC, int NW, class P>
+__global__ void __launch_bounds__(64 * NW) endpoint_reduce_rowblock(const P p, int64_t N, int64_t H, const int* __restrict__ in_ptr,
+                                                                   const int* __restrict__ in_src, const int* __restrict__ in_eid,
+                                                                   const int* __restrict__ out_ptr, const int* __restrict__ out_dst,
+                                                                   const int* __restrict__ out_eid, float sgn_out, float sgn_in,
+                                                                   float* __restrict__ out) {
+    __shared__ float part[NW][64 * VEC];
+    const typename P::Blk blk = p.block_init();
+    const int lane = threadIdx.x & 63;
+    const int wave = __builtin_amdgcn_readfirstlane(threadIdx.x >> 6);
+    const int64_t v = blockIdx.x;
+    const int ob = out_ptr[v], no = out_ptr[v + 1] - ob;
+    const int ib = in_ptr[v], ni = in_ptr[v + 1] - ib;
+    const int total = no + ni;
+    if (P::kVisit)
+        for (int k = threadIdx.x; k < no; k += 64 * NW) p.visit(blk, v, out_eid[ob + k], out_dst[ob + k]);
+    for (int64_t cbase = 0; cbase < H; cbase += 64 * VEC) {
+        const int64_t c0 = cbase + static_cast<int64_t>(lane) * VEC;
+        const int64_t cl = c0 < H ? c0 : cbase;
+        float acc[VEC];
+#pragma unroll
+        for (int j = 0; j < VEC; ++j) acc[j] = 0.f;
+        const typename P::Own own = p.own(v, H, cl);
+        for (int k0 = wave; k0 < total; k0 += 4 * NW) {
+            float sg[4];
+            int er[4], cr[4];
+            bool io[4];
+            typename P::Raw raw[4];
+            const int kl = k0 + NW * (lane & 3);
+            const int kcl = kl < total ? kl : total - 1;
+            const bool iol = kcl < no;
+            const int idl = iol ? ob + kcl : ib + (kcl - no);
+            const int el = (iol ? out_eid : in_eid)[idl];
+            const int cll = P::kCol ? (iol ? out_dst : in_src)[idl] : 0;
+            const typename P::Pre pre = p.preload(el, lane);
+#pragma unroll
+            for (int u = 0; u < 4; ++u) {
+                const int k = k0 + NW * u;
+                const int kc = k < total ? k : total - 1;
+                const bool isout = kc < no;
+                er[u] = __builtin_amdgcn_readlane(el, u);
+                cr[u] = P::kCol ? __builtin_amdgcn_readlane(cll, u) : 0;
+                io[u] = isout;
+                sg[u] = k < total ? (isout ? sgn_out : sgn_in) : 0.f;
+            }
+#pragma unroll
+            for (int u = 0; u < 4; ++u) raw[u] = p.load(pre, u, io[u], er[u], cr[u], H, cl);
+#pragma unroll
+            for (int u = 0; u < 4; ++u) {
+                float m[VEC], t[VEC];
+                p.term(blk, raw[u], own, io[u], m, t);
+#pragma unroll
+                for (int j = 0; j < VEC; ++j) acc[j] = fmaf(sg[u] * m[j], t[j], acc[j]);
+            }
+        }
+#pragma unroll
+        for (int j = 0; j < VEC; ++j) part[wave][lane * VEC + j] = acc[j];
+        __syncthreads();
+        const int tt = threadIdx.x;
+        if (tt < 64 * VEC && cbase + tt < H) {
+            float sum = 0.f;
+#pragma unroll
+            for (int g = 0; g < NW; g += 4) sum += (part[g][tt] + part[g + 1][tt]) + (part[g + 2][tt] + part[g + 3][tt]);
+            out[v * H + cbase + tt] = p.finish(blk, v, cbase + tt, sum);
+        }
+        __syncthreads();
+    }
+}
+
+}
+}
diff --git a/sgs-gnn_amd/csrc/losses.hip b/sgs-gnn_amd/csrc/losses.hip
--- a/sgs-gnn_amd/csrc/losses.hip
+++ b/sgs-gnn_amd/csrc/losses.hip
@@ -2,6 +2,7 @@
 #include <atomic>
 
 #include "sgs_common.h"
+#include "endpoint_reduce.h"
 
 namespace sgs {
 namespace {
@@ -137,11 +138,8 @@
     }
 }
 
-__global__ void __launch_bounds__(kT) ce_rows(const float* __restrict__ logits, int64_t N, int64_t C, const int64_t* __restrict__ y,
-                                             const uint8_t* __restrict__ mask, float* __restrict__ row_lse,
-                                             float* __restrict__ rowloss) {
-    const int lane = threadIdx.x & 63;
-    const int64_t i = (static_cast<int64_t>(blockIdx.x) * kT + threadIdx.x) >> 6;
+__device__ __forceinline__ void ce_row(int64_t i, int lane, const float* __restrict__ logits, int64_t N, int64_t C, const int64_t* __restrict__ y,
+                                       const uint8_t* __restrict__ mask, float* __restrict__ row_lse, float* __restrict__ rowloss) {
     if (i >= N) return;
     if (!mask[i]) {
         if (lane == 0) { rowloss[i] = 0.f; row_lse[i] = 0.f; }
@@ -158,6 +156,11 @@
         row_lse[i] = lse;
         rowloss[i] = lse - logits[i * C + y[i]];
     }
+}
+__global__ void __launch_bounds__(kT) ce_rows(const float* __restrict__ logits, int64_t N, int64_t C, const int64_t* __restrict__ y,
+                                             const uint8_t* __restrict__ mask, float* __restrict__ row_lse,
+                                             float* __restrict__ rowloss) {
+    ce_row((static_cast<int64_t>(blockIdx.x) * kT + threadIdx.x) >> 6, threadIdx.x & 63, logits, N, C, y, mask, row_lse, rowloss);
 }
 
 __global__ void __launch_bounds__(1024) ce_final(const float* __restrict__ rowloss, const uint8_t* __restrict__ mask, int64_t N,
@@ -309,11 +312,9 @@
     return weight ? weight[yi] : 1.f;
 }
 
-__global__ void __launch_bounds__(kT) ce_rows_w(const float* __restrict__ logits, int64_t N, int64_t C, const int64_t* __restrict__ y,
-                                               const uint8_t* __restrict__ mask, const float* __restrict__ weight, float eps,
-                                               float* __restrict__ row_lse, float* __restrict__ rowloss) {
-    const int lane = threadIdx.x & 63;
-    const int64_t i = (static_cast<int64_t>(blockIdx.x) * kT + threadIdx.x) >> 6;
+__device__ __forceinline__ void ce_row_w(int64_t i, int lane, const float* __restrict__ logits, int64_t N, int64_t C,
+                                         const int64_t* __restrict__ y, const uint8_t* __restrict__ mask, const float* __restrict__ weight,
+                                         float eps, float* __restrict__ row_lse, float* __restrict__ rowloss) {
     if (i >= N) return;
     if (!mask[i]) {
         if (lane == 0) { rowloss[i] = 0.f; row_lse[i] = 0.f; }
@@ -338,6 +339,11 @@
         row_lse[i] = lse;
         rowloss[i] = (eps != 0.f) ? (1.f - eps) * hard + (eps / static_cast<float>(C)) * sm : hard;
     }
+}
+__global__ void __launch_bounds__(kT) ce_rows_w(const float* __restrict__ logits, int64_t N, int64_t C, const int64_t* __restrict__ y,
+                                               const uint8_t* __restrict__ mask, const float* __restrict__ weight, float eps,
+                                               float* __restrict__ row_lse, float* __restrict__ rowloss) {
+    ce_row_w((static_cast<int64_t>(blockIdx.x) * kT + threadIdx.x) >> 6, threadIdx.x & 63, logits, N, C, y, mask, weight, eps, row_lse, rowloss);
 }
 
 __global__ void __launch_bounds__(1024) ce_final_w(const float* __restrict__ rowloss, const uint8_t* __restrict__ mask,
@@ -477,6 +483,198 @@
         Gd[j * C + c] = -r * (a * inv - cy * b);
     }
 }
+
+template <bool kW>
+__global__ void __launch_bounds__(kT) hybrid_fwd_pair(const float* __restrict__ w, const int64_t* __restrict__ sei, int64_t q,
+                                                     const float* __restrict__ logits, int64_t N, int64_t C, const int64_t* __restrict__ y,
+                                                     const uint8_t* __restrict__ tm, int64_t nce, float coef2, float q_norm,
+                                                     const float* __restrict__ weight, float eps, float* __restrict__ part,
+                                                     float4* __restrict__ stash, float* __restrict__ row_lse, float* __restrict__ rowloss) {
+    const int64_t blk = static_cast<int64_t>(blockIdx.x) - nce;
+    if (blk < 0) {
+        const int64_t i = (static_cast<int64_t>(blockIdx.x) * kT + threadIdx.x) >> 6;
+        if (kW) ce_row_w(i, threadIdx.x & 63, logits, N, C, y, tm, weight, eps, row_lse, rowloss);
+        else    ce_row(i, threadIdx.x & 63, logits, N, C, y, tm, row_lse, rowloss);
+        return;
+    }
+    __shared__ float red[4][kT / 64];
+    const int sub = threadIdx.x & 15, grp = threadIdx.x >> 4;
+    int64_t jj[kRegRounds], s[kRegRounds], d[kRegRounds];
+    bool live[kRegRounds];
+#pragma unroll
+    for (int r = 0; r < kRegRounds; ++r) {
+        const int64_t j = blk * kRegEdges + r * (kT / 16) + grp;
+        live[r] = j < q;
+        jj[r] = live[r] ? j : 0;
+    }
+#pragma unroll
+    for (int r = 0; r < kRegRounds; ++r) { s[r] = sei[jj[r]]; d[r] = sei[q + jj[r]]; }
+    float wj[kRegRounds];
+    uint8_t ts[kRegRounds], td[kRegRounds];
+    int64_t ys[kRegRounds], yd[kRegRounds];
+#pragma unroll
+    for (int r = 0; r < kRegRounds; ++r) { wj[r] = w[jj[r]]; ts[r] = tm[s[r]]; td[r] = tm[d[r]]; ys[r] = y[s[r]]; yd[r] = y[d[r]]; }
+    float dot[kRegRounds], nx[kRegRounds], ny[kRegRounds];
+#pragma unroll
+    for (int r = 0; r < kRegRounds; ++r) { dot[r] = 0.f; nx[r] = 0.f; ny[r] = 0.f; }
+    for (int64_t c = sub; c < C; c += 16) {
+        float a[kRegRounds], b[kRegRounds];
+#pragma unroll
+        for (int r = 0; r < kRegRounds; ++r) { a[r] = logits[s[r] * C + c]; b[r] = logits[d[r] * C + c]; }
+#pragma unroll
+        for (int r = 0; r < kRegRounds; ++r) {
+            dot[r] = fmaf(a[r], b[r], dot[r]); nx[r] = fmaf(a[r], a[r], nx[r]); ny[r] = fmaf(b[r], b[r], ny[r]);
+        }
+    }
+#pragma unroll
+    for (int r = 0; r < kRegRounds; ++r) { dot[r] = row16_sum_all_dpp(dot[r]); nx[r] = row16_sum_all_dpp(nx[r]); ny[r] = row16_sum_all_dpp(ny[r]); }
+    float dt = dot[0], sx = nx[0], sy = ny[0], wr = wj[0];
+    bool on = live[0], valid = ts[0] && td[0], same = ys[0] == yd[0];
+    int64_t je = jj[0];
+#pragma unroll
+    for (int r = 1; r < kRegRounds; ++r)
+        if (sub == r) {
+            dt = dot[r]; sx = nx[r]; sy = ny[r]; wr = wj[r];
+            on = live[r]; valid = ts[r] && td[r]; same = ys[r] == yd[r];
+            je = jj[r];
+        }
+    on = on && sub < kRegRounds;
+    float t_bce = 0.f, t_sq = 0.f, t_nv = 0.f, t_nl = 0.f;
+    if (on) {
+        const float cs = cos_from(EdgeTerms{dt, sx, sy});
+        const float df = wr - cs;
+        t_sq = df * df;
+        if (valid) {
+            t_nv = 1.f;
+            t_nl = same ? 1.f : 0.f;
+            t_bce = same ? -fmaxf(logf(wr), -100.f) : -fmaxf(logf(1.f - wr), -100.f);
+        }
+        if (stash) {
+            const float den2 = fmaxf(sx * sy, 1e-16f);
+            const float inv = 1.0f / sqrtf(den2);
+            const float csb = dt * inv;
+            const float r0 = 2.0f * (wr - csb) / q_norm * coef2;
+            const bool clamped = sx * sy < 1e-16f;
+            const float cx = clamped ? 0.f : csb / sx, cy = clamped ? 0.f : csb / sy;
+            stash[je] = make_float4(inv, cx, cy, r0);
+        }
+    }
+    float bce = 0.f, sq = 0.f, nv = 0.f, nl = 0.f;
+    const int g0 = threadIdx.x & 48;
+#pragma unroll
+    for (int r = 0; r < kRegRounds; ++r) {
+        bce += __shfl(t_bce, g0 + r, 64); sq += __shfl(t_sq, g0 + r, 64); nv += __shfl(t_nv, g0 + r, 64); nl += __shfl(t_nl, g0 + r, 64);
+    }
+    if (sub != 0) { bce = 0.f; sq = 0.f; nv = 0.f; nl = 0.f; }
+    bce = wave_sum(bce); sq = wave_sum(sq); nv = wave_sum(nv); nl = wave_sum(nl);
+    if ((threadIdx.x & 63) == 0) {
+        const int wid = threadIdx.x >> 6;
+        red[0][wid] = bce; red[1][wid] = sq; red[2][wid] = nv; red[3][wid] = nl;
+    }
+    __syncthreads();
+    if (threadIdx.x == 0) {
+        float r[4];
+#pragma unroll
+        for (int k = 0; k < 4; ++k) {
+            r[k] = 0.f;
+            for (int i = 0; i < kT / 64; ++i) r[k] += red[k][i];
+        }
+        part[4 * blk + 0] = r[0]; part[4 * blk + 1] = r[1];
+        part[4 * blk + 2] = r[2]; part[4 * blk + 3] = r[3];
+    }
+}
+
+template <bool kW>
+struct EpHybridTerms {
+    static constexpr bool kCol = true, kVisit = true;
+    const float* __restrict__ logits;
+    int64_t C;
+    const float4* __restrict__ stash;
+    const float* __restrict__ w;
+    const int64_t* __restrict__ y;
+    const uint8_t* __restrict__ tm;
+    const float* __restrict__ out7;
+    float coef1;
+    const float* __restrict__ grad_loss;
+    float* __restrict__ dw;
+    const float* __restrict__ weight;
+    float eps;
+    const float* __restrict__ row_lse;
+    const void* __restrict__ norm;
+    struct Blk { float W, gl, nvalid; bool reg1; };
+    struct Own { float x; };
+    struct Raw { float4 st; float nb; };
+    template <class T>
+    static __device__ __forceinline__ T uniform_load(const T* ptr) {
+        return *(const __attribute__((address_space(4))) T*)(ptr);
+    }
+    __device__ __forceinline__ Blk block_init() const {
+        __shared__ float red[4];
+        Blk b;
+        b.W = static_cast<float>(C);
+        b.gl = uniform_load(grad_loss);
+        b.nvalid = uniform_load(out7 + 2);
+        b.reg1 = coef1 != 0.f && uniform_load(out7 + 3) > 1.f;
+        if (kW && eps != 0.f && weight) {
+            float v = 0.f;
+            if (threadIdx.x < 256) {
+                for (int64_t c = threadIdx.x; c < C; c += 256) v += weight[c];
+                v = wave_sum_all(v);
+                if ((threadIdx.x & 63) == 0) red[threadIdx.x >> 6] = v;
+            }
+            __syncthreads();
+            float r = 0.f;
+#pragma unroll
+            for (int k = 0; k < 4; ++k) r += red[k];
+            b.W = r;
+        }
+        return b;
+    }
+    __device__ __forceinline__ Own own(int64_t v, int64_t, int64_t c0) const { return Own{logits[v * C + c0]}; }
+    struct Pre { float word; };
+    __device__ __forceinline__ Pre preload(int e_lane, int lane) const {
+        return Pre{reinterpret_cast<const float*>(stash)[static_cast<int64_t>(e_lane) * 4 + ((lane >> 2) & 3)]};
+    }
+    __device__ __forceinline__ Raw load(const Pre& pre, int u, bool, int, int col, int64_t, int64_t c0) const {
+        const int wd = __float_as_int(pre.word);
+        Raw r;
+        r.st = make_float4(__int_as_float(__builtin_amdgcn_readlane(wd, u)), __int_as_float(__builtin_amdgcn_readlane(wd, 4 + u)),
+                           __int_as_float(__builtin_amdgcn_readlane(wd, 8 + u)), __int_as_float(__builtin_amdgcn_readlane(wd, 12 + u)));
+        r.nb = logits[static_cast<int64_t>(col) * C + c0];
+        return r;
+    }
+    __device__ __forceinline__ void term(const Blk& blk, const Raw& rw, const Own& o, bool isout, float (&m)[1], float (&t)[1]) const {
+        const float inv = rw.st.x, cx = rw.st.y, cy = rw.st.z;
+        const float r = rw.st.w * blk.gl;
+        const float a = isout ? o.x : rw.nb, b = isout ? rw.nb : o.x;
+        m[0] = isout ? -r * (b * inv - cx * a) : -r * (a * inv - cy * b);
+        t[0] = 1.f;
+    }
+    __device__ __forceinline__ void visit(const Blk& blk, int64_t v, int e, int col) const {
+        const float gl = blk.gl;
+        const float wj = w[e];
+        const float r = stash[e].w * gl;
+        float g = r;
+        if (blk.reg1 && tm[v] && tm[col]) {
+            const float tgt = (y[v] == y[col]) ? 1.f : 0.f;
+            g += coef1 * gl * (wj - tgt) / fmaxf((1.f - wj) * wj, 1e-12f) / blk.nvalid;
+        }
+        dw[e] = g;
+    }
+    __device__ __forceinline__ float finish(const Blk& blk, int64_t v, int64_t c, float sum) const {
+        if (!tm[v]) return sum;
+        const int64_t idx = v * C + c;
+        if (!kW) {
+            const float sm = expf(logits[idx] - row_lse[v]);
+            return sum + (sm - (y[v] == c ? 1.f : 0.f)) * (grad_loss[0] / static_cast<float>(static_cast<const int*>(norm)[0]));
+        }
+        const float d = static_cast<const float*>(norm)[0];
+        const float sc = (d == 0.f) ? NAN : grad_loss[0] / d;
+        const int64_t yi = y[v];
+        return sum + ce_w_grad(logits[idx], row_lse[v], yi == c, class_weight(weight, yi, C), weight ? weight[c] : 1.f, blk.W, eps,
+                               1.f / static_cast<float>(C), sc);
+    }
+};
 
 
 __global__ void __launch_bounds__(kT) ensemble_mean_correct(const float* __restrict__ logits, int64_t xs, int Dc, int64_t N, int64_t C,
@@ -813,6 +1011,69 @@
     return SGS_OK;
 }
 
+int sgs_hybrid_loss_fused_fwd(const float* logits, int64_t N, int64_t C, const int64_t* y, const uint8_t* train_mask, const float* w,
+                              const int64_t* sampled_edge_index, int64_t q, float coef1, float coef2, int weighted, const float* weight,
+                              float label_smoothing, float* out, float* row_lse, float* rowloss, void* norm, float* stash, void* ws,
+                              size_t ws_bytes, sgs_stream_t stream_) {
+    hipStream_t stream = static_cast<hipStream_t>(stream_);
+    SGS_REQUIRE(q > 0 && N > 0 && N < (int64_t(1) << 24) && C > 0 && logits && y && train_mask && w && sampled_edge_index && out && row_lse &&
+                    rowloss && norm,
+                SGS_EINVAL, "sgs_hybrid_loss_fused_fwd: bad arguments");
+    SGS_REQUIRE(weighted ? (label_smoothing >= 0.f && label_smoothing <= 1.f) : (!weight && label_smoothing == 0.f), SGS_EINVAL,
+                "sgs_hybrid_loss_fused_fwd: label_smoothing outside [0, 1], or a weight / smoothing without `weighted`");
+    SGS_REQUIRE((reinterpret_cast<uintptr_t>(stash) & 15) == 0, SGS_EINVAL, "sgs_hybrid_loss_fused_fwd: stash must be 16-byte aligned");
+    SGS_REQUIRE(ws && ws_bytes >= sgs_edge_reg_workspace_bytes(q), SGS_EWORKSPACE, "sgs_hybrid_loss_fused_fwd: workspace too small");
+    Carver cv(ws);
+    const int64_t nblk = cdiv(q, kRegEdges);
+    float* part = cv.take<float>(4 * (nblk + 1));
+    const int64_t nce = cdiv(N * 64, kT);
+    const dim3 grid(static_cast<unsigned>(nce + nblk));
+    float4* st = reinterpret_cast<float4*>(stash);
+    if (weighted) {
+        hipLaunchKernelGGL(hybrid_fwd_pair<true>, grid, dim3(kT), 0, stream, w, sampled_edge_index, q, logits, N, C, y, train_mask, nce, coef2,
+                           static_cast<float>(q), weight, label_smoothing, part, st, row_lse, rowloss);
+        hipLaunchKernelGGL(hybrid_loss_final_w, dim3(1), dim3(kT), 0, stream, part, nblk, q, coef1, coef2, rowloss, train_mask, y, weight, N, C, out,
+                           static_cast<float*>(norm));
+    } else {
+        hipLaunchKernelGGL(hybrid_fwd_pair<false>, grid, dim3(kT), 0, stream, w, sampled_edge_index, q, logits, N, C, y, train_mask, nce, coef2,
+                           static_cast<float>(q), weight, label_smoothing, part, st, row_lse, rowloss);
+        hipLaunchKernelGGL(hybrid_loss_final, dim3(1), dim3(kT), 0, stream, part, nblk, q, coef1, coef2, rowloss, train_mask, N, out,
+                           static_cast<int*>(norm));
+    }
+    SGS_LAUNCH_OK();
+    return SGS_OK;
+}
+
+int sgs_hybrid_loss_fused_bwd(const float* logits, int64_t N, int64_t C, const int64_t* y, const uint8_t* train_mask, const float* w, int64_t q,
+                              const float* stash, const float* out, float coef1, int weighted, const float* weight, float label_smoothing,
+                              const float* row_lse, const void* norm, const float* grad_loss, const int32_t* in_ptr, const int32_t* in_src,
+                              const int32_t* in_eid, const int32_t* out_ptr, const int32_t* out_dst, const int32_t* out_eid, float* dw,
+                              float* dlogits, sgs_stream_t stream_) {
+    hipStream_t stream = static_cast<hipStream_t>(stream_);
+    SGS_REQUIRE(q > 0 && N > 0 && N < (int64_t(1) << 31) && C > 0 && logits && y && train_mask && w && stash && out && row_lse && norm && grad_loss &&
+                    in_ptr && in_src && in_eid && out_ptr && out_dst && out_eid && dw && dlogits,
+                SGS_EINVAL, "sgs_hybrid_loss_fused_bwd: bad arguments");
+    SGS_REQUIRE(weighted ? (label_smoothing >= 0.f && label_smoothing <= 1.f) : (!weight && label_smoothing == 0.f), SGS_EINVAL,
+                "sgs_hybrid_loss_fused_bwd: label_smoothing outside [0, 1], or a weight / smoothing without `weighted`");
+    SGS_REQUIRE((reinterpret_cast<uintptr_t>(stash) & 15) == 0, SGS_EINVAL, "sgs_hybrid_loss_fused_bwd: stash must be 16-byte aligned");
+    const int nw = ep_traversal(q, N);
+#define SGS_HYB(KW_)                                                                                                                              \
+    do {                                                                                                                                          \
+        const EpHybridTerms<KW_> terms{logits, C, reinterpret_cast<const float4*>(stash), w, y, train_mask, out, coef1, grad_loss, dw, weight,    \
+                                       label_smoothing, row_lse, norm};                                                                           \
+        if (nw == 16)     hipLaunchKernelGGL((endpoint_reduce_rowblock<1, 16, EpHybridTerms<KW_>>), dim3(static_cast<unsigned>(N)), dim3(1024), 0, stream, \
+                                             terms, N, C, in_ptr, in_src, in_eid, out_ptr, out_dst, out_eid, 1.0f, 1.0f, dlogits);               \
+        else if (nw == 4) hipLaunchKernelGGL((endpoint_reduce_rowblock<1, 4, EpHybridTerms<KW_>>), dim3(static_cast<unsigned>(N)), dim3(256), 0, stream,   \
+                                             terms, N, C, in_ptr, in_src, in_eid, out_ptr, out_dst, out_eid, 1.0f, 1.0f, dlogits);               \
+        else              hipLaunchKernelGGL((endpoint_reduce<1, EpHybridTerms<KW_>>), dim3(static_cast<unsigned>(cdiv(N * 64, kEpT))), dim3(kEpT), 0,     \
+                                             stream, terms, N, C, in_ptr, in_src, in_eid, out_ptr, out_dst, out_eid, 1.0f, 1.0f, dlogits);       \
+    } while (0)
+    if (weighted) SGS_HYB(true); else SGS_HYB(false);
+#undef SGS_HYB
+    SGS_LAUNCH_OK();
+    return SGS_OK;
+}
+
 int sgs_ensemble_mean_correct(const float* logits, int64_t x_stride, int64_t Dc, int64_t N, int64_t C, float* acc, int first, int last,
                               int64_t D_total, const int64_t* y, const uint8_t* mask0, const uint8_t* mask1, const uint8_t* mask2, int64_t* counts,
                               sgs_stream_t stream_) {
diff --git a/sgs-gnn_amd/ops.py b/sgs-gnn_amd/ops.py
--- a/sgs-gnn_amd/ops.py
+++ b/sgs-gnn_amd/ops.py
@@ -1291,16 +1291,22 @@
         rowloss = torch.empty(N, dtype=torch.float32, device=dev)
         ws = workspace(L.sgs_edge_reg_workspace_bytes(q), dev)
         ctx.plain = weight is None and eps == 0.0
-        if ctx.plain:
-            n_rows = torch.empty(1, dtype=torch.int32, device=dev)
+        n_rows = torch.empty(1, dtype=torch.int32 if ctx.plain else torch.float32, device=dev)
+        stash = None
+        if coef2 != 0.0:
+            if ctx.needs_input_grad[0] or ctx.needs_input_grad[3]:
+                stash = torch.empty(q, 4, dtype=torch.float32, device=dev)
+            _lib.check(L.sgs_hybrid_loss_fused_fwd(_ptr(logits), N, C, _ptr(y), _ptr(mask_u8), _ptr(w), _ptr(sei), q, float(coef1), float(coef2),
+                                                   0 if ctx.plain else 1, _ptr(weight), eps, _ptr(out), _ptr(row_lse), _ptr(rowloss), _ptr(n_rows),
+                                                   _ptr(stash), ws.data_ptr(), ws.numel(), _stream()), "sgs_hybrid_loss_fused_fwd")
+        elif ctx.plain:
             _lib.check(L.sgs_hybrid_loss_fwd(_ptr(logits), N, C, _ptr(y), _ptr(mask_u8), _ptr(w), _ptr(sei), q, float(coef1), float(coef2), _ptr(out),
                                              _ptr(row_lse), _ptr(rowloss), _ptr(n_rows), ws.data_ptr(), ws.numel(), _stream()), "sgs_hybrid_loss_fwd")
         else:
-            n_rows = torch.empty(1, dtype=torch.float32, device=dev)
             _lib.check(L.sgs_hybrid_loss_w_fwd(_ptr(logits), N, C, _ptr(y), _ptr(mask_u8), _ptr(w), _ptr(sei), q, float(coef1), float(coef2),
                                                _ptr(weight), eps, _ptr(out), _ptr(row_lse), _ptr(rowloss), _ptr(n_rows), ws.data_ptr(), ws.numel(),
                                                _stream()), "sgs_hybrid_loss_w_fwd")
-        ctx.save_for_backward(logits, y, mask_u8, w, sei, out, row_lse, n_rows, weight)
+        ctx.save_for_backward(logits, y, mask_u8, w, sei, out, row_lse, n_rows, weight, stash)
         ctx.eps = eps
         ctx.graph, ctx.coef1, ctx.coef2 = graph, float(coef1), float(coef2)
         ctx.nm_ref = getattr(w, "_sgs_norm", None)
@@ -1310,27 +1316,31 @@
     @staticmethod
     def backward(ctx, g):
         L = _lib.lib()
-        logits, y, mask_u8, w, sei, out, row_lse, n_rows, weight = ctx.saved_tensors
+        logits, y, mask_u8, w, sei, out, row_lse, n_rows, weight, stash = ctx.saved_tensors
         q = w.numel()
         N, C = logits.shape
         dev = w.device
         g = g.reshape(1).contiguous().float()
         dw = torch.empty(q, dtype=torch.float32, device=dev)
-        Gs = torch.empty(q, C, dtype=torch.float32, device=dev)
-        Gd = torch.empty(q, C, dtype=torch.float32, device=dev)
-        _lib.check(L.sgs_edge_reg_bwd(_ptr(w), _ptr(sei), q, q, _ptr(logits), N, C, _ptr(y), _ptr(mask_u8), _ptr(out), ctx.coef1,
-                                      ctx.coef2, _ptr(g), _ptr(dw), _ptr(Gs), _ptr(Gd), _stream()), "sgs_edge_reg_bwd")
-        dlogits = _endpoint_reduce(Gs, Gd, None, ctx.graph, 1.0, 1.0, C) if ctx.coef2 != 0.0 else torch.empty_like(logits)
-        if not ctx.plain:
-            fn, what = (L.sgs_masked_ce_w_bwd_acc, "sgs_masked_ce_w_bwd_acc") if ctx.coef2 != 0.0 else (L.sgs_masked_ce_w_bwd, "sgs_masked_ce_w_bwd")
-            _lib.check(fn(_ptr(logits), N, C, _ptr(y), _ptr(mask_u8), _ptr(weight), ctx.eps, _ptr(row_lse), _ptr(n_rows), _ptr(g), _ptr(dlogits),
-                          _stream()), what)
-        elif ctx.coef2 != 0.0:
-            _lib.check(L.sgs_masked_ce_bwd_acc(_ptr(logits), N, C, _ptr(y), _ptr(mask_u8), _ptr(row_lse), _ptr(n_rows), _ptr(g), _ptr(dlogits),
-                                               _stream()), "sgs_masked_ce_bwd_acc")
+        if ctx.coef2 != 0.0:
+            gr = ctx.graph
+            dlogits = torch.empty_like(logits)
+            _lib.check(L.sgs_hybrid_loss_fused_bwd(_ptr(logits), N, C, _ptr(y), _ptr(mask_u8), _ptr(w), q, _ptr(stash), _ptr(out), ctx.coef1,
+                                                   0 if ctx.plain else 1, _ptr(weight), ctx.eps, _ptr(row_lse), _ptr(n_rows), _ptr(g), _ptr(gr.in_ptr),
+                                                   _ptr(gr.in_src), _ptr(gr.in_eid), _ptr(gr.out_ptr), _ptr(gr.out_dst), _ptr(gr.out_eid), _ptr(dw),
+                                                   _ptr(dlogits), _stream()), "sgs_hybrid_loss_fused_bwd")
         else:
-            _lib.check(L.sgs_masked_ce_bwd(_ptr(logits), N, C, _ptr(y), _ptr(mask_u8), _ptr(row_lse), _ptr(n_rows), _ptr(g), _ptr(dlogits),
-                                           _stream()), "sgs_masked_ce_bwd")
+            Gs = torch.empty(q, C, dtype=torch.float32, device=dev)
+            Gd = torch.empty(q, C, dtype=torch.float32, device=dev)
+            _lib.check(L.sgs_edge_reg_bwd(_ptr(w), _ptr(sei), q, q, _ptr(logits), N, C, _ptr(y), _ptr(mask_u8), _ptr(out), ctx.coef1,
+                                          ctx.coef2, _ptr(g), _ptr(dw), _ptr(Gs), _ptr(Gd), _stream()), "sgs_edge_reg_bwd")
+            dlogits = torch.empty_like(logits)
+            if not ctx.plain:
+                _lib.check(L.sgs_masked_ce_w_bwd(_ptr(logits), N, C, _ptr(y), _ptr(mask_u8), _ptr(weight), ctx.eps, _ptr(row_lse), _ptr(n_rows),
+                                                 _ptr(g), _ptr(dlogits), _stream()), "sgs_masked_ce_w_bwd")
+            else:
+                _lib.check(L.sgs_masked_ce_bwd(_ptr(logits), N, C, _ptr(y), _ptr(mask_u8), _ptr(row_lse), _ptr(n_rows), _ptr(g), _ptr(dlogits),
+                                               _stream()), "sgs_masked_ce_bwd")
         nm = ctx.nm_ref() if ctx.nm_ref is not None else None
         if nm is not None and getattr(nm, "_park_ok", False) and dw.numel() == nm.graph.n_edges:
             import weakref
```

Result: faster. 111.2 million (median of 6 runs) (+3.2%).
